# victordeleau/MUI-DeepAutoEncoder

Measured on AMD Instinct MI355X. Metric: training samples/sec at 3x512-dim input, batch 8192, higher is better.
Workload: dtype bf16; 1 GPU; embedding.yaml topology: 3 slots x 512 (io 1536), z=io, 4+4 layers -> 10 x Linear(1536,1536); batch 8192 rows per GPU, Adam lr 1e-5 wd 1e-4 clip 1.0, slot-blanking k=1; global_batch=8192, parallelism=dp1

## Files before the change

### mui-deepautoencoder_amd/csrc/codae_common.h

```cpp
#pragma once
#include <hip/hip_runtime.h>
#include <stdint.h>
#include <stdio.h>
#include <type_traits>

#include "codae_hip.h"

namespace codae {

void set_error(const char* fmt, ...);

#define CODAE_HIP_CHECK(expr)                                                              \
    do {                                                                                   \
        hipError_t e_ = (expr);                                                            \
        if (e_ != hipSuccess) {                                                            \
            codae::set_error("%s failed: %s (%s:%d)", #expr, hipGetErrorString(e_), __FILE__, __LINE__); \
            return CODAE_E_HIP;                                                            \
        }                                                                                  \
    } while (0)

#define CODAE_LAUNCH_CHECK()                                                               \
    do {                                                                                   \
        hipError_t e_ = hipGetLastError();                                                 \
        if (e_ != hipSuccess) {                                                            \
            codae::set_error("kernel launch failed: %s (%s:%d)", hipGetErrorString(e_), __FILE__, __LINE__); \
            return CODAE_E_HIP;                                                            \
        }                                                                                  \
    } while (0)

#define CODAE_REQUIRE(cond, ...)                                                           \
    do {                                                                                   \
        if (!(cond)) {                                                                     \
            codae::set_error(__VA_ARGS__);                                                 \
            return CODAE_E_INVALID;                                                        \
        }                                                                                  \
    } while (0)

typedef uint16_t bf16_t;

typedef __attribute__((ext_vector_type(16))) float f32x16;
typedef __attribute__((ext_vector_type(4))) float f32x4;
typedef __attribute__((ext_vector_type(8))) __bf16 bf16x8;
typedef __attribute__((ext_vector_type(4))) short s16x4;
typedef __attribute__((ext_vector_type(8))) short s16x8;
typedef __attribute__((ext_vector_type(2))) unsigned int u32x2;
typedef __attribute__((ext_vector_type(4))) unsigned int u32x4;

__device__ __forceinline__ float bf16_to_f32(bf16_t v) { return __uint_as_float(((uint32_t)v) << 16); }
__device__ __forceinline__ bf16_t f32_to_bf16(float f) {
    __bf16 b = (__bf16)f;
    return __builtin_bit_cast(bf16_t, b);
}

__device__ __forceinline__ uint32_t pack_bf16x2(float lo, float hi) {
    typedef float f32x2_t __attribute__((ext_vector_type(2)));
    typedef __bf16 bf16x2_t __attribute__((ext_vector_type(2)));
    const f32x2_t v = {lo, hi};
    return __builtin_bit_cast(uint32_t, __builtin_convertvector(v, bf16x2_t));
}
__device__ __forceinline__ float clamp_below(float x, float floor) {
    float r;
    asm("v_maximum3_f32 %0, %1, %2, %2" : "=v"(r) : "v"(x), "v"(floor));
    return r;
}

__device__ __forceinline__ float4 load_bias4(const float* __restrict__ bias, const void* valid, int j, int N) {
    const bool ok = bias != nullptr && j < N;
    const float4 v = *reinterpret_cast<const float4*>(ok ? bias + j : reinterpret_cast<const float*>(valid));
    return make_float4(ok ? v.x : 0.f, ok ? v.y : 0.f, ok ? v.z : 0.f, ok ? v.w : 0.f);
}

__device__ __forceinline__ float act_opaque(float x) { asm("" : "+v"(x)); return x; }
__device__ __forceinline__ float act_exp(float x) { return __builtin_amdgcn_exp2f(act_opaque(x * 1.44269504f)); }
__device__ __forceinline__ float act_log(float x) { return act_opaque(__builtin_amdgcn_logf(x)) * 0.693147181f; }
__device__ __forceinline__ float act_rcp(float x) { return __builtin_amdgcn_rcpf(x); }
__device__ __forceinline__ float act_expm1(float x) {
    const float u = act_opaque(act_exp(x));
    const float um1 = act_opaque(u - 1.f);
    if (u == 1.f) return x;
    if (um1 == -1.f) return -1.f;
    return act_opaque(um1 * x) * act_rcp(act_log(u));
}
__device__ __forceinline__ float act_log1p(float t) {
    const float u = act_opaque(1.f + t);
    if (u == 1.f) return t;
    return act_opaque(act_log(u) * t) * act_rcp(act_opaque(u - 1.f));
}
__device__ __forceinline__ float act_fwd_(int kind, const float* p, float v) {
    switch (kind) {
        case CODAE_ACT_RELU: return clamp_below(v, 0.f);
        case CODAE_ACT_LEAKY: return v > 0.f ? v : v * p[0];
        case CODAE_ACT_RELU6: return v <= 0.f ? 0.f : (v >= 6.f ? 6.f : v);
        case CODAE_ACT_ELU: return v > 0.f ? v * p[0] : act_expm1(v * p[2]) * act_opaque(p[1] * p[0]);
        case CODAE_ACT_SOFTPLUS: return v * p[0] > p[1] ? v : act_log1p(act_exp(v * p[0])) * act_rcp(p[0]);
        case CODAE_ACT_HARDSIGMOID: { const float t = clamp_below(v + 3.f, 0.f); return (t > 6.f ? 6.f : t) * (1.f / 6.f); }
        default: return v;
    }
}
__device__ __forceinline__ float act_fwd(int kind, const float* p, float v) {
    asm("" : "+v"(v));
    float r = act_fwd_(kind, p, v);
    asm("" : "+v"(r));
    return r;
}
__device__ __forceinline__ float act_dy_from_y_(int kind, const float* p, float y) {
    switch (kind) {
        case CODAE_ACT_RELU: return y > 0.f ? 1.f : 0.f;
        case CODAE_ACT_LEAKY: return y > 0.f ? 1.f : p[0];
        case CODAE_ACT_RELU6: return (y > 0.f && y < 6.f) ? 1.f : 0.f;
        case CODAE_ACT_ELU: return y > 0.f ? p[0] : p[2] * act_opaque(y + act_opaque(p[1] * p[0]));
        case CODAE_ACT_SOFTPLUS: return y * p[0] > p[1] ? 1.f : -act_expm1(-y * p[0]);
        case CODAE_ACT_HARDSIGMOID: return (y > 0.f && y < 1.f) ? 1.f / 6.f : 0.f;
        default: return 1.f;
    }
}
__device__ __forceinline__ float act_dy_from_y(int kind, const float* p, float y) {
    asm("" : "+v"(y));
    float r = act_dy_from_y_(kind, p, y);
    asm("" : "+v"(r));
    return r;
}

__device__ __forceinline__ float act_bwd(int kind, const float* p, float g, float y) {
    const float d = act_dy_from_y(kind, p, y);
    const bool selects = kind == CODAE_ACT_RELU || kind == CODAE_ACT_RELU6 || kind == CODAE_ACT_HARDSIGMOID;
    return (selects && d == 0.f) ? 0.f : g * d;
}

template <typename F>
__device__ __forceinline__ void act_dispatch(int kind, F&& f) {
    switch (kind) {
        case CODAE_ACT_RELU: f(std::integral_constant<int, CODAE_ACT_RELU>{}); break;
        case CODAE_ACT_LEAKY: f(std::integral_constant<int, CODAE_ACT_LEAKY>{}); break;
        case CODAE_ACT_RELU6: f(std::integral_constant<int, CODAE_ACT_RELU6>{}); break;
        case CODAE_ACT_ELU: f(std::integral_constant<int, CODAE_ACT_ELU>{}); break;
        case CODAE_ACT_SOFTPLUS: f(std::integral_constant<int, CODAE_ACT_SOFTPLUS>{}); break;
        case CODAE_ACT_HARDSIGMOID: f(std::integral_constant<int, CODAE_ACT_HARDSIGMOID>{}); break;
        default: f(std::integral_constant<int, CODAE_ACT_NONE>{}); break;
    }
}

__device__ __forceinline__ uint32_t act_dgrad_bf16x2(int kind, const float* p, uint32_t g2, uint32_t h2) {
    const float lo = act_bwd(kind, p, bf16_to_f32((bf16_t)(g2 & 0xffffu)), bf16_to_f32((bf16_t)(h2 & 0xffffu)));
    const float hi = act_bwd(kind, p, bf16_to_f32((bf16_t)(g2 >> 16)), bf16_to_f32((bf16_t)(h2 >> 16)));
    return pack_bf16x2(lo, hi);
}

static inline int64_t round_up(int64_t x, int64_t m) { return (x + m - 1) / m * m; }

struct EnvToggles {
    int gemm_tile = -1;
    int gemm_dbg = 0;
    int wgrad_splitk = 0;
    int small_tile_max = 200;
    int small_stages = 4;
    int f32_gemm = 0;
    int group_tile = -1;
    bool side_priority_set = false; int side_priority = 0;
    bool no_wt = false, single_stream = false, tail_on_side = false, no_fused_loss = false, flat_adam = false,
         no_fused_norm = false, no_chain = false, no_deep_small = false,
         no_relu_bits = false,
         no_prefetch = false,
         no_defer_wgrad = false;
};
const EnvToggles& env();
void env_reload();

struct GemmF32 {
    const float* A; int64_t a_rs, a_ks;
    const float* B; int64_t b_rs, b_ks;
    float* C; int64_t ldc;
    int M, N, K;
    const float* bias;
    int relu;
    const float* relu_src;
    int64_t ld_relu;
    float* colsum_part;
    const int* m_dev;
    int split_k;
    int act;
    float act_p[3];
};
int gemm_f32(const GemmF32& g, hipStream_t s);
int gemm_f32x3(const GemmF32& g, hipStream_t s);
bool gemm_f32x3_takes(const GemmF32& g);
inline int gemm_f32_colsum_rows(int M) { return (M + 63) / 64; }

constexpr int CODAE_GROUP_MAX = 16;
struct GemmF32Group {
    int n;
    GemmF32 g[CODAE_GROUP_MAX];
    int wg_begin[CODAE_GROUP_MAX + 1];
};
int gemm_f32x3_grouped(GemmF32Group& grp, hipStream_t s);

enum { OP_KC = 0,
       OP_KS = 1
};
struct LossFuse {
    int enabled;
    const float* data;
    const int32_t* row_idx;
    const int32_t* mask_id;
    const int32_t* mask_to_use;
    int nb_run, run;
    const uint8_t* table;
    int io;
    int B;
    float inv_n;
    double* parts;
};

struct GemmBf16 {
    const bf16_t* A; int64_t lda; int a_mode;
    const bf16_t* B; int64_t ldb; int b_mode;
    void* C; int64_t ldc; int c_f32;
    int M, N, K;
    const float* bias;
    int relu;
    const bf16_t* relu_src; int64_t ld_relu;
    float* colsum_part;
    int split_k;
    LossFuse loss;
    int dbg;
    uint8_t* relu_bits_out; const uint8_t* relu_bits; int64_t ld_bits;
    const void* prefetch; int64_t prefetch_bytes;
    int coscheduled;
    double* sumsq_slots;
    int act;
    float act_p[3];
};
bool gemm_bf16_supported(int M, int N, int K);
bool gemm_bf16_takes_relu_bits(int M, int N);
int gemm_bf16_colsum_rows(const GemmBf16& g);
int gemm_bf16_loss_parts(const GemmBf16& g);
int gemm_bf16(const GemmBf16& g, hipStream_t s);
int gemm_bf16_pipe(const GemmBf16& g, int cfg, hipStream_t s);
int choose_split_k(int N, int K, int rows);

struct GemmBf16Group {
    int n;
    GemmBf16 g[CODAE_GROUP_MAX];
    int wg_begin[CODAE_GROUP_MAX + 1];
};
int gemm_bf16_grouped(GemmBf16Group& grp, hipStream_t s);
int gemm_bf16_pipe_grouped(GemmBf16Group& grp, hipStream_t s);

constexpr int CODAE_CHAIN_MAX_WIDTH = 512;
constexpr int CODAE_CHAIN_MAX_LAYERS = 16;
constexpr int CODAE_CHAIN_MAX_BIAS = 6144;
struct ChainArgs {
    int L, rows, B;
    int width[CODAE_CHAIN_MAX_LAYERS + 1];
    uint32_t relu_flags;
    double* scalars;
    const bf16_t* W[CODAE_CHAIN_MAX_LAYERS];
    const bf16_t* Wt[CODAE_CHAIN_MAX_LAYERS];
    const float* bias[CODAE_CHAIN_MAX_LAYERS];
    bf16_t* act[CODAE_CHAIN_MAX_LAYERS];
    bf16_t* dact[CODAE_CHAIN_MAX_LAYERS];
    float* colsum_part[CODAE_CHAIN_MAX_LAYERS];
    const float* data; const int32_t* row_idx; const int32_t* mask_id; const uint8_t* mask_table;
    const int32_t* mask_to_use; int nb_run, run;
    float inv_n;
    double* loss_parts;
    int do_backward;
};
bool chain_supported(int L, const int* in, const int* out);
int chain_rows_per_workgroup();
int launch_chain_step(const ChainArgs& a, hipStream_t s);

int launch_gather_corrupt(const codae_batch* b, void* out, int out_bf16, hipStream_t s, int64_t out_ld = 0);
int check_noise(const codae_noise* noise);
int launch_gather_noise(const codae_batch* b, const codae_noise* noise, int32_t step, const double* step_dev, void* out,
                        int out_bf16, hipStream_t s, int64_t out_ld = 0, const int32_t* noise_rows = nullptr);
int launch_noise_box_muller(const uint32_t* ra, const uint32_t* rb, float* rho, float* c, float* sn, int64_t n, hipStream_t s);
int launch_cast_bf16(const float* src, bf16_t* dst, int64_t n, hipStream_t s);
int launch_corrupt(const float* x, const float* mask, float* out, int64_t n, hipStream_t s);
int launch_expand_masks(const int32_t* mask_id, const uint8_t* table, const int32_t* k_of_mask, int B, int io,
                        int k_max, float* masks_out, float* fmask_out, hipStream_t s);
int launch_mse_loss(const codae_batch* b, const float* y, void* dy, int dy_bf16, float inv_n, float* colsum_part,
                    double* loss_parts, int want_grad, hipStream_t s, int64_t dy_ld = 0);
int mse_loss_colsum_rows(int B);
int launch_mse_dense(const float* x, const float* y, const float* fmask, float* dy, int64_t n, float inv_n,
                     double* scalars, hipStream_t s);
int launch_sumsq(const float* g, int64_t n, double* out, hipStream_t s);
int launch_sumsq_to(const float* g, int64_t n, double* acc, hipStream_t s);
int launch_clip_coef(const double* total_sq, float max_norm, double* coef_out, hipStream_t s);
int launch_clip_adam(float* p, float* g, float* m, float* v, int64_t n, const codae_hyper* hp,
                     const double* grad_sq, bf16_t* shadow, const double* coef_in, hipStream_t s,
                     const double* step_dev = nullptr);
int launch_set_scalar(double* dst, double value, hipStream_t s);
int launch_clip_adam_tiled(float* p, float* g, float* m, float* v, const codae_hyper* hp, const double* grad_sq,
                           bf16_t* shadow, bf16_t* shadow_t, int n_layers, const int64_t* w_off, const int* rows,
                           const int* cols, int transposed_from, int64_t bias_off, int64_t bias_n, hipStream_t s,
                           const double* step_dev = nullptr);
int launch_transpose_bf16(const bf16_t* src, bf16_t* dst, int n, const int64_t* off, const int* rows, const int* cols,
                          hipStream_t s);
int gemm_bf16_timeline(unsigned long long* host_out, int n_wg);
int launch_reduce_slabs_epi(const float* slabs, int n_slabs, int64_t stride, int M, int N, float* C, int64_t ldc, const float* bias,
                            int relu, const float* relu_src, int64_t ld_relu, float* colsum_part, hipStream_t s,
                            int act = CODAE_ACT_NONE, const float* act_p = nullptr);
int launch_reduce_slabs(const float* slabs, int n_slabs, int64_t slab_stride, float* out, int64_t n, double* sumsq,
                        hipStream_t s);
int launch_finish_loss(double* scalars, double inv_n, hipStream_t s, const double* parts = nullptr, int n_parts = 0);
int launch_cast_f32(const bf16_t* src, float* dst, int64_t n, hipStream_t s);
int launch_colsum_f32(const float* src, int M, int N, float* out, hipStream_t s);
int launch_colsum_parts_f32(const float* src, int M, int N, float* parts, hipStream_t s);
struct BiasFinishJobs {
    int n;
    const float* parts[64];
    float* out[64];
    int rows[64], cols[64];
    int col_begin[65];
};
struct LossFinish { double* scalars; double inv_n; const double* parts; int n_parts; };
int launch_bias_finish(const BiasFinishJobs& jobs, double* sumsq, hipStream_t s, const LossFinish* loss = nullptr);

}
```

### mui-deepautoencoder_amd/csrc/elementwise.hip

```cpp
#include "codae_common.h"

namespace codae {
namespace {

constexpr int NT = 256;

inline int grid_for(int64_t work_items) {
    int64_t b = (work_items + NT - 1) / NT;
    if (b < 1) b = 1;
    if (b > 2048) b = 2048;
    return (int)b;
}

__device__ __forceinline__ float wave_sum(float v) {
#pragma unroll
    for (int o = 32; o > 0; o >>= 1) v += __shfl_xor(v, o);
    return v;
}

__device__ __forceinline__ float block_sum(float v, float* red ) {
    v = wave_sum(v);
    const int w = threadIdx.x >> 6;
    if ((threadIdx.x & 63) == 0) red[w] = v;
    __syncthreads();
    float r = 0.f;
    if (threadIdx.x == 0) r = red[0] + red[1] + red[2] + red[3];
    __syncthreads();
    return r;
}

__device__ __forceinline__ uint2 pack_bf16x4(float a, float b, float c, float d) {
    uint2 o;
    o.x = (uint32_t)f32_to_bf16(a) | ((uint32_t)f32_to_bf16(b) << 16);
    o.y = (uint32_t)f32_to_bf16(c) | ((uint32_t)f32_to_bf16(d) << 16);
    return o;
}

__global__ __launch_bounds__(NT) void gather_corrupt_bf16x8_kernel(const float* __restrict__ data,
                                                                   const int32_t* __restrict__ row_idx,
                                                                   const int32_t* __restrict__ mask_id,
                                                                   const uint8_t* __restrict__ table, int B, int io,
                                                                   bf16_t* __restrict__ out,
                                                                   const int32_t* __restrict__ mask_to_use, int nb_run,
                                                                   int run, int64_t out_ld) {
    const bool masked = (mask_id != nullptr) || (mask_to_use != nullptr);
    const int cols = io / 8;
    const int64_t total = (int64_t)B * cols;
    for (int64_t e = (int64_t)blockIdx.x * NT + threadIdx.x; e < total; e += (int64_t)gridDim.x * NT) {
        const int b = (int)(e / cols);
        const int c = (int)(e - (int64_t)b * cols) * 8;
        const int64_t src_row = row_idx ? row_idx[b] : b;
        const float* src = data + src_row * io + c;
        const float4 x0 = *reinterpret_cast<const float4*>(src);
        const float4 x1 = *reinterpret_cast<const float4*>(src + 4);
        float v[8] = {x0.x, x0.y, x0.z, x0.w, x1.x, x1.y, x1.z, x1.w};
        if (masked) {
            const int id = mask_id ? mask_id[b] : mask_to_use[src_row * nb_run + run];
            const uint2 m = *reinterpret_cast<const uint2*>(table + (int64_t)id * io + c);
#pragma unroll
            for (int k = 0; k < 8; ++k) v[k] = (((k < 4 ? m.x : m.y) >> (8 * (k & 3))) & 0xff) ? v[k] : 0.f;
        }
        uint4 o;
        o.x = pack_bf16x2(v[0], v[1]); o.y = pack_bf16x2(v[2], v[3]);
        o.z = pack_bf16x2(v[4], v[5]); o.w = pack_bf16x2(v[6], v[7]);
        *reinterpret_cast<uint4*>(out + (int64_t)b * out_ld + c) = o;
    }
}

template <bool VEC, bool OUT_BF16>
__global__ __launch_bounds__(NT) void gather_corrupt_kernel(const float* __restrict__ data,
                                                            const int32_t* __restrict__ row_idx,
                                                            const int32_t* __restrict__ mask_id,
                                                            const uint8_t* __restrict__ table, int B, int io,
                                                            void* __restrict__ out,
                                                            const int32_t* __restrict__ mask_to_use, int nb_run,
                                                            int run, int64_t out_ld) {
    constexpr int W = VEC ? 4 : 1;
    const bool masked = (mask_id != nullptr) || (mask_to_use != nullptr);
    const int cols = io / W;
    const int64_t total = (int64_t)B * cols;
    for (int64_t e = (int64_t)blockIdx.x * NT + threadIdx.x; e < total; e += (int64_t)gridDim.x * NT) {
        const int b = (int)(e / cols);
        const int c = (int)(e - (int64_t)b * cols) * W;
        const int64_t src_row = row_idx ? row_idx[b] : b;
        const float* src = data + src_row * io + c;
        float v[4];
        if constexpr (VEC) {
            const float4 x = *reinterpret_cast<const float4*>(src);
            v[0] = x.x; v[1] = x.y; v[2] = x.z; v[3] = x.w;
            if (masked) {
                const int id = mask_id ? mask_id[b] : mask_to_use[src_row * nb_run + run];
                const uint32_t m = *reinterpret_cast<const uint32_t*>(table + (int64_t)id * io + c);
#pragma unroll
                for (int k = 0; k < 4; ++k) v[k] = ((m >> (8 * k)) & 0xff) ? v[k] : 0.f;
            }
        } else {
            v[0] = src[0];
            if (masked) {
                const int id = mask_id ? mask_id[b] : mask_to_use[src_row * nb_run + run];
                v[0] = table[(int64_t)id * io + c] ? v[0] : 0.f;
            }
        }
        const int64_t o = (int64_t)b * out_ld + c;
        if constexpr (OUT_BF16) {
            bf16_t* op = reinterpret_cast<bf16_t*>(out) + o;
            if constexpr (VEC) *reinterpret_cast<uint2*>(op) = pack_bf16x4(v[0], v[1], v[2], v[3]);
            else op[0] = f32_to_bf16(v[0]);
        } else {
            float* op = reinterpret_cast<float*>(out) + o;
            if constexpr (VEC) *reinterpret_cast<float4*>(op) = make_float4(v[0], v[1], v[2], v[3]);
            else op[0] = v[0];
        }
    }
}

struct NoiseArgs {
    uint32_t key0, key1;
    uint32_t step;
    const double* step_dev;
    const int32_t* rows;
    uint64_t thresh;
    float p0, p1, p2;
};

__device__ __forceinline__ uint4 philox4x32_10(uint32_t c0, uint32_t c1, uint32_t c2, uint32_t c3, uint32_t k0, uint32_t k1) {
#pragma unroll
    for (int r = 0; r < 10; ++r) {
        const uint32_t hi0 = __umulhi(0xD2511F53u, c0), lo0 = 0xD2511F53u * c0;
        const uint32_t hi1 = __umulhi(0xCD9E8D57u, c2), lo1 = 0xCD9E8D57u * c2;
        c0 = hi1 ^ c1 ^ k0; c1 = lo1; c2 = hi0 ^ c3 ^ k1; c3 = lo0;
        k0 += 0x9E3779B9u; k1 += 0xBB67AE85u;
    }
    return make_uint4(c0, c1, c2, c3);
}

__device__ __forceinline__ void box_muller_parts(uint32_t ra, uint32_t rb, float& rho, float& c, float& sn) {
    const float u1 = (float)((ra >> 8) + 1u) * 5.9604644775390625e-8f;
    const float two_u2 = (float)(rb >> 8) * 1.1920928955078125e-7f;
    rho = sqrtf(-2.f * logf(u1));
    sincospif(two_u2, &sn, &c);
}

__device__ __forceinline__ float noise_elem(int kind_masking, uint32_t rk, float x, const NoiseArgs& a) {
    const bool hit = (uint64_t)rk < a.thresh;
    if (kind_masking) return hit ? 0.f : x;
    return hit ? ((uint64_t)rk < (a.thresh >> 1) ? a.p1 : a.p2) : x;
}

template <int KIND>
__device__ __forceinline__ void noise_apply4(float* v, const uint4 r, const NoiseArgs& a) {
    if constexpr (KIND == CODAE_NOISE_GAUSSIAN) {
        float rho, c, sn;
        box_muller_parts(r.x, r.y, rho, c, sn);
        v[0] = fmaf(a.p0, rho * c, v[0]); v[1] = fmaf(a.p0, rho * sn, v[1]);
        box_muller_parts(r.z, r.w, rho, c, sn);
        v[2] = fmaf(a.p0, rho * c, v[2]); v[3] = fmaf(a.p0, rho * sn, v[3]);
    } else {
        constexpr int M = KIND == CODAE_NOISE_MASKING;
        v[0] = noise_elem(M, r.x, v[0], a); v[1] = noise_elem(M, r.y, v[1], a);
        v[2] = noise_elem(M, r.z, v[2], a); v[3] = noise_elem(M, r.w, v[3], a);
    }
}

template <int KIND>
__device__ __forceinline__ float noise_apply1(float x, const uint4 r, int k, const NoiseArgs& a) {
    if constexpr (KIND == CODAE_NOISE_GAUSSIAN) {
        float rho, c, sn;
        box_muller_parts((k & 2) ? r.z : r.x, (k & 2) ? r.w : r.y, rho, c, sn);
        return fmaf(a.p0, rho * ((k & 1) ? sn : c), x);
    } else {
        const uint32_t rk = (k & 2) ? ((k & 1) ? r.w : r.z) : ((k & 1) ? r.y : r.x);
        return noise_elem(KIND == CODAE_NOISE_MASKING, rk, x, a);
    }
}

template <int KIND>
__global__ __launch_bounds__(NT) void gather_noise_bf16x8_kernel(const float* __restrict__ data, const int32_t* __restrict__ row_idx,
                                                                 const int32_t* __restrict__ mask_id, const uint8_t* __restrict__ table,
                                                                 int B, int io, bf16_t* __restrict__ out,
                                                                 const int32_t* __restrict__ mask_to_use, int nb_run, int run,
                                                                 int64_t out_ld, NoiseArgs na) {
    const bool masked = (mask_id != nullptr) || (mask_to_use != nullptr);
    const uint32_t step = na.step_dev ? (uint32_t)*na.step_dev : na.step;
    const int cols = io / 8;
    const int64_t total = (int64_t)B * cols;
    for (int64_t e = (int64_t)blockIdx.x * NT + threadIdx.x; e < total; e += (int64_t)gridDim.x * NT) {
        const int b = (int)(e / cols);
        const int c = (int)(e - (int64_t)b * cols) * 8;
        const int64_t src_row = row_idx ? row_idx[b] : b;
        const float* src = data + src_row * io + c;
        const float4 x0 = *reinterpret_cast<const float4*>(src);
        const float4 x1 = *reinterpret_cast<const float4*>(src + 4);
        float v[8] = {x0.x, x0.y, x0.z, x0.w, x1.x, x1.y, x1.z, x1.w};
        const uint32_t nrow = na.rows ? (uint32_t)na.rows[b] : (uint32_t)src_row;
        noise_apply4<KIND>(v, philox4x32_10((uint32_t)(c >> 2), nrow, step, 0u, na.key0, na.key1), na);
        noise_apply4<KIND>(v + 4, philox4x32_10((uint32_t)(c >> 2) + 1u, nrow, step, 0u, na.key0, na.key1), na);
        if (masked) {
            const int id = mask_id ? mask_id[b] : mask_to_use[src_row * nb_run + run];
            const uint2 m = *reinterpret_cast<const uint2*>(table + (int64_t)id * io + c);
#pragma unroll
            for (int k = 0; k < 8; ++k) v[k] = (((k < 4 ? m.x : m.y) >> (8 * (k & 3))) & 0xff) ? v[k] : 0.f;
        }
        uint4 o;
        o.x = pack_bf16x2(v[0], v[1]); o.y = pack_bf16x2(v[2], v[3]);
        o.z = pack_bf16x2(v[4], v[5]); o.w = pack_bf16x2(v[6], v[7]);
        *reinterpret_cast<uint4*>(out + (int64_t)b * out_ld + c) = o;
    }
}

template <bool VEC, bool OUT_BF16, int KIND>
__global__ __launch_bounds__(NT) void gather_noise_kernel(const float* __restrict__ data, const int32_t* __restrict__ row_idx,
                                                          const int32_t* __restrict__ mask_id, const uint8_t* __restrict__ table, int B,
                                                          int io, void* __restrict__ out, const int32_t* __restrict__ mask_to_use,
                                                          int nb_run, int run, int64_t out_ld, NoiseArgs na) {
    constexpr int W = VEC ? 4 : 1;
    const bool masked = (mask_id != nullptr) || (mask_to_use != nullptr);
    const uint32_t step = na.step_dev ? (uint32_t)*na.step_dev : na.step;
    const int cols = io / W;
    const int64_t total = (int64_t)B * cols;
    for (int64_t e = (int64_t)blockIdx.x * NT + threadIdx.x; e < total; e += (int64_t)gridDim.x * NT) {
        const int b = (int)(e / cols);
        const int c = (int)(e - (int64_t)b * cols) * W;
        const int64_t src_row = row_idx ? row_idx[b] : b;
        const float* src = data + src_row * io + c;
        const uint32_t nrow = na.rows ? (uint32_t)na.rows[b] : (uint32_t)src_row;
        const uint4 r = philox4x32_10((uint32_t)(c >> 2), nrow, step, 0u, na.key0, na.key1);
        float v[4];
        if constexpr (VEC) {
            const float4 x = *reinterpret_cast<const float4*>(src);
            v[0] = x.x; v[1] = x.y; v[2] = x.z; v[3] = x.w;
            noise_apply4<KIND>(v, r, na);
            if (masked) {
                const int id = mask_id ? mask_id[b] : mask_to_use[src_row * nb_run + run];
                const uint32_t m = *reinterpret_cast<const uint32_t*>(table + (int64_t)id * io + c);
#pragma unroll
                for (int k = 0; k < 4; ++k) v[k] = ((m >> (8 * k)) & 0xff) ? v[k] : 0.f;
            }
        } else {
            v[0] = src[0];
            v[0] = noise_apply1<KIND>(v[0], r, c & 3, na);
            if (masked) {
                const int id = mask_id ? mask_id[b] : mask_to_use[src_row * nb_run + run];
                v[0] = table[(int64_t)id * io + c] ? v[0] : 0.f;
            }
        }
        const int64_t o = (int64_t)b * out_ld + c;
        if constexpr (OUT_BF16) {
            bf16_t* op = reinterpret_cast<bf16_t*>(out) + o;
            if constexpr (VEC) *reinterpret_cast<uint2*>(op) = pack_bf16x4(v[0], v[1], v[2], v[3]);
            else op[0] = f32_to_bf16(v[0]);
        } else {
            float* op = reinterpret_cast<float*>(out) + o;
            if constexpr (VEC) *reinterpret_cast<float4*>(op) = make_float4(v[0], v[1], v[2], v[3]);
            else op[0] = v[0];
        }
    }
}

__global__ __launch_bounds__(NT) void noise_box_muller_kernel(const uint32_t* __restrict__ ra, const uint32_t* __restrict__ rb,
                                                              float* __restrict__ rho, float* __restrict__ c, float* __restrict__ sn,
                                                              int64_t n) {
    for (int64_t e = (int64_t)blockIdx.x * NT + threadIdx.x; e < n; e += (int64_t)gridDim.x * NT)
        box_muller_parts(ra[e], rb[e], rho[e], c[e], sn[e]);
}

__global__ __launch_bounds__(NT) void cast_bf16_kernel(const float* __restrict__ src, bf16_t* __restrict__ dst,
                                                       int64_t n) {
    const int64_t n4 = n / 4;
    for (int64_t e = (int64_t)blockIdx.x * NT + threadIdx.x; e < n4; e += (int64_t)gridDim.x * NT) {
        const float4 x = reinterpret_cast<const float4*>(src)[e];
        reinterpret_cast<uint2*>(dst)[e] = pack_bf16x4(x.x, x.y, x.z, x.w);
    }
    for (int64_t e = n4 * 4 + (int64_t)blockIdx.x * NT + threadIdx.x; e < n; e += (int64_t)gridDim.x * NT)
        dst[e] = f32_to_bf16(src[e]);
}

__global__ __launch_bounds__(NT) void cast_f32_kernel(const bf16_t* __restrict__ src, float* __restrict__ dst,
                                                      int64_t n) {
    for (int64_t e = (int64_t)blockIdx.x * NT + threadIdx.x; e < n; e += (int64_t)gridDim.x * NT)
        dst[e] = bf16_to_f32(src[e]);
}

__global__ __launch_bounds__(NT) void corrupt_kernel(const float* __restrict__ x, const float* __restrict__ m,
                                                     float* __restrict__ out, int64_t n) {
    for (int64_t e = (int64_t)blockIdx.x * NT + threadIdx.x; e < n; e += (int64_t)gridDim.x * NT)
        out[e] = x[e] * m[e];
}

__global__ __launch_bounds__(NT) void expand_masks_kernel(const int32_t* __restrict__ mask_id,
                                                          const uint8_t* __restrict__ table,
                                                          const int32_t* __restrict__ k_of_mask, int B, int io,
                                                          int k_max, float* __restrict__ masks,
                                                          float* __restrict__ fmask) {
    const int64_t total = (int64_t)B * io;
    for (int64_t e = (int64_t)blockIdx.x * NT + threadIdx.x; e < total; e += (int64_t)gridDim.x * NT) {
        const int b = (int)(e / io);
        const int c = (int)(e - (int64_t)b * io);
        const int id = mask_id[b];
        const float v = table[(int64_t)id * io + c] ? 1.f : 0.f;
        const int k = k_of_mask[id] - 1;
        for (int kk = 0; kk < k_max; ++kk) masks[(int64_t)kk * total + e] = (kk == k) ? v : 0.f;
        fmask[e] = v;
    }
}

constexpr int LOSS_ROWS = 32;
constexpr int LOSS_UNROLL = 8;
template <bool VEC, bool DY_BF16>
__global__ __launch_bounds__(NT) void mse_loss_kernel(const float* __restrict__ data,
                                                      const int32_t* __restrict__ row_idx,
                                                      const int32_t* __restrict__ mask_id,
                                                      const uint8_t* __restrict__ table, int B, int io,
                                                      const float* __restrict__ y, void* __restrict__ dy,
                                                      float inv_n, float* __restrict__ colsum_part,
                                                      double* __restrict__ loss_parts, int want_grad,
                                                      const int32_t* __restrict__ mask_to_use, int nb_run, int run, int64_t dy_ld) {
    __shared__ float red[4];
    const bool masked = (mask_id != nullptr) || (mask_to_use != nullptr);
    constexpr int W = VEC ? 4 : 1;
    const int cols = io / W;
    const int r_begin = blockIdx.x * LOSS_ROWS;
    float sq = 0.f, sqp = 0.f;
    for (int cv = threadIdx.x; cv < cols; cv += NT) {
        const int c = cv * W;
        float cs[4] = {0.f, 0.f, 0.f, 0.f};
        for (int r0 = 0; r0 < LOSS_ROWS; r0 += LOSS_UNROLL)
#pragma unroll
        for (int ru = 0; ru < LOSS_UNROLL; ++ru) {
            const int rr = r0 + ru;
            const bool live = r_begin + rr < B;
            const int b = live ? r_begin + rr : B - 1;
            const int64_t src_row = row_idx ? row_idx[b] : b;
            float xv[4], yv[4];
            uint32_t m = 0x01010101u;
            const int id = !masked ? 0 : (mask_id ? mask_id[b] : mask_to_use[src_row * nb_run + run]);
            if constexpr (VEC) {
                const float4 x4 = *reinterpret_cast<const float4*>(data + src_row * io + c);
                const float4 y4 = *reinterpret_cast<const float4*>(y + (int64_t)b * io + c);
                xv[0] = x4.x; xv[1] = x4.y; xv[2] = x4.z; xv[3] = x4.w;
                yv[0] = y4.x; yv[1] = y4.y; yv[2] = y4.z; yv[3] = y4.w;
                if (masked) m = *reinterpret_cast<const uint32_t*>(table + (int64_t)id * io + c);
            } else {
                xv[0] = data[src_row * io + c];
                yv[0] = y[(int64_t)b * io + c];
                if (masked) m = table[(int64_t)id * io + c];
            }
            float g[4];
#pragma unroll
            for (int k = 0; k < W; ++k) {
                const float d = live ? xv[k] - yv[k] : 0.f;
                const float se = d * d;
                sq += se;
                if (((m >> (8 * k)) & 0xff) == 0) sqp += se;
                g[k] = -2.f * d * inv_n;
                cs[k] += g[k];
            }
            if (want_grad && live) {
                const int64_t o = (int64_t)b * dy_ld + c;
                if constexpr (DY_BF16) {
                    bf16_t* op = reinterpret_cast<bf16_t*>(dy) + o;
                    if constexpr (VEC) *reinterpret_cast<uint2*>(op) = pack_bf16x4(g[0], g[1], g[2], g[3]);
                    else op[0] = f32_to_bf16(g[0]);
                } else {
                    float* op = reinterpret_cast<float*>(dy) + o;
                    if constexpr (VEC) *reinterpret_cast<float4*>(op) = make_float4(g[0], g[1], g[2], g[3]);
                    else op[0] = g[0];
                }
// ... 218 lines not shown
                    a.z = act_bwd(act, p, a.z, h.z); a.w = act_bwd(act, p, a.w, h.w);
                } else {
                    a.x = act_fwd(act, p, a.x); a.y = act_fwd(act, p, a.y); a.z = act_fwd(act, p, a.z); a.w = act_fwd(act, p, a.w);
                }
            } else {
                if (relu) { a.x = clamp_below(a.x, 0.f); a.y = clamp_below(a.y, 0.f); a.z = clamp_below(a.z, 0.f); a.w = clamp_below(a.w, 0.f); }
                if (relu_src != nullptr) {
                    const float4 h = *reinterpret_cast<const float4*>(relu_src + (int64_t)i * ld_relu + j);
                    a.x = h.x > 0.f ? a.x : 0.f; a.y = h.y > 0.f ? a.y : 0.f; a.z = h.z > 0.f ? a.z : 0.f; a.w = h.w > 0.f ? a.w : 0.f;
                }
            }
            *reinterpret_cast<float4*>(C + (int64_t)i * ldc + j) = a;
            cs[0] += a.x; cs[1] += a.y; cs[2] += a.z; cs[3] += a.w;
        }
    }
    if (colsum_part != nullptr) {
        red[rg][cg * 4 + 0] = cs[0]; red[rg][cg * 4 + 1] = cs[1]; red[rg][cg * 4 + 2] = cs[2]; red[rg][cg * 4 + 3] = cs[3];
        __syncthreads();
        if (threadIdx.x < 64 && blockIdx.x * 64 + (int)threadIdx.x < N) {
            float t = 0.f;
            for (int r = 0; r < 16; ++r) t += red[r][threadIdx.x];
            colsum_part[(int64_t)blockIdx.y * N + blockIdx.x * 64 + threadIdx.x] = t;
        }
    }
}

__global__ __launch_bounds__(NT) void colsum_parts_f32_kernel(const float* __restrict__ src, int M, int N,
                                                              float* __restrict__ parts) {
    const int r_begin = blockIdx.x * 64;
    const int r_end = min(M, r_begin + 64);
    const int c = blockIdx.y * NT + threadIdx.x;
    if (c >= N) return;
    float s = 0.f;
    for (int r0 = r_begin; r0 < r_end; r0 += 8) {
        float v[8];
#pragma unroll
        for (int k = 0; k < 8; ++k) v[k] = src[(int64_t)min(r0 + k, r_end - 1) * N + c];
#pragma unroll
        for (int k = 0; k < 8; ++k) s += (r0 + k < r_end) ? v[k] : 0.f;
    }
    parts[(int64_t)blockIdx.x * N + c] = s;
}

__global__ __launch_bounds__(NT) void colsum_f32_kernel(const float* __restrict__ src, int M, int N,
                                                        float* __restrict__ out) {
    const int c = blockIdx.x * NT + threadIdx.x;
    if (c >= N) return;
    float s = 0.f;
    for (int r = 0; r < M; ++r) s += src[(int64_t)r * N + c];
    out[c] = s;
}

__global__ __launch_bounds__(NT) void bias_finish_kernel(BiasFinishJobs jobs, double* __restrict__ sumsq, LossFinish lf) {
    __shared__ float red[4];
    if (lf.scalars != nullptr && blockIdx.x == gridDim.x - 1) {
        __shared__ double lred[2][NT];
        double a = 0.0, b = 0.0;
        for (int i = threadIdx.x; i < lf.n_parts; i += NT) { a += lf.parts[2 * i]; b += lf.parts[2 * i + 1]; }
        lred[0][threadIdx.x] = a; lred[1][threadIdx.x] = b;
        __syncthreads();
        for (int o = NT / 2; o > 0; o >>= 1) {
            if ((int)threadIdx.x < o) { lred[0][threadIdx.x] += lred[0][threadIdx.x + o]; lred[1][threadIdx.x] += lred[1][threadIdx.x + o]; }
            __syncthreads();
        }
        if (threadIdx.x == 0) {
            lf.scalars[CODAE_S_SQ_FULL] += lred[0][0];
            lf.scalars[CODAE_S_SQ_PARTIAL] += lred[1][0];
            lf.scalars[CODAE_S_LAST_LOSS] = lred[0][0] * lf.inv_n;
            lf.scalars[CODAE_S_STEP_SQ] = 0.0;
        }
        return;
    }
    const int gc = blockIdx.x * NT + threadIdx.x;
    float sq = 0.f;
    if (gc < jobs.col_begin[jobs.n]) {
        int j = 0;
        while (j + 1 < jobs.n && gc >= jobs.col_begin[j + 1]) ++j;
        const int c = gc - jobs.col_begin[j];
        const int N = jobs.cols[j], R = jobs.rows[j];
        const float* p = jobs.parts[j] + c;
        float s = 0.f;
        int r = 0;
        for (; r + 32 <= R; r += 32) {
            float v[32];
#pragma unroll
            for (int u = 0; u < 32; ++u) v[u] = p[(int64_t)(r + u) * N];
#pragma unroll
            for (int u = 0; u < 32; ++u) s += v[u];
        }
        for (; r + 8 <= R; r += 8) {
            float v[8];
#pragma unroll
            for (int u = 0; u < 8; ++u) v[u] = p[(int64_t)(r + u) * N];
#pragma unroll
            for (int u = 0; u < 8; ++u) s += v[u];
        }
        for (; r < R; ++r) s += p[(int64_t)r * N];
        jobs.out[j][c] = s;
        sq = s * s;
    }
    if (sumsq != nullptr) {
        const float bsq = block_sum(sq, red);
        if (threadIdx.x == 0)
            atomicAdd(sumsq + (CODAE_S_GRAD_SQ_SLOTS - CODAE_S_GRAD_SQ) + (blockIdx.x & (CODAE_S_N_SLOTS - 1)), (double)bsq);
    }
}

struct TransposeJobs {
    int n;
    int64_t off[64];
    int rows[64], cols[64];
    int tile_begin[65];
};
__global__ __launch_bounds__(NT) void transpose_bf16_kernel(const bf16_t* __restrict__ src, bf16_t* __restrict__ dst,
                                                            TransposeJobs jobs) {
    __shared__ bf16_t tile[64][72];
    int m = 0;
    while (m + 1 < jobs.n && (int)blockIdx.x >= jobs.tile_begin[m + 1]) ++m;
    const int t = blockIdx.x - jobs.tile_begin[m];
    const int R = jobs.rows[m], C = jobs.cols[m];
    const int tiles_c = (C + 63) / 64;
    const int r0 = (t / tiles_c) * 64, c0 = (t % tiles_c) * 64;
    const bf16_t* S = src + jobs.off[m];
    bf16_t* D = dst + jobs.off[m];
#pragma unroll
    for (int p = 0; p < 2; ++p) {
        const int q = threadIdx.x + p * NT;
        const int r = q >> 3, c8 = (q & 7) * 8;
        uint4 v = make_uint4(0u, 0u, 0u, 0u);
        if (r0 + r < R && c0 + c8 < C) v = *reinterpret_cast<const uint4*>(S + (int64_t)(r0 + r) * C + c0 + c8);
        *reinterpret_cast<uint4*>(&tile[r][c8]) = v;
    }
    __syncthreads();
#pragma unroll
    for (int p = 0; p < 2; ++p) {
        const int q = threadIdx.x + p * NT;
        const int c = q >> 3, r8 = (q & 7) * 8;
        if (c0 + c < C && r0 + r8 < R) {
            bf16_t e[8];
#pragma unroll
            for (int k = 0; k < 8; ++k) e[k] = tile[r8 + k][c];
            uint4 v;
            v.x = (uint32_t)e[0] | ((uint32_t)e[1] << 16); v.y = (uint32_t)e[2] | ((uint32_t)e[3] << 16);
            v.z = (uint32_t)e[4] | ((uint32_t)e[5] << 16); v.w = (uint32_t)e[6] | ((uint32_t)e[7] << 16);
            *reinterpret_cast<uint4*>(D + (int64_t)(c0 + c) * R + r0 + r8) = v;
        }
    }
}

inline bool a16(const void* p) { return (reinterpret_cast<uintptr_t>(p) & 15) == 0; }

}

int launch_gather_corrupt(const codae_batch* b, void* out, int out_bf16, hipStream_t s, int64_t out_ld) {
    if (out_ld <= 0) out_ld = b ? b->io : 0;
    CODAE_REQUIRE(b && b->data && out && b->B > 0 && b->io > 0, "gather_corrupt: bad batch");
    const bool masked = b->mask_id || b->mask_to_use;
    CODAE_REQUIRE(!masked || b->mask_table, "gather_corrupt: mask ids without mask_table");
    CODAE_REQUIRE(!b->mask_to_use || b->mask_id || (b->nb_run > 0 && b->run >= 0 && b->run < b->nb_run),
                  "gather_corrupt: run %d outside [0, %d)", b->run, b->nb_run);
    const bool vec = (b->io % 4 == 0) && (out_ld % 4 == 0) && a16(b->data) && a16(out) && (!masked || (reinterpret_cast<uintptr_t>(b->mask_table) & 3) == 0);
    const int64_t items = (int64_t)b->B * (vec ? b->io / 4 : b->io);
    const int grid = grid_for(items);
    if (vec && out_bf16 && b->io % 8 == 0 && (!masked || (reinterpret_cast<uintptr_t>(b->mask_table) & 7) == 0)) {
        hipLaunchKernelGGL(gather_corrupt_bf16x8_kernel, dim3(grid_for(items / 2)), dim3(NT), 0, s, b->data, b->row_idx, b->mask_id,
                           b->mask_table, b->B, b->io, reinterpret_cast<bf16_t*>(out), b->mask_to_use, b->nb_run, b->run, out_ld);
        CODAE_LAUNCH_CHECK();
        return CODAE_OK;
    }
#define GC(V, O) hipLaunchKernelGGL((gather_corrupt_kernel<V, O>), dim3(grid), dim3(NT), 0, s, b->data, b->row_idx, \
                                    b->mask_id, b->mask_table, b->B, b->io, out, b->mask_to_use, b->nb_run, b->run, out_ld)
    if (vec && out_bf16) GC(true, true);
    else if (vec) GC(true, false);
    else if (out_bf16) GC(false, true);
    else GC(false, false);
#undef GC
    CODAE_LAUNCH_CHECK();
    return CODAE_OK;
}

static bool finite_f(float x) { return x == x && fabsf(x) <= 3.402823466e38f; }

int check_noise(const codae_noise* n) {
    if (n == nullptr || n->kind == CODAE_NOISE_NONE) return CODAE_OK;
    CODAE_REQUIRE(n->kind == CODAE_NOISE_GAUSSIAN || n->kind == CODAE_NOISE_MASKING || n->kind == CODAE_NOISE_SALT_PEPPER,
                  "input noise: unknown kind %d", n->kind);
    if (n->kind == CODAE_NOISE_GAUSSIAN) {
        CODAE_REQUIRE(finite_f(n->p0) && n->p0 >= 0.f, "input noise: sigma %g must be finite and >= 0", (double)n->p0);
        return CODAE_OK;
    }
    CODAE_REQUIRE(finite_f(n->p0) && n->p0 >= 0.f && n->p0 <= 1.f, "input noise: p %g outside [0, 1]", (double)n->p0);
    if (n->kind == CODAE_NOISE_SALT_PEPPER) {
        CODAE_REQUIRE(finite_f(n->p1), "input noise: lo %g is not finite", (double)n->p1);
        CODAE_REQUIRE(finite_f(n->p2), "input noise: hi %g is not finite", (double)n->p2);
    }
    return CODAE_OK;
}

int launch_gather_noise(const codae_batch* b, const codae_noise* noise, int32_t step, const double* step_dev, void* out, int out_bf16,
                        hipStream_t s, int64_t out_ld, const int32_t* noise_rows) {
    if (noise == nullptr || noise->kind == CODAE_NOISE_NONE) return launch_gather_corrupt(b, out, out_bf16, s, out_ld);
    int rc = check_noise(noise);
    if (rc) return rc;
    if (out_ld <= 0) out_ld = b ? b->io : 0;
    CODAE_REQUIRE(b && b->data && out && b->B > 0 && b->io > 0, "gather_corrupt: bad batch");
    const bool masked = b->mask_id || b->mask_to_use;
    CODAE_REQUIRE(!masked || b->mask_table, "gather_corrupt: mask ids without mask_table");
    CODAE_REQUIRE(!b->mask_to_use || b->mask_id || (b->nb_run > 0 && b->run >= 0 && b->run < b->nb_run),
                  "gather_corrupt: run %d outside [0, %d)", b->run, b->nb_run);
    NoiseArgs na{};
    na.key0 = (uint32_t)(noise->seed & 0xffffffffu); na.key1 = (uint32_t)(noise->seed >> 32);
    na.step = (uint32_t)step; na.step_dev = step_dev; na.rows = noise_rows;
    na.thresh = (uint64_t)floor((double)noise->p0 * 4294967296.0);
    na.p0 = noise->p0; na.p1 = noise->p1; na.p2 = noise->p2;
    const bool vec = (b->io % 4 == 0) && (out_ld % 4 == 0) && a16(b->data) && a16(out) && (!masked || (reinterpret_cast<uintptr_t>(b->mask_table) & 3) == 0);
    const int64_t items = (int64_t)b->B * (vec ? b->io / 4 : b->io);
    const int grid = grid_for(items);
    const bool x8 = vec && out_bf16 && b->io % 8 == 0 && (!masked || (reinterpret_cast<uintptr_t>(b->mask_table) & 7) == 0);
#define GN8(K) hipLaunchKernelGGL((gather_noise_bf16x8_kernel<K>), dim3(grid_for(items / 2)), dim3(NT), 0, s, b->data, b->row_idx, b->mask_id, \
                                  b->mask_table, b->B, b->io, reinterpret_cast<bf16_t*>(out), b->mask_to_use, b->nb_run, b->run, out_ld, na)
#define GN(V, O, K) hipLaunchKernelGGL((gather_noise_kernel<V, O, K>), dim3(grid), dim3(NT), 0, s, b->data, b->row_idx, b->mask_id, \
                                       b->mask_table, b->B, b->io, out, b->mask_to_use, b->nb_run, b->run, out_ld, na)
#define GN_KIND(K)                           \
    do {                                     \
        if (x8) GN8(K);                      \
        else if (vec && out_bf16) GN(true, true, K);  \
        else if (vec) GN(true, false, K);    \
        else if (out_bf16) GN(false, true, K);        \
        else GN(false, false, K);            \
    } while (0)
    if (noise->kind == CODAE_NOISE_GAUSSIAN) GN_KIND(CODAE_NOISE_GAUSSIAN);
    else if (noise->kind == CODAE_NOISE_MASKING) GN_KIND(CODAE_NOISE_MASKING);
    else GN_KIND(CODAE_NOISE_SALT_PEPPER);
#undef GN_KIND
#undef GN
#undef GN8
    CODAE_LAUNCH_CHECK();
    return CODAE_OK;
}

int launch_noise_box_muller(const uint32_t* ra, const uint32_t* rb, float* rho, float* c, float* sn, int64_t n, hipStream_t s) {
    CODAE_REQUIRE(ra && rb && rho && c && sn && n > 0, "noise_box_muller: bad args");
    hipLaunchKernelGGL(noise_box_muller_kernel, dim3(grid_for(n)), dim3(NT), 0, s, ra, rb, rho, c, sn, n);
    CODAE_LAUNCH_CHECK();
    return CODAE_OK;
}

int launch_cast_bf16(const float* src, bf16_t* dst, int64_t n, hipStream_t s) {
    CODAE_REQUIRE(src && dst && n > 0 && a16(src) && (reinterpret_cast<uintptr_t>(dst) & 7) == 0, "cast: bad args");
    hipLaunchKernelGGL(cast_bf16_kernel, dim3(grid_for(n / 4 + 1)), dim3(NT), 0, s, src, dst, n);
    CODAE_LAUNCH_CHECK();
    return CODAE_OK;
}

int launch_cast_f32(const bf16_t* src, float* dst, int64_t n, hipStream_t s) {
    CODAE_REQUIRE(src && dst && n > 0, "cast: bad args");
    hipLaunchKernelGGL(cast_f32_kernel, dim3(grid_for(n)), dim3(NT), 0, s, src, dst, n);
    CODAE_LAUNCH_CHECK();
    return CODAE_OK;
}

int launch_corrupt(const float* x, const float* mask, float* out, int64_t n, hipStream_t s) {
    CODAE_REQUIRE(x && mask && out && n > 0, "corrupt: bad args");
    hipLaunchKernelGGL(corrupt_kernel, dim3(grid_for(n)), dim3(NT), 0, s, x, mask, out, n);
    CODAE_LAUNCH_CHECK();
    return CODAE_OK;
}

int launch_expand_masks(const int32_t* mask_id, const uint8_t* table, const int32_t* k_of_mask, int B, int io,
                        int k_max, float* masks_out, float* fmask_out, hipStream_t s) {
    CODAE_REQUIRE(mask_id && table && k_of_mask && masks_out && fmask_out && B > 0 && io > 0 && k_max > 0,
                  "expand_masks: bad args");
    hipLaunchKernelGGL(expand_masks_kernel, dim3(grid_for((int64_t)B * io)), dim3(NT), 0, s, mask_id, table,
                       k_of_mask, B, io, k_max, masks_out, fmask_out);
    CODAE_LAUNCH_CHECK();
    return CODAE_OK;
}

int mse_loss_colsum_rows(int B) { return (B + LOSS_ROWS - 1) / LOSS_ROWS; }

int launch_mse_loss(const codae_batch* b, const float* y, void* dy, int dy_bf16, float inv_n, float* colsum_part,
                    double* loss_parts, int want_grad, hipStream_t s, int64_t dy_ld) {
    if (dy_ld <= 0) dy_ld = b ? b->io : 0;
    CODAE_REQUIRE(b && b->data && y && loss_parts && b->B > 0 && b->io > 0, "mse_loss: bad args");
    CODAE_REQUIRE(!want_grad || dy, "mse_loss: gradient requested without dy");
    const bool masked = b->mask_id || b->mask_to_use;
    CODAE_REQUIRE(!masked || b->mask_table, "mse_loss: mask ids without mask_table");
    const bool vec = (b->io % 4 == 0) && (dy_ld % 4 == 0) && a16(b->data) && a16(y) && (!dy || a16(dy)) &&
                     (!masked || (reinterpret_cast<uintptr_t>(b->mask_table) & 3) == 0);
    const int grid = (b->B + LOSS_ROWS - 1) / LOSS_ROWS;
#define ML(V, O) hipLaunchKernelGGL((mse_loss_kernel<V, O>), dim3(grid), dim3(NT), 0, s, b->data, b->row_idx, \
                                    b->mask_id, b->mask_table, b->B, b->io, y, dy, inv_n, colsum_part, loss_parts, want_grad, \
                                    b->mask_to_use, b->nb_run, b->run, dy_ld)
    if (vec && dy_bf16) ML(true, true);
    else if (vec) ML(true, false);
    else if (dy_bf16) ML(false, true);
    else ML(false, false);
#undef ML
    CODAE_LAUNCH_CHECK();
    return CODAE_OK;
}

int launch_mse_dense(const float* x, const float* y, const float* fmask, float* dy, int64_t n, float inv_n,
                     double* scalars, hipStream_t s) {
    CODAE_REQUIRE(x && y && scalars && n > 0, "mse_dense: bad args");
    hipLaunchKernelGGL(mse_dense_kernel, dim3(grid_for(n)), dim3(NT), 0, s, x, y, fmask, dy, n, inv_n, scalars);
    CODAE_LAUNCH_CHECK();
    return CODAE_OK;
}

int launch_finish_loss(double* scalars, double inv_n, hipStream_t s, const double* parts, int n_parts) {
    hipLaunchKernelGGL(finish_loss_kernel, dim3(1), dim3(NT), 0, s, scalars, inv_n, parts, parts ? n_parts : 0);
    CODAE_LAUNCH_CHECK();
    return CODAE_OK;
}

int launch_sumsq(const float* g, int64_t n, double* out, hipStream_t s) {
    CODAE_REQUIRE(g && out && n > 0 && a16(g), "sumsq: bad args");
    hipLaunchKernelGGL(sumsq_kernel, dim3(grid_for(n / 4 + 1)), dim3(NT), 0, s, g, n, out);
    CODAE_LAUNCH_CHECK();
    return CODAE_OK;
}

struct AdamTiles {
    int n_layers;
    int64_t off[64];
    int rows[64], cols[64];
    int tile_begin[65];
    int transposed_from;
    int64_t bias_off, bias_n;
};
constexpr int AT_R = 64, AT_C = 128;

__global__ __launch_bounds__(NT) void clip_adam_tiled_kernel(float* __restrict__ p, const float* __restrict__ g,
                                                             float* __restrict__ m, float* __restrict__ v, AdamConst c,
                                                             const double* __restrict__ grad_sq, bf16_t* __restrict__ shadow,
                                                             bf16_t* __restrict__ shadow_t, AdamTiles jobs,
                                                             const double* __restrict__ step_dev) {
    __shared__ bf16_t tt[AT_C][AT_R + 8];
    __shared__ double total_sq;
    if (step_dev != nullptr) {
        const double t = *step_dev;
        c.lr_over_bc1 = (float)((double)c.lr / (1.0 - pow((double)c.beta1, t)));
        c.inv_sqrt_bc2 = (float)(1.0 / sqrt(1.0 - pow((double)c.beta2, t)));
    }
    float coef = 1.f;
    if (c.max_norm > 0.f) {
        if (threadIdx.x < 64) {
            double sv = grad_sq[(CODAE_S_GRAD_SQ_SLOTS - CODAE_S_GRAD_SQ) + threadIdx.x];
#pragma unroll
            for (int o = 32; o > 0; o >>= 1) sv += __shfl_xor(sv, o);
            if (threadIdx.x == 0) total_sq = sv + grad_sq[0];
        }
        __syncthreads();
        coef = clip_coef(c.max_norm, sqrtf((float)total_sq));
    }
    const int n_tiles = jobs.tile_begin[jobs.n_layers];
    if ((int)blockIdx.x >= n_tiles) {
        const int64_t nb = (int64_t)gridDim.x - n_tiles;
        for (int64_t e = ((int64_t)blockIdx.x - n_tiles) * NT + threadIdx.x; e < jobs.bias_n; e += nb * NT) {
            const int64_t i = jobs.bias_off + e;
            float pp = p[i], mm = m[i], vv = v[i];
            adam_one(pp, g[i], mm, vv, coef, c);
            p[i] = pp; m[i] = mm; v[i] = vv;
            shadow[i] = f32_to_bf16(pp);
// ... 194 lines not shown
```

### mui-deepautoencoder_amd/csrc/engine.hip

```cpp
#include <stdarg.h>
#include <stdlib.h>
#include <string.h>

#include <cmath>
#include <vector>

#include "layer_gemm.h"
#include <dlfcn.h>
#include <rccl/rccl.h>

namespace codae {

static thread_local char g_err[512] = "";

void set_error(const char* fmt, ...) {
    va_list ap;
    va_start(ap, fmt);
    vsnprintf(g_err, sizeof(g_err), fmt, ap);
    va_end(ap);
}

static EnvToggles g_env;
static bool g_env_loaded = false;

void env_reload() {
    EnvToggles e;
    if (const char* t = getenv("CODAE_GEMM_TILE")) {
        switch (t[0]) { case 's': e.gemm_tile = 0; break; case 'q': e.gemm_tile = 3; break; case 'x': e.gemm_tile = 6; break; case 'm': e.gemm_tile = 7; break; default: break; }
    }
    if (const char* d = getenv("CODAE_GEMM_DBG")) e.gemm_dbg = atoi(d);
    if (const char* k = getenv("CODAE_WGRAD_SPLITK")) e.wgrad_splitk = atoi(k) > 0 ? atoi(k) : 0;
    if (const char* k = getenv("CODAE_GROUP_TILE")) e.group_tile = (k[0] >= '0' && k[0] <= '2') ? k[0] - '0' : -1;
    if (const char* pr = getenv("CODAE_SIDE_PRIORITY")) { e.side_priority_set = true; e.side_priority = atoi(pr); }
    e.no_wt = getenv("CODAE_NO_WT") != nullptr;
    e.single_stream = getenv("CODAE_SINGLE_STREAM") != nullptr;
    e.tail_on_side = getenv("CODAE_TAIL_ON_SIDE") != nullptr;
    e.no_fused_loss = getenv("CODAE_NO_FUSED_LOSS") != nullptr;
    e.flat_adam = getenv("CODAE_FLAT_ADAM") != nullptr;
    e.no_fused_norm = getenv("CODAE_NO_FUSED_NORM") != nullptr;
    e.no_chain = getenv("CODAE_NO_CHAIN") != nullptr;
    e.no_deep_small = getenv("CODAE_NO_DEEP_SMALL") != nullptr;
    e.no_defer_wgrad = getenv("CODAE_NO_DEFER_WGRAD") != nullptr;
    e.no_prefetch = getenv("CODAE_NO_PREFETCH") != nullptr;
    e.no_relu_bits = getenv("CODAE_NO_RELU_BITS") != nullptr;
    if (const char* k = getenv("CODAE_F32_GEMM")) e.f32_gemm = k[0] == 'n' ? 1 : (k[0] == 'x' ? 2 : 0);
    if (const char* k = getenv("CODAE_SMALL_TILE_MAX")) e.small_tile_max = atoi(k);
    if (const char* k = getenv("CODAE_SMALL_STAGES")) e.small_stages = atoi(k) == 2 ? 2 : 4;
    g_env = e;
    g_env_loaded = true;
}

const EnvToggles& env() {
    if (!g_env_loaded) env_reload();
    return g_env;
}

}

using namespace codae;

constexpr int CODAE_MAX_DACT = 16;

struct codae_engine {
    int L = 0;
    std::vector<int> in, out;
    std::vector<int> in_ld, out_ld;
    std::vector<uint8_t> relu;
    std::vector<uint8_t> act;
    std::vector<float> act_p;
    int max_batch = 0, max_rows = 0;
    int prec = CODAE_PREC_F32;
    std::vector<int64_t> w_off, b_off;
    int64_t n_param = 0, bias_begin = 0;
    int maxw = 0;
    std::vector<int64_t> act_off;
    int64_t act_bytes = 0, dact_one = 0, slab_bytes = 0;
    std::vector<int64_t> bits_off;
    int n_dact = 3;
    std::vector<int> split_k;
    std::vector<int64_t> part_off;
    int64_t part_floats = 0;
    int64_t loss_part_off = 0;
    int loss_part_cap = 0;
    bool chain_ok = false;
    codae_noise noise{};
    std::vector<int> parts_pending;
    hipStream_t side = nullptr;
    hipEvent_t ev_ready[CODAE_MAX_DACT] = {}, ev_join = nullptr, ev_w[CODAE_MAX_DACT] = {};
    unsigned ready_turn = 0;
    bool w_pending[CODAE_MAX_DACT] = {};
    bool side_dirty = false;
    bool norm_scalars_zero = false;
    bool prof_on = false;
    uint32_t prof_mask = 0;
    int prof_n = 0;
    int prof_every = 1, prof_step = 0;
    hipGraphExec_t graph_exec = nullptr;
    bool capturing = false;
    struct GraphKey { codae_batch batch; codae_hyper hyper; codae_buffers bufs; codae_noise noise; } graph_key{};
    std::vector<hipEvent_t> prof_start, prof_stop;
    std::vector<int> prof_kind;
    std::vector<int> prof_count;
    bool prof_group = false;
    EnvToggles cfg;
    struct DpState* dp = nullptr;
    int esize() const { return prec == CODAE_PREC_BF16 ? 2 : 4; }
    int rows_for(int B) const { return prec == CODAE_PREC_BF16 ? (int)round_up(B, 64) : B; }
};

struct RcclApi {
    void* lib = nullptr;
    ncclResult_t (*GetUniqueId)(ncclUniqueId*) = nullptr;
    ncclResult_t (*CommInitRank)(ncclComm_t*, int, ncclUniqueId, int) = nullptr;
    ncclResult_t (*CommDestroy)(ncclComm_t) = nullptr;
    ncclResult_t (*AllReduce)(const void*, void*, size_t, ncclDataType_t, ncclRedOp_t, ncclComm_t, hipStream_t) = nullptr;
    const char* (*GetErrorString)(ncclResult_t) = nullptr;
};
static RcclApi g_rccl;

static int rccl_load() {
    if (g_rccl.lib != nullptr) return CODAE_OK;
    void* lib = nullptr;
    for (const char* name : {"librccl.so.1", "librccl.so"}) {
        lib = dlopen(name, RTLD_NOW | RTLD_NOLOAD | RTLD_LOCAL);
        if (lib != nullptr) break;
    }
    if (lib == nullptr)
        for (const char* name : {"librccl.so.1", "librccl.so", "/opt/rocm/lib/librccl.so.1"}) {
            lib = dlopen(name, RTLD_NOW | RTLD_LOCAL);
            if (lib != nullptr) break;
        }
    if (lib == nullptr) { codae::set_error("codae_dp: librccl.so not found (%s)", dlerror()); return CODAE_E_UNSUPPORTED; }
    RcclApi a;
    a.lib = lib;
    a.GetUniqueId = reinterpret_cast<decltype(a.GetUniqueId)>(dlsym(lib, "ncclGetUniqueId"));
    a.CommInitRank = reinterpret_cast<decltype(a.CommInitRank)>(dlsym(lib, "ncclCommInitRank"));
    a.CommDestroy = reinterpret_cast<decltype(a.CommDestroy)>(dlsym(lib, "ncclCommDestroy"));
    a.AllReduce = reinterpret_cast<decltype(a.AllReduce)>(dlsym(lib, "ncclAllReduce"));
    a.GetErrorString = reinterpret_cast<decltype(a.GetErrorString)>(dlsym(lib, "ncclGetErrorString"));
    if (!a.GetUniqueId || !a.CommInitRank || !a.CommDestroy || !a.AllReduce || !a.GetErrorString) {
        codae::set_error("codae_dp: librccl.so lacks an entry point");
        return CODAE_E_UNSUPPORTED;
    }
    g_rccl = a;
    return CODAE_OK;
}

#define CODAE_RCCL_CHECK(expr)                                                                         \
    do {                                                                                               \
        ncclResult_t r_ = (expr);                                                                      \
        if (r_ != ncclSuccess) {                                                                       \
            codae::set_error("%s failed: %s (%s:%d)", #expr, g_rccl.GetErrorString(r_), __FILE__, __LINE__); \
            return CODAE_E_HIP;                                                                        \
        }                                                                                              \
    } while (0)

constexpr int CODAE_DP_MAX_BUCKETS = 64;
struct DpState {
    ncclComm_t comm = nullptr;
    int rank = 0, world = 1;
    hipStream_t stream = nullptr;
    hipEvent_t ev_bucket[CODAE_DP_MAX_BUCKETS + 1] = {};
    hipEvent_t ev_done = nullptr;
};

namespace codae {

int choose_split_k(int N, int K, int rows) {
    const int kt = rows / 64;
    int s;
    if (kt <= 4 && env().wgrad_splitk <= 0) return 1;
    if (env().wgrad_splitk > 0) {
        s = env().wgrad_splitk;
    } else {
        const int tiles_big = ((N + 255) / 256) * ((K + 191) / 192);
        s = (256 + tiles_big / 2) / tiles_big;
        if (s > 8) s = 8;
        if (s > kt) s = kt;
        if (s < 1) s = 1;
        if (tiles_big * s >= 160) return s;
        const int tiles = ((N + 127) / 128) * ((K + 127) / 128);
        s = (512 + tiles / 2) / tiles;
        if (s > 8) s = 8;
    }
    if (s > kt) s = kt;
    if (s < 1) s = 1;
    return s;
}

}

namespace {

struct ProfScope {
    codae_engine* e;
    hipStream_t s;
    int slot = -1;
// ... 132 lines not shown
    const int B = batch->B, L = e->L, rows = e->rows_for(B);
    ChainArgs a{};
    a.L = L; a.rows = rows; a.B = B;
    for (int l = 0; l < L; ++l) {
        a.width[l] = e->in[l];
        if (e->relu[l]) a.relu_flags |= 1u << l;
        a.W[l] = reinterpret_cast<const bf16_t*>(b->shadow_w) + e->w_off[l];
        a.Wt[l] = reinterpret_cast<const bf16_t*>(b->shadow_wt) + e->w_off[l];
        a.bias[l] = b->params + e->b_off[l];
        a.act[l] = reinterpret_cast<bf16_t*>(act_ptr(e, b, l));
        a.dact[l] = reinterpret_cast<bf16_t*>(dact_ptr(e, b, l));
        a.colsum_part[l] = part_ptr(e, b, l);
    }
    a.width[L] = e->out[L - 1];
    a.data = batch->data; a.row_idx = batch->row_idx; a.mask_id = batch->mask_id; a.mask_table = batch->mask_table;
    a.mask_to_use = batch->mask_to_use; a.nb_run = batch->nb_run; a.run = batch->run;
    a.inv_n = (float)loss_inv_n(hyper, batch);
    a.loss_parts = loss_parts_ptr(e, b);
    a.do_backward = backward ? 1 : 0;
    a.scalars = loss_out != nullptr ? b->scalars : nullptr;
    const int n_wg = rows / chain_rows_per_workgroup();
    CODAE_REQUIRE(n_wg <= e->loss_part_cap, "chain: %d workgroups exceed the partial-sum rows (%d)", n_wg, e->loss_part_cap);
    int rc;
    {
        ProfScope prof(e, CODAE_K_CHAIN, s);
        rc = launch_chain_step(a, s);
    }
    if (rc) return rc;
    if (backward)
        for (int l = 0; l < L; ++l) e->parts_pending[l] = n_wg;
    e->norm_scalars_zero = true;
    if (loss_out != nullptr) {
        loss_out->scalars = b->scalars; loss_out->inv_n = 1.0 / ((double)B * batch->io);
        loss_out->parts = loss_parts_ptr(e, b); loss_out->n_parts = n_wg;
        return CODAE_OK;
    }
    return finish_loss(e, b, batch, n_wg, s);
}

int run_wgrad_grouped(codae_engine* e, const codae_buffers* b, int rows, bool with_norm, hipStream_t s) {
    for (int base = 0; base < e->L; base += CODAE_GROUP_MAX) {
        GemmBf16Group grp{};
        grp.n = 0;
        for (int l = base; l < e->L && grp.n < CODAE_GROUP_MAX; ++l) {
            GemmBf16& g = grp.g[grp.n++];
            g = layer_wgrad_bf16(e, b, l, rows);
            g.sumsq_slots = with_norm ? b->scalars + CODAE_S_GRAD_SQ_SLOTS : nullptr;
        }
        ProfScope prof(e, CODAE_K_GEMM_WGRAD, s);
        int rc = gemm_bf16_grouped(grp, s);
        if (rc) return rc;
    }
    return CODAE_OK;
}

int defer_wgrad_mode(codae_engine* e, int rows) {
    if (e->prec == CODAE_PREC_F32) {
        if (env().f32_gemm == 1 || e->cfg.no_defer_wgrad || e->cfg.single_stream || e->L > CODAE_GROUP_MAX || e->n_dact <= e->L || rows < 256 ||
            rows % 32 != 0)
            return 0;
        int total = 0;
        for (int l = 0; l < e->L; ++l) {
            if (e->in[l] % 4 != 0 || e->out[l] % 4 != 0) return 0;
            total += ((e->out[l] + 127) / 128) * ((e->in[l] + 127) / 128);
        }
        return total >= 256 ? 3 : 0;
    }
    if (e->prec != CODAE_PREC_BF16 || e->cfg.no_defer_wgrad || e->cfg.single_stream || e->L > CODAE_GROUP_MAX || e->n_dact <= e->L || rows < 64)
        return 0;
    int total = 0, total_small = 0;
    for (int l = 0; l < e->L; ++l) {
        total += ((e->out[l] + 255) / 256) * ((e->in[l] + 191) / 192);
        total_small += ((e->out[l] + 63) / 64) * ((e->in[l] + 63) / 64);
        if ((int64_t)rows * e->out_ld[l] * 2 >= (int64_t)1 << 32 || (int64_t)rows * e->in_ld[l] * 2 >= (int64_t)1 << 32) return 0;
    }
    if (total >= 200) return 1;
    return total_small >= 128 ? 2 : 0;
}

int run_wgrad_deferred_f32(codae_engine* e, const codae_buffers* b, int rows, hipStream_t s) {
    GemmF32Group grp{};
    grp.n = 0;
    for (int l = e->L - 1; l >= 0; --l)
        grp.g[grp.n++] = layer_wgrad_f32(e, b, l, rows);
    ProfScope prof(e, CODAE_K_GEMM_WGRAD, s);
    prof.counts_as(grp.n);
    return gemm_f32x3_grouped(grp, s);
}

int run_wgrad_deferred(codae_engine* e, const codae_buffers* b, int rows, bool with_norm, hipStream_t s) {
    GemmBf16Group grp{};
    grp.n = 0;
    for (int l = e->L - 1; l >= 0; --l) {
        GemmBf16& g = grp.g[grp.n++];
        g = layer_wgrad_bf16(e, b, l, rows);
        g.sumsq_slots = with_norm ? b->scalars + CODAE_S_GRAD_SQ_SLOTS : nullptr;
    }
    ProfScope prof(e, CODAE_K_GEMM_WGRAD, s);
    prof.counts_as(grp.n);
    return gemm_bf16_pipe_grouped(grp, s);
}

int gemm_f32_small(codae_engine* e, const codae_buffers* b, const GemmF32& g, hipStream_t s) {
    const int tiles = ((g.M + 127) / 128) * ((g.N + 127) / 128);
    const int kt = (g.K + 31) / 32;
    int S = tiles >= 128 ? 1 : (256 + tiles / 2) / tiles;
    if (S > kt / 4) S = kt / 4;
    if (S > 16) S = 16;
    while (S > 1 && (int64_t)S * g.M * g.N * 4 > e->slab_bytes) --S;
    if (S <= 1 || b->slabs == nullptr || e->cfg.no_deep_small || (g.N % 4) != 0 || (g.ldc % 4) != 0 || g.m_dev != nullptr ||
        (g.relu_src != nullptr && (g.ld_relu % 4) != 0))
        return gemm_f32(g, s);
    float* slab = reinterpret_cast<float*>(reinterpret_cast<char*>(b->slabs) + 2 * e->slab_bytes);
    GemmF32 p = g;
    p.C = slab; p.ldc = g.N; p.bias = nullptr; p.relu = 0; p.relu_src = nullptr; p.ld_relu = 0; p.colsum_part = nullptr; p.split_k = S;
    p.act = CODAE_ACT_NONE;
    int rc = gemm_f32(p, s);
    if (rc) return rc;
    return launch_reduce_slabs_epi(slab, S, (int64_t)g.M * g.N, g.M, g.N, g.C, g.ldc, g.bias, g.relu, g.relu_src, g.ld_relu, g.colsum_part, s,
                                   g.act, g.act_p);
}

int run_linear(codae_engine* e, const codae_buffers* b, int l, const void* x, void* y, bool y_f32, int rows,
               hipStream_t s) {
    const int N = e->out[l], K = e->in[l];
    ProfScope prof(e, CODAE_K_GEMM_FWD, s);
    if (e->prec == CODAE_PREC_BF16) {
        GemmBf16 g = layer_fwd_bf16(e, b, l, x, y, y_f32 ? N : e->out_ld[l], y_f32, rows);
        set_activation(g, e->relu[l], e->act[l], &e->act_p[3 * l]);
        if (!y_f32 && l + 1 < e->L && e->bits_off[l + 1] >= 0 && e->relu[l] && y == act_ptr(e, b, l + 1) && gemm_bf16_takes_relu_bits(rows, N)) {
            g.relu_bits_out = reinterpret_cast<uint8_t*>(b->acts) + e->bits_off[l + 1];
            g.ld_bits = e->in_ld[l + 1] / 8;
        }
        if (l + 1 < e->L && !e->cfg.no_prefetch) {
            g.prefetch = reinterpret_cast<const bf16_t*>(b->shadow_w) + e->w_off[l + 1];
            g.prefetch_bytes = (int64_t)e->in[l + 1] * e->out[l + 1] * 2;
        }
        return gemm_bf16(g, s);
    }
    GemmF32 g = fwd_gemm_f32(reinterpret_cast<const float*>(x), b->params + e->w_off[l], reinterpret_cast<float*>(y), rows, N, K,
                             b->params + e->b_off[l]);
    set_activation(g, e->relu[l], e->act[l], &e->act_p[3 * l]);
    return gemm_f32_small(e, b, g, s);
}

int run_wgrad(codae_engine* e, const codae_buffers* b, int l, int rows, bool with_norm, hipStream_t s, int slot = 0) {
    const int N = e->out[l], K = e->in[l];
    float* dW = b->grads + e->w_off[l];
    if (e->prec == CODAE_PREC_BF16) {
        const int S = e->split_k[l] <= rows / 64 ? e->split_k[l] : rows / 64;
        GemmBf16 g = layer_wgrad_bf16(e, b, l, rows);
        g.split_k = S;
        if (S > 1) {
            CODAE_REQUIRE(b->slabs != nullptr, "bf16 wgrad needs the slab workspace");
            char* slab = reinterpret_cast<char*>(b->slabs) + (int64_t)slot * e->slab_bytes;
            g.C = slab;
            int rc;
            {
                ProfScope prof(e, CODAE_K_GEMM_WGRAD, s);
                rc = gemm_bf16(g, s);
            }
            if (rc) return rc;
            ProfScope prof(e, CODAE_K_SLAB_REDUCE, s);
            return launch_reduce_slabs(reinterpret_cast<const float*>(slab), S, (int64_t)N * K, dW, (int64_t)N * K,
                                       with_norm ? b->scalars + CODAE_S_GRAD_SQ : nullptr, s);
        }
        if (with_norm) g.sumsq_slots = b->scalars + CODAE_S_GRAD_SQ_SLOTS;
        ProfScope prof(e, CODAE_K_GEMM_WGRAD, s);
        return gemm_bf16(g, s);
    }
    GemmF32 g = layer_wgrad_f32(e, b, l, rows);
    int S = e->split_k[l];
    if (S > rows / 32) S = rows / 32;
    if (S > 1 && b->slabs != nullptr) {
        float* slab = reinterpret_cast<float*>(reinterpret_cast<char*>(b->slabs) + (int64_t)slot * e->slab_bytes);
        g.C = slab; g.split_k = S;
        int rc;
        {
            ProfScope prof(e, CODAE_K_GEMM_WGRAD, s);
            rc = gemm_f32(g, s);
        }
        if (rc) return rc;
        ProfScope prof(e, CODAE_K_SLAB_REDUCE, s);
        return launch_reduce_slabs(slab, S, (int64_t)N * K, dW, (int64_t)N * K, nullptr, s);
    }
    ProfScope prof(e, CODAE_K_GEMM_WGRAD, s);
    return gemm_f32(g, s);
}

int run_dgrad(codae_engine* e, const codae_buffers* b, int l, int rows, bool coscheduled, float* dx_f32, hipStream_t s) {
    const int N = e->out[l], K = e->in[l];
    const bool to_dx = (dx_f32 != nullptr);
    ProfScope prof(e, CODAE_K_GEMM_DGRAD, s);
    if (e->prec == CODAE_PREC_BF16) {
        const bool wt = b->shadow_wt != nullptr && l >= 1 && !e->cfg.no_wt;
        const bf16_t* W = reinterpret_cast<const bf16_t*>(wt ? b->shadow_wt : b->shadow_w) + e->w_off[l];
        GemmBf16 g = dgrad_gemm_bf16(dact_ptr(e, b, l), e->out_ld[l], W, wt ? N : K, wt, to_dx ? (void*)dx_f32 : dact_ptr(e, b, l - 1),
                                     to_dx ? K : e->out_ld[l - 1], to_dx ? 1 : 0, rows, K, e->out_ld[l]);
        g.coscheduled = coscheduled ? 1 : 0;
        if (!to_dx) {
            if (e->act[l - 1] != CODAE_ACT_NONE) {
                g.relu_src = reinterpret_cast<const bf16_t*>(act_ptr(e, b, l)); g.ld_relu = e->in_ld[l];
                set_activation(g, 0, e->act[l - 1], &e->act_p[3 * (l - 1)]);
            } else if (e->relu[l - 1]) {
                g.relu_src = reinterpret_cast<const bf16_t*>(act_ptr(e, b, l)); g.ld_relu = e->in_ld[l];
                if (e->bits_off[l] >= 0 && gemm_bf16_takes_relu_bits(rows, K)) {
                    g.relu_bits = reinterpret_cast<const uint8_t*>(b->acts) + e->bits_off[l];
                    g.ld_bits = e->in_ld[l] / 8;
                }
            }
            g.colsum_part = part_ptr(e, b, l - 1);
            e->parts_pending[l - 1] = gemm_bf16_colsum_rows(g);
            if (b->shadow_wt != nullptr && l >= 2 && !e->cfg.no_wt && !e->cfg.no_prefetch) {
                g.prefetch = reinterpret_cast<const bf16_t*>(b->shadow_wt) + e->w_off[l - 1];
                g.prefetch_bytes = (int64_t)e->in[l - 1] * e->out[l - 1] * 2;
            }
        }
        return gemm_bf16(g, s);
    }
    GemmF32 g = dgrad_gemm_f32(reinterpret_cast<const float*>(dact_ptr(e, b, l)), b->params + e->w_off[l],
                               to_dx ? dx_f32 : reinterpret_cast<float*>(dact_ptr(e, b, l - 1)), rows, N, K);
    if (!to_dx) {
        if (e->relu[l - 1] || e->act[l - 1] != CODAE_ACT_NONE) {
            g.relu_src = reinterpret_cast<const float*>(act_ptr(e, b, l)); g.ld_relu = K;
            set_activation(g, 0, e->act[l - 1], &e->act_p[3 * (l - 1)]);
        }
        g.colsum_part = part_ptr(e, b, l - 1);
        e->parts_pending[l - 1] = gemm_f32_colsum_rows(rows);
    }
    return gemm_f32_small(e, b, g, s);
}

int refresh_transposed(codae_engine* e, const codae_buffers* b, hipStream_t s, int l_lo = 1, int l_hi = -1) {
    if (e->prec != CODAE_PREC_BF16 || b->shadow_wt == nullptr || e->L < 2) return CODAE_OK;
    if (l_hi < 0) l_hi = e->L;
    for (int base = l_lo; base < l_hi; base += 64) {
        int64_t off[64]; int rows[64], cols[64]; int n = 0;
        for (int l = base; l < l_hi && n < 64; ++l) { off[n] = e->w_off[l]; rows[n] = e->out[l]; cols[n] = e->in[l]; ++n; }
        int rc = launch_transpose_bf16(reinterpret_cast<const bf16_t*>(b->shadow_w), reinterpret_cast<bf16_t*>(b->shadow_wt),
                                       n, off, rows, cols, s);
        if (rc) return rc;
    }
    return CODAE_OK;
}

int zero_pad_rows(codae_engine* e, void* base, int B, int rows, int width, hipStream_t s) {
    if (rows > B) {
        char* p = reinterpret_cast<char*>(base) + (int64_t)B * width * e->esize();
        CODAE_HIP_CHECK(hipMemsetAsync(p, 0, (int64_t)(rows - B) * width * e->esize(), s));
    }
    return CODAE_OK;
}

int ensure_side_stream(codae_engine* h) {
    if (h->side != nullptr) return CODAE_OK;
    int prio_least = 0, prio_greatest = 0;
    CODAE_HIP_CHECK(hipDeviceGetStreamPriorityRange(&prio_least, &prio_greatest));
    const int prio = h->cfg.side_priority_set ? h->cfg.side_priority : prio_least;
    CODAE_HIP_CHECK(hipStreamCreateWithPriority(&h->side, hipStreamNonBlocking, prio));
    for (int i = 0; i < CODAE_MAX_DACT; ++i) CODAE_HIP_CHECK(hipEventCreateWithFlags(&h->ev_ready[i], hipEventDisableTiming));
    CODAE_HIP_CHECK(hipEventCreateWithFlags(&h->ev_join, hipEventDisableTiming));
    for (int i = 0; i < CODAE_MAX_DACT; ++i) CODAE_HIP_CHECK(hipEventCreateWithFlags(&h->ev_w[i], hipEventDisableTiming));
    return CODAE_OK;
}

int join_side(codae_engine* h, hipStream_t s) {
    if (!h->side_dirty || h->side == nullptr) return CODAE_OK;
    CODAE_HIP_CHECK(hipEventRecord(h->ev_join, h->side));
    CODAE_HIP_CHECK(hipStreamWaitEvent(s, h->ev_join, 0));
    for (int i = 0; i < CODAE_MAX_DACT; ++i) h->w_pending[i] = false;
    h->side_dirty = false;
    return CODAE_OK;
}

int backward_range(codae_handle h, const codae_buffers* b, int B, int lo, int hi, float* dx, bool step_mode, bool with_norm,
                   hipStream_t s, bool join = true) {
    const int rows = h->rows_for(B);
    const bool dual = !h->cfg.single_stream;
    if (dual) {
        int rc = ensure_side_stream(h);
        if (rc) return rc;
    }
    const int defer = ((step_mode || dx == nullptr) && join && lo == 0 && hi == h->L && h->L >= 2) ? defer_wgrad_mode(h, rows) : 0;
    if (defer != 0) {
        int rc = join_side(h, s);
        if (rc) return rc;
        for (int l = hi - 1; l >= 1; --l) {
            rc = run_dgrad(h, b, l, rows, false, nullptr, s);
            if (rc) return rc;
        }
        rc = defer == 3 ? run_wgrad_deferred_f32(h, b, rows, s)
                        : (defer == 1 ? run_wgrad_deferred(h, b, rows, with_norm, s) : run_wgrad_grouped(h, b, rows, with_norm, s));
        if (rc) return rc;
        return finish_bias(h, b, s, with_norm);
    }
    bool* w_pending = h->w_pending;
    const bool coscheduled = dual;
    for (int l = hi - 1; l >= lo; --l) {
        int rc;
        if (!dual) {
            rc = run_wgrad(h, b, l, rows, with_norm, s);
        } else if (join && step_mode && l == 0 && hi - lo >= 3 && !h->cfg.tail_on_side) {
            rc = run_wgrad(h, b, l, rows, with_norm, s, 2);
        } else {
            hipEvent_t ready = h->ev_ready[h->ready_turn++ % CODAE_MAX_DACT];
            CODAE_HIP_CHECK(hipEventRecord(ready, s));
            CODAE_HIP_CHECK(hipStreamWaitEvent(h->side, ready, 0));
            rc = run_wgrad(h, b, l, rows, with_norm, h->side, l & 1);
            if (rc == CODAE_OK && h->n_dact <= h->L) {
                CODAE_HIP_CHECK(hipEventRecord(h->ev_w[l % h->n_dact], h->side));
                w_pending[l % h->n_dact] = true;
            }
        }
        if (rc) return rc;
        const bool chain = step_mode ? (l > 0) : (l > lo);
        const bool to_dx = !chain && !step_mode && dx != nullptr;
        if (chain || to_dx) {
            const int wb = (l - 1 + h->n_dact) % h->n_dact;
            if (dual && chain && w_pending[wb]) {
                CODAE_HIP_CHECK(hipStreamWaitEvent(s, h->ev_w[wb], 0));
                w_pending[wb] = false;
            }
            rc = chain ? run_dgrad(h, b, l, rows, coscheduled, nullptr, s) : run_dgrad(h, b, l, B, coscheduled, dx, s);
            if (rc) return rc;
        }
    }
    if (join || lo == 0) {
        int rc = finish_bias(h, b, s, with_norm);
        if (rc) return rc;
    }
    if (dual) {
        h->side_dirty = true;
        if (join) return join_side(h, s);
    }
    return CODAE_OK;
}

}

extern "C" {

const char* codae_last_error(void) { return g_err; }
int codae_abi_version(void) { return CODAE_ABI_VERSION; }

int codae_reload_env(void) {
    env_reload();
    return CODAE_OK;
}

int codae_struct_sizes(int32_t* out, int32_t capacity) {
    CODAE_REQUIRE(out != nullptr && capacity >= CODAE_N_STRUCTS, "codae_struct_sizes: need room for %d entries", CODAE_N_STRUCTS);
    out[0] = (int32_t)sizeof(codae_spec);
    out[1] = (int32_t)sizeof(codae_sizes);
    out[2] = (int32_t)sizeof(codae_buffers);
    out[3] = (int32_t)sizeof(codae_batch);
    out[4] = (int32_t)sizeof(codae_hyper);
    out[5] = CODAE_S_COUNT;
    out[6] = CODAE_K_COUNT;
    return CODAE_OK;
}

int codae_create(const codae_spec* spec, codae_handle* out) {
    CODAE_REQUIRE(spec && out, "codae_create: null argument");
    CODAE_REQUIRE(spec->n_layers > 0 && spec->n_layers <= 64, "codae_create: n_layers %d", spec->n_layers);
    CODAE_REQUIRE(spec->max_batch > 0, "codae_create: max_batch %d", spec->max_batch);
    CODAE_REQUIRE(spec->precision == CODAE_PREC_F32 || spec->precision == CODAE_PREC_BF16, "codae_create: precision");
    for (int l = 0; l < spec->n_layers; ++l) {
        CODAE_REQUIRE(spec->in_features[l] > 0 && spec->out_features[l] > 0, "codae_create: layer %d has an empty side", l);
        CODAE_REQUIRE(l == 0 || spec->in_features[l] == spec->out_features[l - 1],
                      "codae_create: layer %d input %d != previous output %d", l, spec->in_features[l], spec->out_features[l - 1]);
        if (spec->precision == CODAE_PREC_BF16) {
            if (spec->in_features[l] % 8 != 0 || spec->out_features[l] % 8 != 0) {
                set_error("codae_create: bf16 mode needs every layer width to be a multiple of 8 (layer %d is %d -> %d); use CODAE_PREC_F32",
                          l, spec->in_features[l], spec->out_features[l]);
                return CODAE_E_UNSUPPORTED;
            }
        }
    }
    if (spec->act_kind != nullptr) {
        for (int l = 0; l < spec->n_layers; ++l) {
            const int kind = spec->act_kind[l];
            const float* p = spec->act_param ? spec->act_param + 3 * l : nullptr;
            CODAE_REQUIRE(kind >= CODAE_ACT_NONE && kind <= CODAE_ACT_HARDSIGMOID, "codae_create: layer %d: unknown activation kind %d", l, kind);
            CODAE_REQUIRE(l + 1 < spec->n_layers || kind == CODAE_ACT_NONE || kind == CODAE_ACT_RELU,
                          "codae_create: the last layer takes no activation other than ReLU (kind %d)", kind);
            const bool needs_p = kind == CODAE_ACT_LEAKY || kind == CODAE_ACT_ELU || kind == CODAE_ACT_SOFTPLUS;
            CODAE_REQUIRE(!needs_p || p != nullptr, "codae_create: layer %d: activation kind %d needs act_param", l, kind);
            if (kind == CODAE_ACT_LEAKY)
                CODAE_REQUIRE(p[0] >= 0.f && std::isfinite(p[0]), "codae_create: layer %d: LeakyReLU slope %g (need >= 0)", l, p[0]);
            if (kind == CODAE_ACT_ELU)
                CODAE_REQUIRE(p[0] > 0.f && p[1] > 0.f && p[2] > 0.f && std::isfinite(p[0]) && std::isfinite(p[1]) && std::isfinite(p[2]),
                              "codae_create: layer %d: ELU parameters scale %g alpha %g 1/beta %g (need all > 0)", l, p[0], p[1], p[2]);
            if (kind == CODAE_ACT_SOFTPLUS)
                CODAE_REQUIRE(p[0] > 0.f && std::isfinite(p[0]) && !std::isnan(p[1]),
                              "codae_create: layer %d: Softplus beta %g threshold %g (need beta > 0)", l, p[0], p[1]);
        }
    }
    env_reload();
    codae_engine* e = new codae_engine();
    e->cfg = env();
    e->L = spec->n_layers;
    e->prec = spec->precision;
    e->max_batch = spec->max_batch;
    e->max_rows = (int)round_up(spec->max_batch, 64);
    int64_t off = 0;
    for (int l = 0; l < e->L; ++l) {
        e->in.push_back(spec->in_features[l]);
        e->out.push_back(spec->out_features[l]);
        const int kind = spec->act_kind ? spec->act_kind[l] : (spec->relu[l] ? CODAE_ACT_RELU : CODAE_ACT_NONE);
        e->relu.push_back(kind == CODAE_ACT_RELU ? 1 : 0);
        e->act.push_back(kind == CODAE_ACT_RELU ? CODAE_ACT_NONE : (uint8_t)kind);
        for (int k = 0; k < 3; ++k) e->act_p.push_back(spec->act_kind && spec->act_param ? spec->act_param[3 * l + k] : 0.f);
        e->in_ld.push_back(e->prec == CODAE_PREC_BF16 ? (int)round_up(e->in[l], 64) : e->in[l]);
        e->out_ld.push_back(e->prec == CODAE_PREC_BF16 ? (int)round_up(e->out[l], 64) : e->out[l]);
        e->w_off.push_back(off);
        off += round_up((int64_t)e->in[l] * e->out[l], 64);
        if (e->in_ld[l] > e->maxw) e->maxw = e->in_ld[l];
        if (e->out_ld[l] > e->maxw) e->maxw = e->out_ld[l];
    }
    e->bias_begin = off;
    for (int l = 0; l < e->L; ++l) {
        e->b_off.push_back(off);
        off += round_up(e->out[l], 64);
    }
    e->n_param = off;
    int64_t a = 0;
    for (int l = 0; l < e->L; ++l) {
        e->act_off.push_back(a);
        a += round_up((int64_t)e->max_rows * e->in_ld[l] * e->esize(), 256);
    }
    e->act_off.push_back(a);
    a += round_up((int64_t)e->max_rows * e->out[e->L - 1] * 4, 256);
    e->bits_off.assign(e->L, -1);
    if (e->prec == CODAE_PREC_BF16 && !e->cfg.no_relu_bits) {
        for (int l = 1; l < e->L; ++l) {
            if (!e->relu[l - 1]) continue;
            e->bits_off[l] = a;
            a += round_up((int64_t)e->max_rows * (e->in_ld[l] / 8), 256);
        }
    }
    e->act_bytes = a;
    e->dact_one = round_up((int64_t)e->max_rows * e->maxw * e->esize(), 256);
    e->n_dact = e->L + 1 <= CODAE_MAX_DACT ? e->L + 1 : CODAE_MAX_DACT;
    if (e->n_dact < 3) e->n_dact = 3;
    if (e->prec == CODAE_PREC_BF16 && e->n_dact <= e->L) {
        for (int l = 0; l < e->L; ++l)
            if (e->in[l] % 64 != 0 || e->out[l] % 64 != 0) {
                set_error("codae_create: bf16 stacks deeper than %d layers need widths that are multiples of 64 (layer %d is %d -> %d)",
                          CODAE_MAX_DACT - 1, l, e->in[l], e->out[l]);
                delete e;
                return CODAE_E_UNSUPPORTED;
            }
    }
    bool generic_act = false;
    for (int l = 0; l < e->L; ++l) generic_act = generic_act || e->act[l] != CODAE_ACT_NONE;
    e->chain_ok = e->prec == CODAE_PREC_BF16 && !e->cfg.no_chain && !generic_act && e->L + 1 <= CODAE_MAX_DACT &&
                  chain_supported(e->L, e->in.data(), e->out.data()) && e->in[0] == e->out[e->L - 1];
    e->parts_pending.assign(e->L, 0);
    e->part_floats = 0;
    const int chain_rows = e->max_rows < CHAIN_MAX_ROWS ? e->max_rows : CHAIN_MAX_ROWS;
    for (int l = 0; l < e->L; ++l) {
        e->part_off.push_back(e->part_floats);
        int64_t rows_cap = (l == e->L - 1) ? (e->max_rows + 31) / 32 : (e->max_rows + 63) / 64;
        if (e->chain_ok && chain_rows / 16 > rows_cap) rows_cap = chain_rows / 16;
        e->part_floats += round_up(rows_cap * (int64_t)e->out[l], 64);
    }
    {
        const int io = e->out[e->L - 1];
        const int by_rows = (e->max_rows + 31) / 32;
        const int by_tiles = ((e->max_rows + 63) / 64) * ((io + 63) / 64);
        e->loss_part_cap = by_rows > by_tiles ? by_rows : by_tiles;
        if (e->chain_ok && chain_rows / 16 > e->loss_part_cap) e->loss_part_cap = chain_rows / 16;
        e->loss_part_off = e->part_floats;
        e->part_floats += round_up((int64_t)e->loss_part_cap * 4, 64);
    }
    e->slab_bytes = 0;
    for (int l = 0; l < e->L; ++l) {
        int s = 1;
        if (e->prec == CODAE_PREC_BF16) s = choose_split_k(e->out[l], e->in[l], e->max_rows);
        else s = choose_split_k_f32(e->out[l], e->in[l], e->max_rows);
        e->split_k.push_back(s);
        if (s > 1) {
            const int64_t bytes = (int64_t)s * e->in[l] * e->out[l] * 4;
            if (bytes > e->slab_bytes) e->slab_bytes = bytes;
        }
    }
    if (e->prec == CODAE_PREC_F32 && e->max_rows <= 512) {
        const int64_t bytes = (int64_t)16 * e->max_rows * e->maxw * 4;
        if (bytes > e->slab_bytes) e->slab_bytes = bytes;
    }
    *out = e;
    return CODAE_OK;
}

static void profile_release(codae_handle h) {
    for (hipEvent_t ev : h->prof_start) (void)hipEventDestroy(ev);
    for (hipEvent_t ev : h->prof_stop) (void)hipEventDestroy(ev);
    h->prof_start.clear(); h->prof_stop.clear(); h->prof_kind.clear(); h->prof_count.clear(); h->prof_group = false;
    h->prof_on = false; h->prof_n = 0;
}

int codae_destroy(codae_handle h) {
    if (h) profile_release(h);
    if (h && h->graph_exec) { (void)hipGraphExecDestroy(h->graph_exec); h->graph_exec = nullptr; }
    if (h && h->side) {
        (void)hipStreamSynchronize(h->side);
        for (int i = 0; i < CODAE_MAX_DACT; ++i) if (h->ev_ready[i]) (void)hipEventDestroy(h->ev_ready[i]);
        (void)hipEventDestroy(h->ev_join);
        for (int i = 0; i < CODAE_MAX_DACT; ++i) (void)hipEventDestroy(h->ev_w[i]);
        (void)hipStreamDestroy(h->side);
    }
    if (h && h->dp) (void)codae_dp_destroy(h);
    delete h;
    return CODAE_OK;
}

int codae_profile_begin(codae_handle h, uint32_t class_mask, int32_t max_records) {
    CODAE_REQUIRE(h && max_records > 0 && max_records <= (1 << 20), "codae_profile_begin: bad arguments");
    profile_release(h);
    h->prof_start.resize(max_records); h->prof_stop.resize(max_records); h->prof_kind.assign(max_records, -1); h->prof_count.assign(max_records, 1);
    for (int i = 0; i < max_records; ++i) {
        CODAE_HIP_CHECK(hipEventCreate(&h->prof_start[i]));
        CODAE_HIP_CHECK(hipEventCreate(&h->prof_stop[i]));
    }
    h->prof_mask = class_mask; h->prof_n = 0; h->prof_on = true; h->prof_step = 0;
    return CODAE_OK;
}

int codae_profile_stride(codae_handle h, int32_t every_n_steps) {
    CODAE_REQUIRE(h && every_n_steps >= 1, "codae_profile_stride: bad arguments");
    h->prof_every = every_n_steps;
    return CODAE_OK;
}

int codae_profile_end(codae_handle h, int32_t* kinds, float* ms, int32_t capacity, int32_t* n_out) {
    CODAE_REQUIRE(h && kinds && ms && n_out, "codae_profile_end: null argument");
    h->prof_on = false;
    int n = 0;
    for (int i = 0; i < h->prof_n && n < capacity; ++i) {
        CODAE_HIP_CHECK(hipEventSynchronize(h->prof_stop[i]));
        float t = 0.f;
        CODAE_HIP_CHECK(hipEventElapsedTime(&t, h->prof_start[i], h->prof_stop[i]));
        const int c = h->prof_count[i];
        for (int k = 0; k < c && n < capacity; ++k) { kinds[n] = h->prof_kind[i]; ms[n] = t / (float)c; ++n; }
    }
    *n_out = n;
    profile_release(h);
    return CODAE_OK;
}

int codae_get_sizes(codae_handle h, codae_sizes* out) {
    CODAE_REQUIRE(h && out, "codae_get_sizes: null argument");
    out->n_param = h->n_param;
    out->n_weight = h->prec == CODAE_PREC_BF16 ? h->n_param + (int64_t)64 * h->maxw : 0;
    out->act_bytes = h->act_bytes;
    out->dact_bytes = h->n_dact * h->dact_one;
    out->slab_bytes = 3 * h->slab_bytes;
    out->bias_part_bytes = h->part_floats * 4;
    out->n_scalars = CODAE_S_COUNT;
    return CODAE_OK;
}

int codae_param_offsets(codae_handle h, int32_t layer, int64_t* w_off, int64_t* b_off, int64_t* shadow_off) {
    CODAE_REQUIRE(h && layer >= 0 && layer < h->L, "codae_param_offsets: layer %d", layer);
    if (w_off) *w_off = h->w_off[layer];
    if (b_off) *b_off = h->b_off[layer];
    if (shadow_off) *shadow_off = h->w_off[layer];
    return CODAE_OK;
}

int codae_sync_shadows(codae_handle h, const codae_buffers* b, void* stream) {
    CODAE_REQUIRE(h && b && b->params, "codae_sync_shadows: null argument");
    if (h->prec != CODAE_PREC_BF16) return CODAE_OK;
    CODAE_REQUIRE(b->shadow_w, "codae_sync_shadows: shadow_w missing");
    int rc = launch_cast_bf16(b->params, reinterpret_cast<bf16_t*>(b->shadow_w), h->n_param, (hipStream_t)stream);
    if (rc) return rc;
    return refresh_transposed(h, b, (hipStream_t)stream);
}

int codae_forward(codae_handle h, const codae_buffers* b, const float* x, float* y, int32_t B, int32_t layer_lo,
                  int32_t layer_hi, int32_t save_for_backward, void* stream) {
    int rc = check_common(h, b, B);
    if (rc) return rc;
    CODAE_REQUIRE(x && y, "codae_forward: null x or y");
    CODAE_REQUIRE(layer_lo >= 0 && layer_lo < layer_hi && layer_hi <= h->L, "codae_forward: layer range [%d, %d)", layer_lo, layer_hi);
    (void)save_for_backward;
    hipStream_t s = (hipStream_t)stream;
    const int rows = h->rows_for(B);
    codae_batch in{};
    in.data = x; in.B = B; in.io = h->in[layer_lo];
    rc = launch_gather_corrupt(&in, act_ptr(h, b, layer_lo), h->prec == CODAE_PREC_BF16, s, h->in_ld[layer_lo]);
    if (rc) return rc;
    rc = zero_pad_rows(h, act_ptr(h, b, layer_lo), B, rows, h->in_ld[layer_lo], s);
    if (rc) return rc;
    for (int l = layer_lo; l < layer_hi; ++l) {
        const bool last = (l == layer_hi - 1);
        if (last) {
            rc = run_linear(h, b, l, act_ptr(h, b, l), y, true, B, s);
        } else {
            rc = run_linear(h, b, l, act_ptr(h, b, l), act_ptr(h, b, l + 1), false, rows, s);
        }
        if (rc) return rc;
    }
    return CODAE_OK;
}

int codae_backward(codae_handle h, const codae_buffers* b, const float* dy, float* dx, int32_t B, int32_t layer_lo,
                   int32_t layer_hi, void* stream) {
    int rc = check_common(h, b, B);
    if (rc) return rc;
    CODAE_REQUIRE(dy && b->grads && b->dacts, "codae_backward: null dy / grads / dacts");
    CODAE_REQUIRE(layer_lo >= 0 && layer_lo < layer_hi && layer_hi <= h->L, "codae_backward: layer range [%d, %d)", layer_lo, layer_hi);
    hipStream_t s = (hipStream_t)stream;
    const int rows = h->rows_for(B);
    const int top = layer_hi - 1;
    CODAE_REQUIRE(b->bias_parts, "codae_backward: bias_parts missing");
    codae_batch in{};
    in.data = dy; in.B = B; in.io = h->out[top];
    rc = launch_gather_corrupt(&in, dact_ptr(h, b, top), h->prec == CODAE_PREC_BF16, s, h->out_ld[top]);
    if (rc) return rc;
    rc = zero_pad_rows(h, dact_ptr(h, b, top), B, rows, h->out_ld[top], s);
    if (rc) return rc;
    rc = launch_colsum_parts_f32(dy, B, h->out[top], part_ptr(h, b, top), s);
    if (rc) return rc;
    h->parts_pending[top] = (B + 63) / 64;
    return backward_range(h, b, B, layer_lo, layer_hi, dx, false, false, s);
}

int codae_step_forward_loss(codae_handle h, const codae_buffers* b, const codae_batch* batch, const codae_hyper* hyper,
                            float* out_y, void* stream) {
    CODAE_REQUIRE(batch != nullptr, "codae_step_forward_loss: null batch");
    int rc = check_common(h, b, batch->B);
    if (rc) return rc;
    CODAE_REQUIRE(batch->io == h->in[0] && batch->io == h->out[h->L - 1], "batch.io %d does not match the model (%d -> %d)",
                  batch->io, h->in[0], h->out[h->L - 1]);
    CODAE_REQUIRE(b->grads && b->dacts && b->scalars, "codae_step_forward_loss: grads / dacts / scalars missing");
    CODAE_REQUIRE(b->bias_parts, "codae_step_forward_loss: bias_parts missing");
    if (h->prof_on) ++h->prof_step;
    hipStream_t s = (hipStream_t)stream;
    const int B = batch->B, L = h->L;
    const int rows = h->rows_for(B);
    const bool bf = h->prec == CODAE_PREC_BF16;
    {
        ProfScope prof(h, CODAE_K_GATHER, s);
        if (hyper != nullptr && h->noise.kind != CODAE_NOISE_NONE)
            rc = launch_gather_noise(batch, &h->noise, hyper->step, h->capturing ? b->scalars + CODAE_S_ADAM_STEP : nullptr,
                                     act_ptr(h, b, 0), bf, s, h->in_ld[0]);
        else
            rc = launch_gather_corrupt(batch, act_ptr(h, b, 0), bf, s, h->in_ld[0]);
    }
    if (rc) return rc;
    rc = zero_pad_rows(h, act_ptr(h, b, 0), B, rows, h->in_ld[0], s);
    if (rc) return rc;
    float* y = out_y ? out_y : reinterpret_cast<float*>(act_ptr(h, b, L));
    const bool fuse_loss = bf && hyper != nullptr && out_y == nullptr && !h->cfg.no_fused_loss;
    GroupScope fwd_group(h, CODAE_K_GEMM_FWD, s);
    for (int l = 0; l < L; ++l) {
        const bool last = (l == L - 1);
        if (last && fuse_loss) {
            fwd_group.close();
            GemmBf16 g = layer_fwd_bf16(h, b, l, act_ptr(h, b, l), dact_ptr(h, b, l), h->out_ld[l], false, rows);
            g.colsum_part = part_ptr(h, b, l);
            g.loss.enabled = 1; g.loss.data = batch->data; g.loss.row_idx = batch->row_idx; g.loss.mask_id = batch->mask_id;
            g.loss.mask_to_use = batch->mask_to_use; g.loss.nb_run = batch->nb_run; g.loss.run = batch->run;
            g.loss.table = batch->mask_table; g.loss.io = batch->io; g.loss.B = B; g.loss.inv_n = (float)loss_inv_n(hyper, batch);
            g.loss.parts = loss_parts_ptr(h, b);
            if (b->shadow_wt != nullptr && l >= 1 && !h->cfg.no_wt && !h->cfg.no_prefetch) {
                g.prefetch = reinterpret_cast<const bf16_t*>(b->shadow_wt) + h->w_off[l];
                g.prefetch_bytes = (int64_t)h->in[l] * h->out[l] * 2;
            }
            const int n_loss_parts = gemm_bf16_loss_parts(g);
            CODAE_REQUIRE(n_loss_parts <= h->loss_part_cap, "fused loss: %d workgroups exceed the partial-sum rows (%d)", n_loss_parts, h->loss_part_cap);
            {
                ProfScope prof(h, CODAE_K_LOSS, s);
                rc = gemm_bf16(g, s);
            }
            if (rc) return rc;
            h->parts_pending[l] = gemm_bf16_colsum_rows(g);
            h->norm_scalars_zero = true;
            return finish_loss(h, b, batch, n_loss_parts, s);
        }
        rc = last ? run_linear(h, b, l, act_ptr(h, b, l), y, true, B, s)
                  : run_linear(h, b, l, act_ptr(h, b, l), act_ptr(h, b, l + 1), false, rows, s);
        if (rc) return rc;
        fwd_group.launched();
    }
    fwd_group.close();
    if (hyper != nullptr) {
        rc = zero_pad_rows(h, dact_ptr(h, b, L - 1), B, rows, h->out_ld[L - 1], s);
        if (rc) return rc;
        {
            ProfScope prof(h, CODAE_K_LOSS, s);
            rc = launch_mse_loss(batch, y, dact_ptr(h, b, L - 1), bf, (float)loss_inv_n(hyper, batch), part_ptr(h, b, L - 1),
                                 loss_parts_ptr(h, b), 1, s, h->out_ld[L - 1]);
        }
        if (rc) return rc;
        h->parts_pending[L - 1] = mse_loss_colsum_rows(B);
        h->norm_scalars_zero = true;
        return finish_loss(h, b, batch, mse_loss_colsum_rows(B), s);
    }
    rc = launch_mse_loss(batch, y, nullptr, 0, 0.f, nullptr, loss_parts_ptr(h, b), 0, s);
    if (rc) return rc;
    return finish_loss(h, b, batch, mse_loss_colsum_rows(B), s);
}

int codae_set_input_noise(codae_handle h, const codae_noise* noise) {
    CODAE_REQUIRE(h != nullptr, "codae_set_input_noise: null handle");
    int rc = check_noise(noise);
    if (rc) return rc;
    codae_noise n{};
    if (noise != nullptr && noise->kind != CODAE_NOISE_NONE) {
        n.kind = noise->kind; n.p0 = noise->p0; n.seed = noise->seed;
        if (noise->kind == CODAE_NOISE_SALT_PEPPER) { n.p1 = noise->p1; n.p2 = noise->p2; }
    }
    h->noise = n;
    return CODAE_OK;
}

int codae_eval_step(codae_handle h, const codae_buffers* b, const codae_batch* batch, float* out_y, void* stream) {
    return codae_step_forward_loss(h, b, batch, nullptr, out_y, stream);
}

int codae_step_backward(codae_handle h, const codae_buffers* b, int32_t B, int32_t layer_lo, int32_t layer_hi, void* stream) {
    int rc = check_common(h, b, B);
    if (rc) return rc;
    CODAE_REQUIRE(b->grads && b->dacts, "codae_step_backward: grads / dacts missing");
    CODAE_REQUIRE(layer_lo >= 0 && layer_lo < layer_hi && layer_hi <= h->L, "codae_step_backward: layer range [%d, %d)", layer_lo, layer_hi);
    return backward_range(h, b, B, layer_lo, layer_hi, nullptr, true, false, (hipStream_t)stream);
}

int codae_step_backward_async(codae_handle h, const codae_buffers* b, int32_t B, int32_t layer_lo, int32_t layer_hi, void* stream) {
    int rc = check_common(h, b, B);
    if (rc) return rc;
    CODAE_REQUIRE(b->grads && b->dacts, "codae_step_backward_async: grads / dacts missing");
    CODAE_REQUIRE(layer_lo >= 0 && layer_lo < layer_hi && layer_hi <= h->L, "codae_step_backward_async: layer range [%d, %d)", layer_lo, layer_hi);
    return backward_range(h, b, B, layer_lo, layer_hi, nullptr, true, false, (hipStream_t)stream, false);
}

int codae_side_stream(codae_handle h, void** out) {
    CODAE_REQUIRE(h && out, "codae_side_stream: null argument");
    *out = nullptr;
    if (h->cfg.single_stream) return CODAE_OK;
    int rc = ensure_side_stream(h);
    if (rc) return rc;
    *out = h->side;
    return CODAE_OK;
}

static int update_impl(codae_handle h, const codae_buffers* b, const codae_hyper* hyper, hipStream_t s, bool weights_norm_done) {
    CODAE_REQUIRE(h && b && hyper, "codae_step_update: null argument");
    CODAE_REQUIRE(b->params && b->grads && b->adam_m && b->adam_v && b->scalars, "codae_step_update: buffer missing");
    int rc = join_side(h, s);
    if (rc) return rc;
    bool pending = false;
    for (int l = 0; l < h->L; ++l) pending = pending || h->parts_pending[l] > 0;
    if (pending && b->bias_parts != nullptr) {
        rc = finish_bias(h, b, s, false);
        if (rc) return rc;
    }
    const bool scalars_zero = h->norm_scalars_zero;
    h->norm_scalars_zero = false;
    if (hyper->max_grad_norm > 0.f && !weights_norm_done) {
        ProfScope prof(h, CODAE_K_SUMSQ, s);
        if (!scalars_zero) {
            CODAE_HIP_CHECK(hipMemsetAsync(b->scalars + CODAE_S_GRAD_SQ, 0, sizeof(double), s));
            CODAE_HIP_CHECK(hipMemsetAsync(b->scalars + CODAE_S_GRAD_SQ_SLOTS, 0, CODAE_S_N_SLOTS * sizeof(double), s));
        }
        rc = launch_sumsq(b->grads, h->n_param, b->scalars + CODAE_S_GRAD_SQ, s);
        if (rc) return rc;
    }
    bf16_t* shadow = h->prec == CODAE_PREC_BF16 ? reinterpret_cast<bf16_t*>(b->shadow_w) : nullptr;
    CODAE_REQUIRE(h->prec != CODAE_PREC_BF16 || shadow, "codae_step_update: shadow_w missing");
    const double* step_dev = h->capturing ? b->scalars + CODAE_S_ADAM_STEP : nullptr;
    ProfScope prof(h, CODAE_K_ADAM, s);
    if (h->prec == CODAE_PREC_BF16 && b->shadow_wt != nullptr && h->L <= 64 && !h->cfg.flat_adam) {
        return launch_clip_adam_tiled(b->params, b->grads, b->adam_m, b->adam_v, hyper, b->scalars + CODAE_S_GRAD_SQ, shadow,
                                      reinterpret_cast<bf16_t*>(b->shadow_wt), h->L, h->w_off.data(), h->out.data(), h->in.data(),
                                      1, h->bias_begin, h->n_param - h->bias_begin, s, step_dev);
    }
    rc = launch_clip_adam(b->params, b->grads, b->adam_m, b->adam_v, h->n_param, hyper, b->scalars + CODAE_S_GRAD_SQ,
                          shadow, nullptr, s, step_dev);
    if (rc) return rc;
    return refresh_transposed(h, b, s);
}

int codae_step_update(codae_handle h, const codae_buffers* b, const codae_hyper* hyper, void* stream) {
    return update_impl(h, b, hyper, (hipStream_t)stream, false);
}

int codae_span_sumsq(const float* g, int64_t n, double* acc, void* stream) {
    return launch_sumsq_to(g, n, acc, (hipStream_t)stream);
}

int codae_step_update_span(codae_handle h, const codae_buffers* b, const codae_hyper* hyper, int64_t lo, int64_t hi,
                           const double* total_sq, void* stream) {
    CODAE_REQUIRE(h && b && hyper, "codae_step_update_span: null argument");
    CODAE_REQUIRE(b->params && b->grads && b->adam_m && b->adam_v && b->scalars, "codae_step_update_span: buffer missing");
    CODAE_REQUIRE(lo >= 0 && lo < hi && hi <= h->n_param && lo % 4 == 0 && hi % 4 == 0, "codae_step_update_span: range [%lld, %lld)",
                  (long long)lo, (long long)hi);
    CODAE_REQUIRE(hyper->max_grad_norm <= 0.f || total_sq != nullptr, "codae_step_update_span: clipping needs the global sum g^2");
    hipStream_t s = (hipStream_t)stream;
    int rc = join_side(h, s);
    if (rc) return rc;
    h->norm_scalars_zero = false;
    const double* coef = nullptr;
    if (hyper->max_grad_norm > 0.f) {
        rc = launch_clip_coef(total_sq, hyper->max_grad_norm, b->scalars + CODAE_S_CLIP_COEF, s);
        if (rc) return rc;
        coef = b->scalars + CODAE_S_CLIP_COEF;
    }
    bf16_t* shadow = h->prec == CODAE_PREC_BF16 ? reinterpret_cast<bf16_t*>(b->shadow_w) : nullptr;
    CODAE_REQUIRE(h->prec != CODAE_PREC_BF16 || shadow, "codae_step_update_span: shadow_w missing");
    ProfScope prof(h, CODAE_K_ADAM, s);
    return launch_clip_adam(b->params + lo, b->grads + lo, b->adam_m + lo, b->adam_v + lo, hi - lo, hyper, nullptr,
                            shadow ? shadow + lo : nullptr, coef, s);
}

int codae_sync_transposed(codae_handle h, const codae_buffers* b, void* stream) {
    CODAE_REQUIRE(h && b, "codae_sync_transposed: null argument");
    return refresh_transposed(h, b, (hipStream_t)stream);
}

int codae_join(codae_handle h, void* stream) {
    CODAE_REQUIRE(h != nullptr, "codae_join: null handle");
    return join_side(h, (hipStream_t)stream);
}

int codae_step_path(codae_handle h, const codae_buffers* b, int32_t B) {
    return (h != nullptr && b != nullptr && B > 0 && B <= h->max_batch && chain_eligible(h, b, B)) ? 1 : 0;
}

int codae_train_step(codae_handle h, const codae_buffers* b, const codae_batch* batch, const codae_hyper* hyper, void* stream) {
    CODAE_REQUIRE(hyper != nullptr, "codae_train_step: null hyper");
    CODAE_REQUIRE(batch != nullptr, "codae_train_step: null batch");
    if (h != nullptr && b != nullptr && chain_eligible(h, b, batch->B)) {
        int rcc = check_common(h, b, batch->B);
        if (rcc) return rcc;
        CODAE_REQUIRE(batch->io == h->in[0], "batch.io %d does not match the model (%d)", batch->io, h->in[0]);
        CODAE_REQUIRE(b->grads && b->dacts && b->scalars && b->bias_parts, "codae_train_step: grads / dacts / scalars / bias_parts missing");
        CODAE_REQUIRE(batch->data && batch->B > 0 && (!(batch->mask_id || batch->mask_to_use) || batch->mask_table), "codae_train_step: bad batch");
        CODAE_REQUIRE(!batch->mask_to_use || batch->mask_id || (batch->nb_run > 0 && batch->run >= 0 && batch->run < batch->nb_run),
                      "codae_train_step: run %d outside [0, %d)", batch->run, batch->nb_run);
        if (h->prof_on) ++h->prof_step;
        hipStream_t s = (hipStream_t)stream;
        rcc = join_side(h, s);
        if (rcc) return rcc;
        LossFinish lf{};
        rcc = run_chain(h, b, batch, hyper, true, s, &lf);
        if (rcc) return rcc;
        const bool with_norm = hyper->max_grad_norm > 0.f && !h->cfg.no_fused_norm;
        rcc = run_wgrad_grouped(h, b, h->rows_for(batch->B), with_norm, s);
        if (rcc) return rcc;
        rcc = finish_bias(h, b, s, with_norm, &lf);
        if (rcc) return rcc;
        return update_impl(h, b, hyper, s, with_norm);
    }
    int rc = codae_step_forward_loss(h, b, batch, hyper, nullptr, stream);
    if (rc) return rc;
    const bool all_slabbed = h->prec == CODAE_PREC_BF16 && hyper->max_grad_norm > 0.f && !h->cfg.no_fused_norm;
    rc = backward_range(h, b, batch->B, 0, h->L, nullptr, true, all_slabbed, (hipStream_t)stream);
    if (rc) return rc;
    return update_impl(h, b, hyper, (hipStream_t)stream, all_slabbed);
}

static bool same_bytes(const void* a, const void* b, size_t n) { return memcmp(a, b, n) == 0; }

int codae_train_step_graph(codae_handle h, const codae_buffers* b, const codae_batch* batch, const codae_hyper* hyper, void* stream) {
    CODAE_REQUIRE(h && b && batch && hyper, "codae_train_step_graph: null argument");
    CODAE_REQUIRE(!h->prof_on, "codae_train_step_graph: launch profiling (codae_profile_begin) cannot run inside a graph");
    CODAE_REQUIRE(b->scalars != nullptr, "codae_train_step_graph: scalars missing");
    CODAE_REQUIRE(stream != nullptr, "codae_train_step_graph: the default (null) stream cannot be captured - pass a created stream");
    hipStream_t s = (hipStream_t)stream;
    codae_hyper hk = *hyper;
    hk.step = 0;
    const bool fresh = h->graph_exec == nullptr || !same_bytes(&h->graph_key.batch, batch, sizeof(*batch)) ||
                       !same_bytes(&h->graph_key.hyper, &hk, sizeof(hk)) || !same_bytes(&h->graph_key.bufs, b, sizeof(*b)) ||
                       !same_bytes(&h->graph_key.noise, &h->noise, sizeof(h->noise));
    if (fresh) {
        if (h->graph_exec) { (void)hipGraphExecDestroy(h->graph_exec); h->graph_exec = nullptr; }
        int rc = check_common(h, b, batch->B);
        if (rc) return rc;
        if (!h->cfg.single_stream) {
            rc = ensure_side_stream(h);
            if (rc) return rc;
        }
        rc = codae_join(h, stream);
        if (rc) return rc;
        CODAE_HIP_CHECK(hipStreamBeginCapture(s, hipStreamCaptureModeRelaxed));
        h->capturing = true;
        rc = codae_train_step(h, b, batch, hyper, stream);
        h->capturing = false;
        hipGraph_t graph = nullptr;
        const hipError_t ee = hipStreamEndCapture(s, &graph);
        if (rc != CODAE_OK) { if (graph) (void)hipGraphDestroy(graph); return rc; }
        if (ee != hipSuccess || graph == nullptr) {
            set_error("codae_train_step_graph: stream capture failed: %s", hipGetErrorString(ee));
            return CODAE_E_HIP;
        }
        const hipError_t ei = hipGraphInstantiate(&h->graph_exec, graph, nullptr, nullptr, 0);
        (void)hipGraphDestroy(graph);
        if (ei != hipSuccess) {
            h->graph_exec = nullptr;
            set_error("codae_train_step_graph: hipGraphInstantiate failed: %s", hipGetErrorString(ei));
            return CODAE_E_HIP;
        }
        h->graph_key.batch = *batch; h->graph_key.hyper = hk; h->graph_key.bufs = *b; h->graph_key.noise = h->noise;
    }
    int rc = launch_set_scalar(b->scalars + CODAE_S_ADAM_STEP, (double)hyper->step, s);
    if (rc) return rc;
    CODAE_HIP_CHECK(hipGraphLaunch(h->graph_exec, s));
    return CODAE_OK;
}


int codae_dp_unique_id(void* out, int32_t capacity) {
    CODAE_REQUIRE(out != nullptr && capacity >= (int32_t)sizeof(ncclUniqueId), "codae_dp_unique_id: need %d bytes", (int)sizeof(ncclUniqueId));
    int rc = rccl_load();
    if (rc) return rc;
    ncclUniqueId id;
    CODAE_RCCL_CHECK(g_rccl.GetUniqueId(&id));
    memcpy(out, &id, sizeof(id));
    return CODAE_OK;
}

int codae_dp_init(codae_handle h, const void* unique_id, int32_t rank, int32_t world) {
    CODAE_REQUIRE(h != nullptr && unique_id != nullptr && world >= 1 && rank >= 0 && rank < world, "codae_dp_init: bad arguments");
    CODAE_REQUIRE(h->dp == nullptr, "codae_dp_init: this engine already has a communicator");
    int rc = rccl_load();
    if (rc) return rc;
    DpState* d = new DpState();
    d->rank = rank; d->world = world;
    ncclUniqueId id;
    memcpy(&id, unique_id, sizeof(id));
    ncclResult_t r = g_rccl.CommInitRank(&d->comm, world, id, rank);
    if (r != ncclSuccess) { set_error("ncclCommInitRank failed: %s", g_rccl.GetErrorString(r)); delete d; return CODAE_E_HIP; }
    int prio_least = 0, prio_greatest = 0;
    hipError_t e1 = hipDeviceGetStreamPriorityRange(&prio_least, &prio_greatest);
    if (e1 == hipSuccess) e1 = hipStreamCreateWithPriority(&d->stream, hipStreamNonBlocking, prio_greatest);
    for (int i = 0; i <= CODAE_DP_MAX_BUCKETS && e1 == hipSuccess; ++i) e1 = hipEventCreateWithFlags(&d->ev_bucket[i], hipEventDisableTiming);
    if (e1 == hipSuccess) e1 = hipEventCreateWithFlags(&d->ev_done, hipEventDisableTiming);
    if (e1 != hipSuccess) {
        set_error("codae_dp_init: stream / event creation failed: %s", hipGetErrorString(e1));
        (void)g_rccl.CommDestroy(d->comm);
        delete d;
        return CODAE_E_HIP;
    }
    h->dp = d;
    return CODAE_OK;
}

int codae_dp_destroy(codae_handle h) {
    if (h == nullptr || h->dp == nullptr) return CODAE_OK;
    DpState* d = h->dp;
    if (d->stream) (void)hipStreamSynchronize(d->stream);
    if (d->comm) (void)g_rccl.CommDestroy(d->comm);
    for (int i = 0; i <= CODAE_DP_MAX_BUCKETS; ++i) if (d->ev_bucket[i]) (void)hipEventDestroy(d->ev_bucket[i]);
    if (d->ev_done) (void)hipEventDestroy(d->ev_done);
    if (d->stream) (void)hipStreamDestroy(d->stream);
    delete d;
    h->dp = nullptr;
    return CODAE_OK;
}

int codae_train_step_dp(codae_handle h, const codae_buffers* b, const codae_batch* batch, const codae_hyper* hyper, int32_t n_buckets,
                        const int32_t* bucket_lo, const int32_t* bucket_hi, void* stream) {
    CODAE_REQUIRE(h != nullptr && h->dp != nullptr, "codae_train_step_dp: codae_dp_init has not been called on this engine");
    CODAE_REQUIRE(b && batch && hyper && bucket_lo && bucket_hi, "codae_train_step_dp: null argument");
    CODAE_REQUIRE(n_buckets >= 1 && n_buckets <= CODAE_DP_MAX_BUCKETS, "codae_train_step_dp: %d buckets", n_buckets);
    CODAE_REQUIRE(bucket_hi[0] == h->L && bucket_lo[n_buckets - 1] == 0, "codae_train_step_dp: buckets must run from the top layer down to layer 0");
    for (int i = 0; i < n_buckets; ++i) {
        CODAE_REQUIRE(bucket_lo[i] >= 0 && bucket_lo[i] < bucket_hi[i] && (i == 0 || bucket_hi[i] == bucket_lo[i - 1]),
                      "codae_train_step_dp: bucket %d = [%d, %d) does not continue the one above it", i, bucket_lo[i], bucket_hi[i]);
    }
    DpState* d = h->dp;
    hipStream_t s = (hipStream_t)stream;
    int rc = codae_step_forward_loss(h, b, batch, hyper, nullptr, stream);
    if (rc) return rc;
    for (int i = 0; i < n_buckets; ++i) {
        rc = backward_range(h, b, batch->B, bucket_lo[i], bucket_hi[i], nullptr, true, false, s, false);
        if (rc) return rc;
        hipStream_t producer = h->side != nullptr && !h->cfg.single_stream ? h->side : s;
        CODAE_HIP_CHECK(hipEventRecord(d->ev_bucket[i], producer));
        CODAE_HIP_CHECK(hipStreamWaitEvent(d->stream, d->ev_bucket[i], 0));
        const int64_t lo_off = h->w_off[bucket_lo[i]];
        const int64_t hi_off = bucket_hi[i] < h->L ? h->w_off[bucket_hi[i]] : h->bias_begin;
        float* span = b->grads + lo_off;
        CODAE_RCCL_CHECK(g_rccl.AllReduce(span, span, (size_t)(hi_off - lo_off), ncclFloat, ncclSum, d->comm, d->stream));
    }
    rc = join_side(h, s);
    if (rc) return rc;
    CODAE_HIP_CHECK(hipEventRecord(d->ev_bucket[n_buckets], s));
    CODAE_HIP_CHECK(hipStreamWaitEvent(d->stream, d->ev_bucket[n_buckets], 0));
    float* bias = b->grads + h->bias_begin;
    CODAE_RCCL_CHECK(g_rccl.AllReduce(bias, bias, (size_t)(h->n_param - h->bias_begin), ncclFloat, ncclSum, d->comm, d->stream));
    CODAE_HIP_CHECK(hipEventRecord(d->ev_done, d->stream));
    CODAE_HIP_CHECK(hipStreamWaitEvent(s, d->ev_done, 0));
    return update_impl(h, b, hyper, s, false);
}

}
```

### mui-deepautoencoder_amd/csrc/gemm_bf16.hip

```cpp
#include "codae_common.h"

namespace codae {
namespace {

constexpr int BK = 64;

#if defined(CODAE_DBG_5D)
constexpr int DBG5D_WGS = 1024;
__device__ float g_dbg5d[DBG5D_WGS * 256 * 2];
#endif

typedef __attribute__((address_space(3))) char lds_char;
typedef __attribute__((address_space(1))) const void gvoid;

__device__ __forceinline__ void glds16(const void* gsrc, lds_char* dst_wave_base) {
    __builtin_amdgcn_global_load_lds((gvoid*)gsrc, (__attribute__((address_space(3))) void*)dst_wave_base, 16, 0, 0);
}

template <int R>
__device__ __forceinline__ int ks_to_lds_block(int block, int kr) {
    if constexpr (R == 192) {
        const int b = block + ((kr >> 1) & 1) + 2 * ((kr >> 3) & 1);
        return b >= 12 ? b - 12 : b;
    } else if constexpr (R == 64) {
// ... 428 lines not shown
    }
    {
        constexpr int NT = 64 * NW;
        constexpr int HR = BM / 2;
        constexpr int PITCH = BN * 4 + 16;
        static_assert(HR * PITCH <= 2 * BUF_BYTES, "fp32 half tile must fit in the staging buffers");
        static_assert((BM / WM) <= HR, "a wave's rows must lie in one half");
        constexpr int CH = BN / 4, RL = NT / CH;
        float* Cf = reinterpret_cast<float*>(g.C);
        if (g.split_k > 1) Cf += (int64_t)z * g.M * g.ldc;
        const int c = threadIdx.x % CH, rl = threadIdx.x / CH;
        const int j = j0 + c * 4;
        float sq = 0.f;
#pragma unroll
        for (int hh = 0; hh < 2; ++hh) {
            if (((BM / WM) * wr) / HR == hh) {
#pragma unroll
                for (int nt = 0; nt < TN; ++nt) {
                    const int jl = (BN / WN) * wc + 16 * nt + g4;
                    const float4 bj = load_bias4(g.bias, g.A, j0 + jl, g.N);
#pragma unroll
                    for (int mt = 0; mt < TM; ++mt) {
                        const int il = (BM / WM) * wr + 16 * mt + li - hh * HR;
                        f32x4 v = acc[mt][nt];
                        v[0] += bj.x; v[1] += bj.y; v[2] += bj.z; v[3] += bj.w;
                        if (!ACT && g.relu) {
                            v[0] = clamp_below(v[0], 0.f); v[1] = clamp_below(v[1], 0.f); v[2] = clamp_below(v[2], 0.f); v[3] = clamp_below(v[3], 0.f);
                        }
                        *reinterpret_cast<__attribute__((address_space(3))) f32x4*>(smem + il * PITCH + jl * 4) = v;
                    }
                }
            }
            __syncthreads();
            if (rl < RL && j < g.N) {
                for (int r = rl; r < HR; r += RL) {
                    const int i = i0 + hh * HR + r;
                    if (i >= g.M) break;
                    f32x4 v = *reinterpret_cast<const __attribute__((address_space(3))) f32x4*>(smem + r * PITCH + c * 16);
                    if constexpr (ACT) {
                        v[0] = act_fwd(g.act, g.act_p, v[0]); v[1] = act_fwd(g.act, g.act_p, v[1]);
                        v[2] = act_fwd(g.act, g.act_p, v[2]); v[3] = act_fwd(g.act, g.act_p, v[3]);
                    }
                    *reinterpret_cast<float4*>(Cf + (int64_t)i * g.ldc + j) = make_float4(v[0], v[1], v[2], v[3]);
                    sq += v[0] * v[0] + v[1] * v[1] + v[2] * v[2] + v[3] * v[3];
                }
            }
            __syncthreads();
        }
        if (g.sumsq_slots != nullptr) {
#pragma unroll
            for (int o = 32; o > 0; o >>= 1) sq += __shfl_xor(sq, o);
            float* red = reinterpret_cast<float*>(smem_raw);
            if (lane == 0) red[w] = sq;
            __syncthreads();
            if (threadIdx.x == 0) {
                float t = 0.f;
                for (int ww = 0; ww < NW; ++ww) t += red[ww];
                atomicAdd(g.sumsq_slots + (blockIdx.x & (CODAE_S_N_SLOTS - 1)), (double)t);
            }
        }
    }
}

template <int BM, int BN, int WM, int WN, int A_MODE, int B_MODE, bool C_F32, bool LOSS = false, int NS = 2, bool ACT = false>
__global__ __launch_bounds__(64 * WM * WN, (64 * WM * WN) / 256 * ((NS * (BM + BN) * 128 <= 80 * 1024) ? 2 : 1))
void gemm_bf16_kernel(GemmBf16 g, int tiles_n, int tiles_mn, int kt_total) {
    __shared__ __attribute__((aligned(16))) char smem_raw[NS * (BM + BN) * 128 + (LOSS ? BM * 8 : 0)];
    gemm_bf16_tile<BM, BN, WM, WN, A_MODE, B_MODE, C_F32, LOSS, NS, ACT>(g, tiles_n, tiles_mn, kt_total, blockIdx.x, gridDim.x, smem_raw);
}

template <int BM, int BN>
__global__ __launch_bounds__(256, 2) void gemm_bf16_grouped_kernel(GemmBf16Group grp) {
    __shared__ __attribute__((aligned(16))) char smem_raw[2 * (BM + BN) * 128];
    int j = 0;
    while (j + 1 < grp.n && (int)blockIdx.x >= grp.wg_begin[j + 1]) ++j;
    const GemmBf16& g = grp.g[j];
    const int tiles_m = (g.M + BM - 1) / BM, tiles_n = (g.N + BN - 1) / BN;
    gemm_bf16_tile<BM, BN, 2, 2, OP_KS, OP_KS, true, false>(g, tiles_n, tiles_m * tiles_n, g.K / BK, blockIdx.x - grp.wg_begin[j],
                                                            grp.wg_begin[j + 1] - grp.wg_begin[j], smem_raw);
}

template <int BM, int BN, int WM, int WN>
int launch_cfg(const GemmBf16& g, hipStream_t s) {
    const int tiles_m = (g.M + BM - 1) / BM, tiles_n = (g.N + BN - 1) / BN;
    const int kt_total = g.K / BK;
    const int64_t nwg = (int64_t)tiles_m * tiles_n * g.split_k;
    CODAE_REQUIRE(nwg < (1 << 30), "gemm_bf16: grid too large");
    dim3 grid((unsigned)nwg), block(64 * WM * WN);
    if (g.act != CODAE_ACT_NONE) {
#define LAUNCH_ACT(BMODE, CF, NS) \
    hipLaunchKernelGGL((gemm_bf16_kernel<BM, BN, WM, WN, OP_KC, BMODE, CF, false, NS, true>), grid, block, 0, s, g, tiles_n, tiles_m * tiles_n, kt_total)
        const bool deep = !g.c_f32 && nwg <= 256 && kt_total >= 6 && !env().no_deep_small && env().small_stages >= 4;
        if (g.b_mode == OP_KC) {
            if (g.c_f32) LAUNCH_ACT(OP_KC, true, 2);
            else if (deep) LAUNCH_ACT(OP_KC, false, 4);
            else LAUNCH_ACT(OP_KC, false, 2);
        } else {
            LAUNCH_ACT(OP_KS, false, 2);
        }
#undef LAUNCH_ACT
        CODAE_LAUNCH_CHECK();
        return CODAE_OK;
    }
#define LAUNCH(AM, BMODE, CF) \
    hipLaunchKernelGGL((gemm_bf16_kernel<BM, BN, WM, WN, AM, BMODE, CF>), grid, block, 0, s, g, tiles_n, tiles_m * tiles_n, kt_total)
    if (g.loss.enabled) {
        hipLaunchKernelGGL((gemm_bf16_kernel<BM, BN, WM, WN, OP_KC, OP_KC, false, true>), grid, block, 0, s, g, tiles_n,
                           tiles_m * tiles_n, kt_total);
    } else if (g.a_mode == OP_KC && g.b_mode == OP_KC) {
        const bool deep = !g.c_f32 && nwg <= 256 && kt_total >= 6 && !env().no_deep_small && env().small_stages >= 4;
        if (g.c_f32) LAUNCH(OP_KC, OP_KC, true);
        else if (deep)
            hipLaunchKernelGGL((gemm_bf16_kernel<BM, BN, WM, WN, OP_KC, OP_KC, false, false, 4>), grid, block, 0, s, g, tiles_n,
                               tiles_m * tiles_n, kt_total);
        else LAUNCH(OP_KC, OP_KC, false);
    }
    else if (g.a_mode == OP_KC && g.b_mode == OP_KS) { if (g.c_f32) LAUNCH(OP_KC, OP_KS, true); else LAUNCH(OP_KC, OP_KS, false); }
    else if (g.a_mode == OP_KS && g.b_mode == OP_KS) { if (g.c_f32) LAUNCH(OP_KS, OP_KS, true); else LAUNCH(OP_KS, OP_KS, false); }
    else { set_error("gemm_bf16: operand mode combination not built"); return CODAE_E_UNSUPPORTED; }
#undef LAUNCH
    CODAE_LAUNCH_CHECK();
    return CODAE_OK;
}

}

int gemm_bf16_grouped(GemmBf16Group& grp, hipStream_t s) {
    CODAE_REQUIRE(grp.n >= 1 && grp.n <= CODAE_GROUP_MAX, "gemm_bf16_grouped: %d GEMMs", grp.n);
    auto count = [&](int bm, int bn) {
        int total = 0;
        for (int j = 0; j < grp.n; ++j) {
            const GemmBf16& g = grp.g[j];
            grp.wg_begin[j] = total;
            total += ((g.M + bm - 1) / bm) * ((g.N + bn - 1) / bn) * g.split_k;
        }
        grp.wg_begin[grp.n] = total;
        return total;
    };
    for (int j = 0; j < grp.n; ++j) {
        const GemmBf16& g = grp.g[j];
        CODAE_REQUIRE(g.a_mode == OP_KS && g.b_mode == OP_KS && g.c_f32 && g.split_k >= 1 && g.K % BK == 0 && g.K >= BK && g.M % 8 == 0 &&
                          g.N % 8 == 0 && !g.loss.enabled && g.relu_src == nullptr && g.colsum_part == nullptr && g.bias == nullptr,
                      "gemm_bf16_grouped: GEMM %d is not a plain weight-gradient form", j);
    }
    int tile = env().group_tile;
    if (tile < 0) tile = count(128, 128) >= 256 ? 0 : (count(64, 128) >= 256 ? 1 : 2);
    if (tile == 0) { const int total = count(128, 128); hipLaunchKernelGGL((gemm_bf16_grouped_kernel<128, 128>), dim3(total), dim3(256), 0, s, grp); }
    else if (tile == 1) { const int total = count(64, 128); hipLaunchKernelGGL((gemm_bf16_grouped_kernel<64, 128>), dim3(total), dim3(256), 0, s, grp); }
    else { const int total = count(64, 64); hipLaunchKernelGGL((gemm_bf16_grouped_kernel<64, 64>), dim3(total), dim3(256), 0, s, grp); }
    CODAE_LAUNCH_CHECK();
    return CODAE_OK;
}

bool gemm_bf16_supported(int M, int N, int K) {
    return M > 0 && N >= 8 && K >= BK && (K % BK) == 0 && (N % 8) == 0;
}

int gemm_bf16_tile_big(int M, int N, int split_k, bool k_strided = false) {
    if (env().gemm_tile >= 0) return env().gemm_tile;
    const int64_t big = (int64_t)((M + 255) / 256) * ((N + 191) / 192) * split_k;
    (void)k_strided;
    if (big < 160) return 0;
    return 6;
}

static bool small_tile_64(const GemmBf16& g) {
    if (env().no_deep_small || g.c_f32 || g.a_mode != OP_KC || g.b_mode != OP_KC || g.split_k != 1) return false;
    return (int64_t)((g.M + 127) / 128) * ((g.N + 127) / 128) <= env().small_tile_max;
}

static int bf16_path(const GemmBf16& g) {
    const int t = gemm_bf16_tile_big(g.M, g.N, g.split_k, g.b_mode == OP_KS || g.c_f32);
    switch (t) {
        case 3: return 1;
        case 6: return 6;
        case 7: return 7;
        default:
            if (small_tile_64(g)) return -64;
            if (g.a_mode == OP_KC && g.b_mode == OP_KC && !g.c_f32 && g.split_k == 1 && !env().no_deep_small) return 7;
            return -128;
    }
}

bool gemm_bf16_takes_relu_bits(int M, int N) {
    if (env().gemm_dbg) return false;
    GemmBf16 probe{};
    probe.M = M; probe.N = N; probe.a_mode = OP_KC; probe.b_mode = OP_KC; probe.c_f32 = 0; probe.split_k = 1;
    return bf16_path(probe) > 0;
}

int gemm_bf16_colsum_rows(const GemmBf16& g) {
    const int t = gemm_bf16_tile_big(g.M, g.N, g.loss.enabled ? 1 : g.split_k, g.b_mode == OP_KS || g.c_f32);
    const int bm = (t && g.act == CODAE_ACT_NONE) ? 256 : (small_tile_64(g) ? 64 : 128);
    return (g.M + bm - 1) / bm;
}

int gemm_bf16_loss_parts(const GemmBf16& g) {
    const int t = gemm_bf16_tile_big(g.M, g.N, 1);
    const int sm = small_tile_64(g) ? 64 : 128;
    const int bm = t ? 256 : sm, bn = t ? 192 : sm;
    return ((g.M + bm - 1) / bm) * ((g.N + bn - 1) / bn);
}

int gemm_bf16(const GemmBf16& g, hipStream_t s) {
    CODAE_REQUIRE(gemm_bf16_supported(g.M, g.N, g.K), "gemm_bf16: unsupported shape M=%d N=%d K=%d (need K %% 64 == 0, N %% 8 == 0)",
                  g.M, g.N, g.K);
    CODAE_REQUIRE(g.a_mode == OP_KC || g.M % 8 == 0, "gemm_bf16: k-strided A needs M %% 8 == 0");
    CODAE_REQUIRE(g.a_mode == OP_KC || g.M >= 8, "gemm_bf16: k-strided A needs M >= 8");
    CODAE_REQUIRE((g.lda % 8) == 0 && (g.ldb % 8) == 0 && (g.ldc % 4) == 0, "gemm_bf16: leading dimensions must keep 16-byte rows");
    CODAE_REQUIRE(g.split_k >= 1 && (g.split_k == 1 || g.c_f32), "gemm_bf16: split-K needs fp32 output slabs");
    CODAE_REQUIRE((reinterpret_cast<uintptr_t>(g.A) & 15) == 0 && (reinterpret_cast<uintptr_t>(g.B) & 15) == 0 &&
                      (reinterpret_cast<uintptr_t>(g.C) & 15) == 0,
                  "gemm_bf16: operands must be 16-byte aligned");
    CODAE_REQUIRE(g.split_k <= g.K / BK, "gemm_bf16: split_k %d > k tiles %d", g.split_k, g.K / BK);
    CODAE_REQUIRE(!g.c_f32 || (g.relu_src == nullptr && g.colsum_part == nullptr), "gemm_bf16: ReLU mask / column sums need bf16 output");
    if (g.act != CODAE_ACT_NONE) {
        CODAE_REQUIRE(!g.loss.enabled && g.a_mode == OP_KC && g.split_k == 1 && g.relu_bits == nullptr && g.relu_bits_out == nullptr &&
                          !(g.c_f32 && g.b_mode == OP_KS) && g.dbg == 0,
                      "gemm_bf16: an activation needs the forward / data-gradient form (k-contiguous A, unsplit, no 1-bit masks, "
                      "no fused loss, k-strided B only with bf16 output)");
    }
    if (g.loss.enabled) {
        CODAE_REQUIRE(g.a_mode == OP_KC && g.b_mode == OP_KC && !g.c_f32 && g.split_k == 1 && !g.relu && !g.relu_src,
                      "gemm_bf16: fused loss only on the plain forward form");
        CODAE_REQUIRE(g.loss.data && g.loss.parts && g.loss.io == g.N && g.loss.B <= g.M && (g.N % 8) == 0,
                      "gemm_bf16: fused loss arguments");
        CODAE_REQUIRE(!(g.loss.mask_id || g.loss.mask_to_use) || ((reinterpret_cast<uintptr_t>(g.loss.table) & 7) == 0),
                      "gemm_bf16: mask table must be 8-byte aligned");
        CODAE_REQUIRE((reinterpret_cast<uintptr_t>(g.loss.data) & 15) == 0, "gemm_bf16: dataset must be 16-byte aligned");
    }
    if (env().gemm_dbg && g.act == CODAE_ACT_NONE) { GemmBf16 g2 = g; g2.dbg = env().gemm_dbg; return gemm_bf16_pipe(g2, 0, s); }
    if (g.loss.enabled) {
        const int t = gemm_bf16_tile_big(g.M, g.N, 1);
        if (t) return gemm_bf16_pipe(g, t >= 6 ? 6 : 1, s);
        if (small_tile_64(g)) return launch_cfg<64, 64, 2, 2>(g, s);
        return launch_cfg<128, 128, 2, 2>(g, s);
    }
    if (g.act != CODAE_ACT_NONE) return small_tile_64(g) ? launch_cfg<64, 64, 2, 2>(g, s) : launch_cfg<128, 128, 2, 2>(g, s);
    const int path = bf16_path(g);
    if (path > 0) return gemm_bf16_pipe(g, path, s);
    if (path == -64) return launch_cfg<64, 64, 2, 2>(g, s);
    return launch_cfg<128, 128, 2, 2>(g, s);
}

#if defined(CODAE_DBG_5D) && (CODAE_DBG_5D & 2)
}
extern "C" int codae_debug_5d(float* host_out, int n_floats) {
    if (hipMemcpyFromSymbol(host_out, HIP_SYMBOL(codae::g_dbg5d), (size_t)n_floats * sizeof(float)) != hipSuccess) return -1;
    return 0;
}
namespace codae {
#endif
}
```

### mui-deepautoencoder_amd/csrc/gemm_bf16_pipe.hip

```cpp
#include "codae_common.h"
#include <type_traits>

namespace codae {
namespace {

#include "gemm_bf16_halftile.h"

constexpr int TIMELINE_WGS = 4096, TIMELINE_SLOTS = 6;
__device__ unsigned long long g_timeline[TIMELINE_WGS * TIMELINE_SLOTS];

template <int BM, int BN, int WM, int WN, int NLB, int A_MODE, int B_MODE, bool C_F32, int DBG = 0, int EPI = 0>
__device__ __forceinline__ void gemm_bf16_pipe_tile(const GemmBf16& g, int tiles_n, int tiles_mn, int kt_total, int wg, int nwg,
                                                    char* smem_raw) {
    constexpr int NW = WM * WN;
    constexpr int SM = BM / WM, SN = BN / WN;
    constexpr int AHR = BM / 2, BHR = BN / 2;
    constexpr int TMH = SM / 32, TNH = SN / 32;
    constexpr int AH = AHR * 128, BH = BHR * 128;
    constexpr int BUF = 2 * AH + 2 * BH;
    constexpr int NLA = (NLB == 4 && NW == 8) ? 4 : (((AHR / 8) % NW == 0) ? NW : 8);
    constexpr int NA = AHR / 8 / NLA, NB = BHR / 8 / NLB;
    static_assert(NLB <= NW && NLA <= NW && (AHR / 8) % NLA == 0 && (BHR / 8) % NLB == 0, "loader waves");
    static_assert(SM % 32 == 0 && SN % 32 == 0, "wave sub-tile must split into 16-wide half tiles");
    lds_char* smem = (lds_char*)smem_raw;

    const int lane = threadIdx.x & 63;
    const int w = __builtin_amdgcn_readfirstlane(threadIdx.x >> 6);
    const int wr = w / WN, wc = w % WN;

    int bid = wg;
    if (nwg > 0) {
        const int q = nwg >> 3, r = nwg & 7, xcd = bid & 7;
        bid = (xcd < r ? xcd * (q + 1) : r * (q + 1) + (xcd - r) * q) + (bid >> 3);
    }
    const int z = bid / tiles_mn;
    const int tmn = bid - z * tiles_mn;
    constexpr int TILE_GROUP_M = 4;
    const int tiles_m = tiles_mn / tiles_n;
    const int grp = tmn / (TILE_GROUP_M * tiles_n);
    const int tm0 = grp * TILE_GROUP_M;
    const int gsz = tiles_m - tm0 < TILE_GROUP_M ? tiles_m - tm0 : TILE_GROUP_M;
    const int within = tmn - grp * (TILE_GROUP_M * tiles_n);
    const int tn = within / gsz, tm = tm0 + (within - tn * gsz);
    const int i0 = tm * BM, j0 = tn * BN;
    const int kt_begin = (int)((int64_t)kt_total * z / g.split_k);
    const int kt_end = (int)((int64_t)kt_total * (z + 1) / g.split_k);
    const int nkt = kt_end - kt_begin;

    auto a_img = [&](int tile, int h) { return smem + (tile & 1) * BUF + h * AH; };
    auto b_img = [&](int tile, int h) { return smem + (tile & 1) * BUF + 2 * AH + h * BH; };
    constexpr bool dbg_noload = DBG & 1, dbg_nomma = DBG & 2, dbg_nostore = DBG & 4, dbg_time = DBG & 8;
    constexpr bool dbg_no_a = DBG & 16, dbg_no_b = DBG & 32;
    auto stamp = [&](int slot) {
        if constexpr (dbg_time) {
            if (threadIdx.x == 0 && blockIdx.x < TIMELINE_WGS) g_timeline[blockIdx.x * TIMELINE_SLOTS + slot] = wall_clock64();
        }
    };
    stamp(0);
    if constexpr (dbg_time) {
        if (threadIdx.x == 0 && blockIdx.x < TIMELINE_WGS) {
            unsigned xcc;
            asm volatile("s_getreg_b32 %0, hwreg(HW_REG_XCC_ID)" : "=s"(xcc));
            g_timeline[blockIdx.x * TIMELINE_SLOTS + 5] = xcc & 0xf;
        }
    }
    if constexpr (EPI == 3) {
        const LossFuse& L = g.loss;
        int* rowinfo = reinterpret_cast<int*>(smem_raw + 2 * BUF);
        for (int r = threadIdx.x; r < BM; r += 64 * NW) {
            const int i = i0 + r;
            int src = -1, id = 0;
            if (i < L.B && i < g.M) {
                src = L.row_idx ? L.row_idx[i] : i;
                if (L.mask_id != nullptr) id = L.mask_id[i];
                else if (L.mask_to_use != nullptr) id = L.mask_to_use[(int64_t)src * L.nb_run + L.run];
            }
            rowinfo[2 * r] = src; rowinfo[2 * r + 1] = id;
        }
    }

    f32x4 acc[2][TMH][2][TNH];
#pragma unroll
    for (int a = 0; a < 2; ++a)
#pragma unroll
        for (int b = 0; b < TMH; ++b)
#pragma unroll
            for (int c = 0; c < 2; ++c)
#pragma unroll
                for (int d = 0; d < TNH; ++d) acc[a][b][c][d] = (f32x4){0.f, 0.f, 0.f, 0.f};

    auto k_loop = [&](auto al_tag, auto bl_tag) {
    constexpr bool a_loader = decltype(al_tag)::value, b_loader = decltype(bl_tag)::value;
    uint32_t a_src[2][NA], b_src[2][NB];
#pragma unroll
    for (int h = 0; h < 2; ++h) {
#pragma unroll
        for (int it = 0; it < NA; ++it) a_src[h][it] = half_src<A_MODE, AHR, SM, NLA>(g.lda, i0, g.M, h, it, a_loader ? w : 0, lane);
#pragma unroll
        for (int it = 0; it < NB; ++it) b_src[h][it] = half_src<B_MODE, BHR, SN, NLB>(g.ldb, j0, g.N, h, it, b_loader ? w : 0, lane);
    }
    const int64_t a_step = (A_MODE == OP_KC ? BK : (int64_t)BK * g.lda) * 2;
    const int64_t b_step = (B_MODE == OP_KC ? BK : (int64_t)BK * g.ldb) * 2;
    const char* a_base = reinterpret_cast<const char*>(g.A) + kt_begin * a_step;
    const char* b_base = reinterpret_cast<const char*>(g.B) + kt_begin * b_step;
    auto issue_a = [&](int tile, int h) {
        if constexpr (!dbg_noload && !dbg_no_a && a_loader) {
            const char* base = a_base + (int64_t)(tile < nkt ? tile : nkt - 1) * a_step;
            lds_char* img = a_img(tile, h);
#pragma unroll
            for (int it = 0; it < NA; ++it) glds16(base + a_src[h][it], img + (it * NLA + w) * 1024);
        }
    };
    auto issue_b = [&](int tile, int h) {
        if constexpr (!dbg_noload && !dbg_no_b && b_loader) {
            const char* base = b_base + (int64_t)(tile < nkt ? tile : nkt - 1) * b_step;
            lds_char* img = b_img(tile, h);
#pragma unroll
            for (int it = 0; it < NB; ++it) glds16(base + b_src[h][it], img + (it * NLB + w) * 1024);
        }
    };

    bf16x8 a0x[TMH][2], a0y[TMH][2], a1[TMH][2], b0[TNH][2], b1[TNH][2];

    auto read_a = [&](bf16x8 (&dst)[TMH][2], int tile, int h) {
#pragma unroll
        for (int mt = 0; mt < TMH; ++mt) dst[mt][0] = read_frag<A_MODE, AHR, 0>(a_img(tile, h), wr * TMH + mt, lane);
#pragma unroll
        for (int mt = 0; mt < TMH; ++mt) dst[mt][1] = read_frag<A_MODE, AHR, 1>(a_img(tile, h), wr * TMH + mt, lane);
    };
    auto read_b = [&](bf16x8 (&dst)[TNH][2], int tile, int h) {
#pragma unroll
        for (int nt = 0; nt < TNH; ++nt) dst[nt][0] = read_frag<B_MODE, BHR, 0>(b_img(tile, h), wc * TNH + nt, lane);
#pragma unroll
        for (int nt = 0; nt < TNH; ++nt) dst[nt][1] = read_frag<B_MODE, BHR, 1>(b_img(tile, h), wc * TNH + nt, lane);
    };
    auto mma = [&](const bf16x8 (&a)[TMH][2], const bf16x8 (&b)[TNH][2], int mh, int nh) {
        if constexpr (dbg_nomma) {
#pragma unroll
            for (int s = 0; s < 2; ++s) {
#pragma unroll
                for (int mt = 0; mt < TMH; ++mt) asm volatile("" ::"v"(a[mt][s]));
#pragma unroll
                for (int nt = 0; nt < TNH; ++nt) asm volatile("" ::"v"(b[nt][s]));
            }
            return;
        }
#pragma unroll
        for (int s = 0; s < 2; ++s)
#pragma unroll
            for (int mt = 0; mt < TMH; ++mt)
#pragma unroll
                for (int nt = 0; nt < TNH; ++nt)
                    acc[mh][mt][nh][nt] = __builtin_amdgcn_mfma_f32_16x16x32_bf16(b[nt][s], a[mt][s], acc[mh][mt][nh][nt], 0, 0, 0);
    };
    auto wait_dma = [&](auto ca, auto cb) {
        constexpr int CA = decltype(ca)::value, CB = decltype(cb)::value;
        constexpr int N = (a_loader ? CA * NA : 0) + (b_loader ? CB * NB : 0);
        if constexpr (a_loader || b_loader) wait_vmcnt<N>();
    };
    auto wait_for_a = [&]() { wait_dma(std::integral_constant<int, 2>{}, std::integral_constant<int, 3>{}); };
    auto wait_for_b = [&]() { wait_dma(std::integral_constant<int, 3>{}, std::integral_constant<int, 2>{}); };

    issue_a(0, 0); issue_b(0, 0); issue_a(0, 1); issue_b(0, 1);
    issue_a(1, 0); issue_b(1, 0); issue_a(1, 1); issue_b(1, 1);
// ... 41 lines not shown
        if constexpr (A_MODE == OP_KS) settle(a1);
        issue_b(t + 2, 0);
        read_b(b1, t, 1);
        mma(a1, b0, 1, 0);
        phase_order(RB{}, DB{});
        wait_for_a();
        phase_barrier<KEEP_B, PINP>();
        if constexpr (B_MODE == OP_KS) settle(b1);
        issue_a(t + 2, 1);
        read_a(a0n, t + 1, 0);
        mma(a1, b1, 1, 1);
        phase_order(RA{}, DA{});
        wait_for_b();
        phase_barrier<KEEP_A, PINP>();
        issue_b(t + 2, 1);
        read_b(b0, t + 1, 0);
        mma(a0, b1, 0, 1);
        phase_order(RB{}, DB{});
    };
    int t = 0;
    for (; t + 1 < nkt; t += 2) {
        ktile(t, a0x, a0y);
        ktile(t + 1, a0y, a0x);
    }
    if (t < nkt) ktile(t, a0x, a0y);
    if constexpr (A_MODE == OP_KS || B_MODE == OP_KS) {
        asm volatile("s_waitcnt lgkmcnt(0)" ::: "memory");
        if constexpr (A_MODE == OP_KS) { settle(a0x); settle(a0y); }
        if constexpr (B_MODE == OP_KS) settle(b0);
    }
    };
    {
        const bool al = (NLA == NW) || (w < NLA), bl = (NLB == NW) || (w < NLB);
        if constexpr (NLA == NW && NLB == NW) k_loop(std::true_type{}, std::true_type{});
        else if constexpr (NLA == NW) { if (bl) k_loop(std::true_type{}, std::true_type{}); else k_loop(std::true_type{}, std::false_type{}); }
        else {
            if (al && bl) k_loop(std::true_type{}, std::true_type{});
            else if (al) k_loop(std::true_type{}, std::false_type{});
            else if (bl) k_loop(std::false_type{}, std::true_type{});
            else k_loop(std::false_type{}, std::false_type{});
        }
    }
    wait_vmcnt<0>();
    stamp(2);

    const int li = lane & 15, g4 = (lane >> 4) * 4;
    uint32_t pf_val = 0;
    if (g.prefetch != nullptr) {
        const int64_t lines = (g.prefetch_bytes + 127) >> 7;
        const int64_t per_wg = (lines + nwg - 1) / nwg;
        for (int64_t i = threadIdx.x; i < per_wg; i += 64 * NW) {
            const int64_t mine = (int64_t)wg * per_wg + i;
            if (mine < lines) pf_val ^= *reinterpret_cast<const uint32_t*>(reinterpret_cast<const char*>(g.prefetch) + (mine << 7));
        }
    }
    auto consume_prefetch = [&]() { asm volatile("" ::"v"(pf_val)); };
    phase_barrier();
    if constexpr (EPI == 3) {
        const LossFuse& L = g.loss;
        const int* rowinfo = reinterpret_cast<const int*>(smem_raw + 2 * BUF);
        const bool masked = (L.mask_id != nullptr) || (L.mask_to_use != nullptr);
        const uint8_t* tb = masked ? L.table : reinterpret_cast<const uint8_t*>(L.data);
        constexpr int NT = 64 * NW;
        constexpr int PITCH = BN * 2 + 16;
        static_assert(BM * PITCH <= 2 * BUF, "output tile must fit in the staging buffers");
        float sq = 0.f, sqp = 0.f;
        float cs[2][TNH][4];
        int jcl[2][TNH];
        bool jok[2][TNH];
#pragma unroll
        for (int nh = 0; nh < 2; ++nh)
#pragma unroll
            for (int nt = 0; nt < TNH; ++nt) {
                const int j = j0 + nh * BHR + wc * (SN / 2) + 16 * nt + g4;
                jok[nh][nt] = j < g.N;
                jcl[nh][nt] = jok[nh][nt] ? j : 0;
                const float4 bj = load_bias4(g.bias, g.A, j, g.N);
#pragma unroll
                for (int mh = 0; mh < 2; ++mh)
#pragma unroll
                    for (int mt = 0; mt < TMH; ++mt) {
                        acc[mh][mt][nh][nt][0] += bj.x; acc[mh][mt][nh][nt][1] += bj.y;
                        acc[mh][mt][nh][nt][2] += bj.z; acc[mh][mt][nh][nt][3] += bj.w;
                    }
#pragma unroll
                for (int k = 0; k < 4; ++k) cs[nh][nt][k] = 0.f;
            }
        const int jbase = j0 + wc * (SN / 2) + g4;
        auto loss_rows = [&](auto full_tag) {
            constexpr bool FULL = decltype(full_tag)::value;
#pragma unroll
            for (int mh = 0; mh < 2; ++mh) {
                float4 xv[TMH][2][TNH];
                uint32_t mk[TMH][2][TNH];
                bool live[TMH];
#pragma unroll
                for (int mt = 0; mt < TMH; ++mt) {
                    const int il = mh * AHR + wr * (SM / 2) + 16 * mt + li;
                    const int src = rowinfo[2 * il], id = rowinfo[2 * il + 1];
                    live[mt] = src >= 0;
                    const float* xrow = L.data + (int64_t)(src >= 0 ? src : 0) * L.io;
                    const uint8_t* mrow = tb + (int64_t)id * L.io;
#pragma unroll
                    for (int nh = 0; nh < 2; ++nh)
#pragma unroll
                        for (int nt = 0; nt < TNH; ++nt) {
                            const int off = FULL ? jbase + (nh * BHR + 16 * nt) : jcl[nh][nt];
                            xv[mt][nh][nt] = *reinterpret_cast<const float4*>(xrow + off);
                            const uint32_t mv = *reinterpret_cast<const uint32_t*>(mrow + off);
                            mk[mt][nh][nt] = masked ? mv : 0x01010101u;
                        }
                }
#pragma unroll
                for (int mt = 0; mt < TMH; ++mt) {
                    const int il = mh * AHR + wr * (SM / 2) + 16 * mt + li;
#pragma unroll
                    for (int nh = 0; nh < 2; ++nh)
#pragma unroll
                        for (int nt = 0; nt < TNH; ++nt) {
                            const int jl = nh * BHR + wc * (SN / 2) + 16 * nt + g4;
                            const f32x4 a = acc[mh][mt][nh][nt];
                            const float4 x = xv[mt][nh][nt];
                            const float yv[4] = {a[0], a[1], a[2], a[3]};
                            const float xs[4] = {x.x, x.y, x.z, x.w};
                            const bool on = live[mt] && (FULL || jok[nh][nt]);
                            float gq[4];
#pragma unroll
                            for (int k = 0; k < 4; ++k) {
                                const float d = on ? xs[k] - yv[k] : 0.f;
                                const float se = d * d;
                                sq += se;
                                asm volatile("" : "+v"(sq));
                                sqp += ((mk[mt][nh][nt] >> (8 * k)) & 0xffu) == 0 ? se : 0.f;
                                gq[k] = on ? -2.f * d * L.inv_n : 0.f;
                                cs[nh][nt][k] += gq[k];
                            }
                            u32x2 o;
                            o[0] = pack_bf16x2(gq[0], gq[1]);
                            o[1] = pack_bf16x2(gq[2], gq[3]);
                            *reinterpret_cast<__attribute__((address_space(3))) u32x2*>(smem + il * PITCH + jl * 2) = o;
                        }
                }
                __builtin_amdgcn_sched_barrier(0);
            }
        };
        if (j0 + BN <= g.N) loss_rows(std::true_type{}); else loss_rows(std::false_type{});
        stamp(3);
        phase_barrier();
        {
            constexpr int CH = BN / 8, RL = NT / CH;
            const int c = threadIdx.x % CH, rl = threadIdx.x / CH;
            const int j = j0 + c * 8;
            bf16_t* Cb = reinterpret_cast<bf16_t*>(g.C);
            constexpr int ITER = (BM + RL - 1) / RL;
#pragma unroll
            for (int it = 0; it < ITER; ++it) {
                const int r = rl + it * RL;
                const bool ok = rl < RL && j < g.N && r < BM && i0 + r < g.M;
                const u32x4 lv = *reinterpret_cast<const __attribute__((address_space(3))) u32x4*>(smem + (ok ? r : 0) * PITCH + c * 16);
                if (ok) *reinterpret_cast<uint4*>(Cb + (int64_t)(i0 + r) * g.ldc + j) = make_uint4(lv[0], lv[1], lv[2], lv[3]);
            }
        }
        if constexpr (dbg_time) { wait_vmcnt<0>(); stamp(4); }
#pragma unroll
        for (int o2 = 32; o2 > 0; o2 >>= 1) { sq += __shfl_xor(sq, o2); sqp += __shfl_xor(sqp, o2); }
#pragma unroll
        for (int nh = 0; nh < 2; ++nh)
#pragma unroll
            for (int nt = 0; nt < TNH; ++nt)
#pragma unroll
                for (int k = 0; k < 4; ++k) {
                    float v = cs[nh][nt][k];
                    v += __shfl_xor(v, 1); v += __shfl_xor(v, 2); v += __shfl_xor(v, 4); v += __shfl_xor(v, 8);
                    cs[nh][nt][k] = v;
                }
        phase_barrier();
        float* red = reinterpret_cast<float*>(smem_raw);
        static_assert((WM * BN + 2 * NW) * 4 <= 2 * BUF, "reduction scratch must fit");
        if (li == 0) {
#pragma unroll
            for (int nh = 0; nh < 2; ++nh)
#pragma unroll
                for (int nt = 0; nt < TNH; ++nt) {
                    const int jl = nh * BHR + wc * (SN / 2) + 16 * nt + g4;
#pragma unroll
                    for (int k = 0; k < 4; ++k) red[wr * BN + jl + k] = cs[nh][nt][k];
                }
        }
        float* wsum = red + WM * BN;
        if (lane == 0) { wsum[2 * w] = sq; wsum[2 * w + 1] = sqp; }
        phase_barrier();
        if (threadIdx.x == 0) {
            float a = 0.f, b2 = 0.f;
            for (int ww = 0; ww < NW; ++ww) { a += wsum[2 * ww]; b2 += wsum[2 * ww + 1]; }
            L.parts[2 * bid] = (double)a;
            L.parts[2 * bid + 1] = masked ? (double)b2 : 0.0;
        }
        if (g.colsum_part != nullptr) {
            for (int col = threadIdx.x; col < BN; col += NT) {
                float sum = 0.f;
#pragma unroll
                for (int r = 0; r < WM; ++r) sum += red[r * BN + col];
                if (j0 + col < g.N) g.colsum_part[(int64_t)tm * g.N + j0 + col] = sum;
            }
        }
        consume_prefetch();
        return;
    }
    if constexpr (!C_F32 && !dbg_nostore) {
        constexpr int NT = 64 * NW;
        constexpr int PITCH = BN * 2 + 16;
        static_assert(BM * PITCH <= 2 * BUF, "output tile must fit in the staging buffers");
        const float floor_v = g.relu ? 0.f : -__builtin_inff();
        constexpr int CH = BN / 8, RL = NT / CH;
        constexpr int ITER = (BM + RL - 1) / RL;
        const int c = threadIdx.x % CH, rl = threadIdx.x / CH;
        const int j = j0 + c * 8;
        const int jc = j < g.N ? j : 0;
        const bool bit_mask = EPI != 1 && g.relu_bits != nullptr;
        uint8_t hb[ITER];
        if constexpr (EPI != 1) {
            const uint8_t* bsrc = bit_mask ? g.relu_bits : reinterpret_cast<const uint8_t*>(g.A);
            const int64_t bld = bit_mask ? g.ld_bits : 0;
            if (bit_mask) {
#pragma unroll
                for (int it = 0; it < ITER; ++it) {
                    const int r = rl + it * RL;
                    const bool ok = rl < RL && j < g.N && r < BM && i0 + r < g.M;
                    hb[it] = bsrc[(int64_t)(ok ? i0 + r : 0) * bld + (ok ? (jc >> 3) : 0)];
                }
            }
        }
#pragma unroll
        for (int nh = 0; nh < 2; ++nh)
#pragma unroll
            for (int nt = 0; nt < TNH; ++nt) {
                const int jl = nh * BHR + wc * (SN / 2) + 16 * nt + g4;
                const float4 bj = load_bias4(g.bias, g.A, j0 + jl, g.N);
#pragma unroll
                for (int mh = 0; mh < 2; ++mh)
#pragma unroll
                    for (int mt = 0; mt < TMH; ++mt) {
                        const int il = mh * AHR + wr * (SM / 2) + 16 * mt + li;
                        const f32x4 a = acc[mh][mt][nh][nt];
                        const float v0 = clamp_below(a[0] + bj.x, floor_v), v1 = clamp_below(a[1] + bj.y, floor_v);
                        const float v2 = clamp_below(a[2] + bj.z, floor_v), v3 = clamp_below(a[3] + bj.w, floor_v);
                        u32x2 o;
                        o[0] = pack_bf16x2(v0, v1);
                        o[1] = pack_bf16x2(v2, v3);
                        *reinterpret_cast<__attribute__((address_space(3))) u32x2*>(smem + il * PITCH + jl * 2) = o;
                    }
            }
        __syncthreads();
        float cs[8] = {0.f, 0.f, 0.f, 0.f, 0.f, 0.f, 0.f, 0.f};
        {
            bf16_t* Cb = reinterpret_cast<bf16_t*>(g.C);
            const bool relu_mask = EPI != 1 && !bit_mask && g.relu_src != nullptr;
            const bf16_t* hsrc = relu_mask ? g.relu_src : g.A;
            const int64_t hld = relu_mask ? g.ld_relu : 0;
            uint4 hv[ITER];
            if constexpr (EPI != 1) {
                if (!bit_mask) {
#pragma unroll
                    for (int it = 0; it < ITER; ++it) {
                        const int r = rl + it * RL;
                        const bool ok = rl < RL && j < g.N && r < BM && i0 + r < g.M;
                        hv[it] = *reinterpret_cast<const uint4*>(hsrc + (int64_t)(ok ? i0 + r : 0) * hld + (relu_mask ? jc : 0));
                    }
                }
            }
#pragma unroll
            for (int it = 0; it < ITER; ++it) {
                const int r = rl + it * RL;
                const bool ok = rl < RL && j < g.N && r < BM && i0 + r < g.M;
                const u32x4 lv = *reinterpret_cast<const __attribute__((address_space(3))) u32x4*>(smem + (ok ? r : 0) * PITCH + c * 16);
                uint4 v = make_uint4(lv[0], lv[1], lv[2], lv[3]);
                if constexpr (EPI != 1) {
                    if (bit_mask) {
                        const uint32_t hbv = hb[it];
                        auto keepb = [](uint32_t val, uint32_t b2) -> uint32_t {
                            return val & (((b2 & 1u) ? 0x0000ffffu : 0u) | ((b2 & 2u) ? 0xffff0000u : 0u));
                        };
                        v.x = keepb(v.x, hbv); v.y = keepb(v.y, hbv >> 2); v.z = keepb(v.z, hbv >> 4); v.w = keepb(v.w, hbv >> 6);
                    } else if (relu_mask) {
                        const uint4 h = hv[it];
                        auto keep = [](uint32_t val, uint32_t hh) -> uint32_t {
                            const uint32_t lo = ((hh & 0x8000u) == 0 && (hh & 0x7fffu) != 0) ? 0x0000ffffu : 0u;
                            const uint32_t hi = ((hh & 0x80000000u) == 0 && (hh & 0x7fff0000u) != 0) ? 0xffff0000u : 0u;
                            return val & (lo | hi);
                        };
                        v.x = keep(v.x, h.x); v.y = keep(v.y, h.y); v.z = keep(v.z, h.z); v.w = keep(v.w, h.w);
                    }
                }
                if constexpr (EPI == 1) {
                    if (g.relu_bits_out != nullptr) {
                        auto pos = [](uint32_t w2) -> uint32_t {
                            const uint32_t t = (w2 & 0x7fff7fffu) + 0x7fff7fffu;
                            return ((t >> 15) & 1u) | ((t >> 30) & 2u);
                        };
                        const uint32_t b0 = ok ? (pos(v.x) | (pos(v.y) << 2) | (pos(v.z) << 4) | (pos(v.w) << 6)) : 0u;
                        const uint32_t b1 = (uint32_t)__builtin_amdgcn_update_dpp(0, (int)b0, 0x39, 0xf, 0xf, true);
                        const uint32_t b2 = (uint32_t)__builtin_amdgcn_update_dpp(0, (int)b0, 0x4e, 0xf, 0xf, true);
                        const uint32_t b3 = (uint32_t)__builtin_amdgcn_update_dpp(0, (int)b0, 0x93, 0xf, 0xf, true);
                        if (ok && (c & 3) == 0)
                            *reinterpret_cast<uint32_t*>(g.relu_bits_out + (int64_t)(i0 + r) * g.ld_bits + (j >> 3)) = b0 | (b1 << 8) | (b2 << 16) | (b3 << 24);
                    }
                }
                if (ok) {
                    *reinterpret_cast<uint4*>(Cb + (int64_t)(i0 + r) * g.ldc + j) = v;
                    if (EPI != 1 && g.colsum_part != nullptr) {
                        cs[0] += bf16_to_f32((bf16_t)(v.x & 0xffff)); cs[1] += bf16_to_f32((bf16_t)(v.x >> 16));
                        cs[2] += bf16_to_f32((bf16_t)(v.y & 0xffff)); cs[3] += bf16_to_f32((bf16_t)(v.y >> 16));
                        cs[4] += bf16_to_f32((bf16_t)(v.z & 0xffff)); cs[5] += bf16_to_f32((bf16_t)(v.z >> 16));
                        cs[6] += bf16_to_f32((bf16_t)(v.w & 0xffff)); cs[7] += bf16_to_f32((bf16_t)(v.w >> 16));
                    }
                }
            }
        }
        stamp(3);
        if constexpr (dbg_time) { wait_vmcnt<0>(); stamp(4); }
        if (EPI != 1 && g.colsum_part != nullptr) {
            __syncthreads();
            float* red = reinterpret_cast<float*>(smem_raw);
            static_assert(RL * BN * 4 <= 2 * BUF, "reduction scratch must fit");
            if (rl < RL) {
#pragma unroll
                for (int k = 0; k < 8; ++k) red[rl * BN + c * 8 + k] = cs[k];
            }
            __syncthreads();
            for (int col = threadIdx.x; col < BN; col += NT) {
                float sum = 0.f;
                for (int r = 0; r < RL; ++r) sum += red[r * BN + col];
                if (j0 + col < g.N) g.colsum_part[(int64_t)tm * g.N + j0 + col] = sum;
            }
        }
        consume_prefetch();
        return;
    }
    if constexpr (C_F32) {
        constexpr int NT = 64 * NW;
        constexpr int HR = AHR;
        constexpr int PITCH = BN * 4 + 16;
        static_assert(HR * PITCH <= 2 * BUF, "fp32 half tile must fit in the staging buffers");
        constexpr int CH = BN / 4, RL = NT / CH;
        float* Cf = reinterpret_cast<float*>(g.C);
        if (g.split_k > 1) Cf += (int64_t)z * g.M * g.ldc;
        const float floor_v = g.relu ? 0.f : -__builtin_inff();
        const int c = threadIdx.x % CH, rl = threadIdx.x / CH;
        const int j = j0 + c * 4;
        float sq = 0.f;
#pragma unroll
        for (int hh = 0; hh < 2; ++hh) {
#pragma unroll
            for (int nh = 0; nh < 2; ++nh)
#pragma unroll
                for (int nt = 0; nt < TNH; ++nt) {
                    const int jl = nh * BHR + wc * (SN / 2) + 16 * nt + g4;
                    const float4 bj = load_bias4(g.bias, g.A, j0 + jl, g.N);
#pragma unroll
                    for (int mt = 0; mt < TMH; ++mt) {
                        const int il = wr * (SM / 2) + 16 * mt + li;
                        const f32x4 a = acc[hh][mt][nh][nt];
                        f32x4 v;
                        v[0] = clamp_below(a[0] + bj.x, floor_v); v[1] = clamp_below(a[1] + bj.y, floor_v);
                        v[2] = clamp_below(a[2] + bj.z, floor_v); v[3] = clamp_below(a[3] + bj.w, floor_v);
                        *reinterpret_cast<__attribute__((address_space(3))) f32x4*>(smem + il * PITCH + jl * 4) = v;
                    }
                }
            __syncthreads();
            constexpr int ITER = (HR + RL - 1) / RL;
#pragma unroll
            for (int it = 0; it < ITER; ++it) {
                const int r = rl + it * RL;
                const bool ok = rl < RL && j < g.N && r < HR && i0 + hh * HR + r < g.M;
                const f32x4 v = *reinterpret_cast<const __attribute__((address_space(3))) f32x4*>(smem + (ok ? r : 0) * PITCH + c * 16);
                if (ok) {
                    *reinterpret_cast<float4*>(Cf + (int64_t)(i0 + hh * HR + r) * g.ldc + j) = make_float4(v[0], v[1], v[2], v[3]);
                    sq += v[0] * v[0] + v[1] * v[1] + v[2] * v[2] + v[3] * v[3];
                }
            }
            __syncthreads();
        }
        if (g.sumsq_slots != nullptr) {
#pragma unroll
            for (int o = 32; o > 0; o >>= 1) sq += __shfl_xor(sq, o);
            float* red = reinterpret_cast<float*>(smem_raw);
            if (lane == 0) red[w] = sq;
            __syncthreads();
            if (threadIdx.x == 0) {
                float t = 0.f;
                for (int ww = 0; ww < NW; ++ww) t += red[ww];
                atomicAdd(g.sumsq_slots + (wg & (CODAE_S_N_SLOTS - 1)), (double)t);
            }
        }
    }
}

template <int BM, int BN, int WM, int WN, int NLB, int A_MODE, int B_MODE, bool C_F32, int DBG = 0, int EPI = 0>
__global__ __launch_bounds__(64 * WM * WN, (WM * WN + 3) / 4)
void gemm_bf16_pipe_kernel(GemmBf16 g, int tiles_n, int tiles_mn, int kt_total) {
    __shared__ __attribute__((aligned(16))) char smem_raw[2 * (BM + BN) * 128 + (EPI == 3 ? BM * 8 : 0)];
    gemm_bf16_pipe_tile<BM, BN, WM, WN, NLB, A_MODE, B_MODE, C_F32, DBG, EPI>(g, tiles_n, tiles_mn, kt_total, blockIdx.x, gridDim.x, smem_raw);
}

__global__ __launch_bounds__(512, 2) void gemm_bf16_pipe_grouped_kernel(GemmBf16Group grp) {
    constexpr int BM = 256, BN = 192;
    __shared__ __attribute__((aligned(16))) char smem_raw[2 * (BM + BN) * 128];
    const int total = grp.wg_begin[grp.n];
    int t = (int)blockIdx.x;
    {
        const int q = total >> 3, r = total & 7, xcd = t & 7;
        t = (xcd < r ? xcd * (q + 1) : r * (q + 1) + (xcd - r) * q) + (t >> 3);
    }
    int j = 0;
    while (j + 1 < grp.n && t >= grp.wg_begin[j + 1]) ++j;
    const GemmBf16& g = grp.g[j];
    const int tiles_m = (g.M + BM - 1) / BM, tiles_n = (g.N + BN - 1) / BN;
    gemm_bf16_pipe_tile<BM, BN, 4, 2, 4, OP_KS, OP_KS, true, 0, 0>(g, tiles_n, tiles_m * tiles_n, g.K / BK, t - grp.wg_begin[j], 0, smem_raw);
}

template <int BM, int BN, int WM, int WN, int NLB>
int launch_pipe(const GemmBf16& g, hipStream_t s) {
    const int tiles_m = (g.M + BM - 1) / BM, tiles_n = (g.N + BN - 1) / BN;
    const int kt_total = g.K / BK;
    const int64_t nwg = (int64_t)tiles_m * tiles_n * g.split_k;
    CODAE_REQUIRE(nwg < (1 << 30), "gemm_bf16: grid too large");
    CODAE_REQUIRE((int64_t)(g.a_mode == OP_KC ? g.M : g.K) * g.lda * 2 < (int64_t)1 << 32 &&
                      (int64_t)(g.b_mode == OP_KC ? g.N : g.K) * g.ldb * 2 < (int64_t)1 << 32,
                  "gemm_bf16: operand larger than 4 GiB");
    dim3 grid((unsigned)nwg), block(64 * WM * WN);
#define LAUNCH(AM, BMODE, CF, EP) \
    hipLaunchKernelGGL((gemm_bf16_pipe_kernel<BM, BN, WM, WN, NLB, AM, BMODE, CF, 0, EP>), grid, block, 0, s, g, tiles_n, tiles_m * tiles_n, kt_total)
#define LAUNCH_BF16(AM, BMODE) do { if (bwd_epi) LAUNCH(AM, BMODE, false, 2); else LAUNCH(AM, BMODE, false, 1); } while (0)
    const bool bwd_epi = g.relu_src != nullptr || g.colsum_part != nullptr;
    if (g.coscheduled && bwd_epi && !g.loss.enabled && g.a_mode == OP_KC && g.b_mode == OP_KC && !g.c_f32) {
        hipLaunchKernelGGL((gemm_bf16_pipe_kernel<BM, BN, WM, WN, NLB, OP_KC, OP_KC, false, 64, 2>), grid, block, 0, s, g, tiles_n, tiles_m * tiles_n, kt_total);
        CODAE_LAUNCH_CHECK();
        return CODAE_OK;
    }
    if (g.loss.enabled) {
        if constexpr (WM * WN == 8) LAUNCH(OP_KC, OP_KC, false, 3);
        else { set_error("gemm_bf16: fused loss is built for the 8-wave pipelined tile only"); return CODAE_E_UNSUPPORTED; }
    } else if (g.a_mode == OP_KC && g.b_mode == OP_KC) { if (g.c_f32) LAUNCH(OP_KC, OP_KC, true, 0); else LAUNCH_BF16(OP_KC, OP_KC); }
    else if (g.a_mode == OP_KC && g.b_mode == OP_KS) { if (g.c_f32) LAUNCH(OP_KC, OP_KS, true, 0); else LAUNCH_BF16(OP_KC, OP_KS); }
    else if (g.a_mode == OP_KS && g.b_mode == OP_KS) { if (g.c_f32) LAUNCH(OP_KS, OP_KS, true, 0); else LAUNCH_BF16(OP_KS, OP_KS); }
    else { set_error("gemm_bf16: operand mode combination not built"); return CODAE_E_UNSUPPORTED; }
#undef LAUNCH_BF16
#undef LAUNCH
    CODAE_LAUNCH_CHECK();
    return CODAE_OK;
}

}

template <int DBG>
int launch_dbg(const GemmBf16& g, hipStream_t s) {
    constexpr int BM = 256, BN = 192;
    const int tiles_m = (g.M + BM - 1) / BM, tiles_n = (g.N + BN - 1) / BN;
    hipLaunchKernelGGL((gemm_bf16_pipe_kernel<BM, BN, 4, 2, 4, OP_KC, OP_KC, false, DBG>), dim3(tiles_m * tiles_n), dim3(512), 0, s, g,
                       tiles_n, tiles_m * tiles_n, g.K / BK);
    CODAE_LAUNCH_CHECK();
    return CODAE_OK;
}

int launch_pipe_mid(const GemmBf16& g, hipStream_t s) {
    constexpr int BM = 128, BN = 192;
    const int tiles_m = (g.M + BM - 1) / BM, tiles_n = (g.N + BN - 1) / BN;
    CODAE_REQUIRE(g.a_mode == OP_KC && g.b_mode == OP_KC && !g.c_f32 && !g.loss.enabled && g.split_k == 1, "gemm_bf16: 128 x 192 tile is forward-form only");
    CODAE_REQUIRE((int64_t)g.M * g.lda * 2 < (int64_t)1 << 32 && (int64_t)g.N * g.ldb * 2 < (int64_t)1 << 32, "gemm_bf16: operand larger than 4 GiB");
    dim3 grid((unsigned)(tiles_m * tiles_n)), block(512);
    if (g.relu_src != nullptr || g.colsum_part != nullptr)
        hipLaunchKernelGGL((gemm_bf16_pipe_kernel<BM, BN, 4, 2, 4, OP_KC, OP_KC, false, 0, 2>), grid, block, 0, s, g, tiles_n, tiles_m * tiles_n, g.K / BK);
    else
        hipLaunchKernelGGL((gemm_bf16_pipe_kernel<BM, BN, 4, 2, 4, OP_KC, OP_KC, false, 0, 1>), grid, block, 0, s, g, tiles_n, tiles_m * tiles_n, g.K / BK);
    CODAE_LAUNCH_CHECK();
    return CODAE_OK;
}

int gemm_bf16_pipe_grouped(GemmBf16Group& grp, hipStream_t s) {
    CODAE_REQUIRE(grp.n >= 1 && grp.n <= CODAE_GROUP_MAX, "gemm_bf16_pipe_grouped: %d GEMMs", grp.n);
    int total = 0;
    for (int j = 0; j < grp.n; ++j) {
        const GemmBf16& g = grp.g[j];
        CODAE_REQUIRE(g.a_mode == OP_KS && g.b_mode == OP_KS && g.c_f32 && g.split_k == 1 && g.K % BK == 0 && g.K >= BK && g.M % 8 == 0 &&
                          g.N % 8 == 0 && g.M >= 8 && g.N >= 8 && !g.loss.enabled && g.relu_src == nullptr && g.colsum_part == nullptr &&
                          g.bias == nullptr && !g.relu && (g.lda % 8) == 0 && (g.ldb % 8) == 0 && (g.ldc % 4) == 0,
                      "gemm_bf16_pipe_grouped: GEMM %d is not a plain unsplit weight-gradient form", j);
        CODAE_REQUIRE((int64_t)g.K * g.lda * 2 < (int64_t)1 << 32 && (int64_t)g.K * g.ldb * 2 < (int64_t)1 << 32,
                      "gemm_bf16_pipe_grouped: operand larger than 4 GiB");
        CODAE_REQUIRE((reinterpret_cast<uintptr_t>(g.A) & 15) == 0 && (reinterpret_cast<uintptr_t>(g.B) & 15) == 0 &&
                          (reinterpret_cast<uintptr_t>(g.C) & 15) == 0, "gemm_bf16_pipe_grouped: operands must be 16-byte aligned");
        grp.wg_begin[j] = total;
        total += ((g.M + 255) / 256) * ((g.N + 191) / 192);
    }
    grp.wg_begin[grp.n] = total;
    hipLaunchKernelGGL(gemm_bf16_pipe_grouped_kernel, dim3(total), dim3(512), 0, s, grp);
    CODAE_LAUNCH_CHECK();
    return CODAE_OK;
}

int gemm_bf16_pipe(const GemmBf16& g, int cfg, hipStream_t s) {
    if (cfg == 7) return launch_pipe_mid(g, s);
    if (g.dbg == 8 && g.loss.enabled) {
        const int tiles_m = (g.M + 255) / 256, tiles_n = (g.N + 191) / 192;
        hipLaunchKernelGGL((gemm_bf16_pipe_kernel<256, 192, 4, 2, 6, OP_KC, OP_KC, false, 8, 3>), dim3(tiles_m * tiles_n), dim3(512), 0, s, g,
                           tiles_n, tiles_m * tiles_n, g.K / BK);
        CODAE_LAUNCH_CHECK();
        return CODAE_OK;
    }
    if (g.dbg && !g.loss.enabled && g.a_mode == OP_KC && g.b_mode == OP_KC && !g.c_f32 && g.split_k == 1) {
        switch (g.dbg) {
            case 1: return launch_dbg<1>(g, s);
            case 2: return launch_dbg<2>(g, s);
            case 3: return launch_dbg<3>(g, s);
            case 4: return launch_dbg<4>(g, s);
            case 5: return launch_dbg<5>(g, s);
            case 6: return launch_dbg<6>(g, s);
            case 7: return launch_dbg<7>(g, s);
            case 8: return launch_dbg<8>(g, s);
            case 9: return launch_dbg<9>(g, s);
            case 10: return launch_dbg<10>(g, s);
            case 16: return launch_dbg<16>(g, s);
            case 32: return launch_dbg<32>(g, s);
            default: break;
        }
    }
    if (cfg == 6) return launch_pipe<256, 192, 4, 2, 4>(g, s);
    return launch_pipe<256, 192, 4, 2, 6>(g, s);
}

int gemm_bf16_timeline(unsigned long long* host_out, int n_wg) {
    CODAE_REQUIRE(host_out && n_wg > 0 && n_wg <= TIMELINE_WGS, "timeline: bad args");
    CODAE_HIP_CHECK(hipMemcpyFromSymbol(host_out, HIP_SYMBOL(g_timeline), (size_t)n_wg * TIMELINE_SLOTS * sizeof(unsigned long long)));
    return CODAE_OK;
}

}
```

### mui-deepautoencoder_amd/csrc/layer_gemm.h

```cpp
#pragma once
#include "codae_common.h"

namespace codae {

inline GemmBf16 fwd_gemm_bf16(const void* x, int64_t ldx, const void* W, int64_t ldw, void* y, int64_t ldy, int y_f32,
                              int rows, int n_out, int k, const float* bias) {
    GemmBf16 g{};
    g.A = reinterpret_cast<const bf16_t*>(x); g.lda = ldx; g.a_mode = OP_KC;
    g.B = reinterpret_cast<const bf16_t*>(W); g.ldb = ldw; g.b_mode = OP_KC;
    g.C = y; g.ldc = ldy; g.c_f32 = y_f32;
    g.M = rows; g.N = n_out; g.K = k;
    g.bias = bias; g.split_k = 1;
    return g;
}

inline GemmBf16 dgrad_gemm_bf16(const void* dy, int64_t lddy, const void* W, int64_t ldw, bool w_transposed, void* dx, int64_t lddx,
                                int dx_f32, int rows, int n_in, int k) {
    GemmBf16 g{};
    g.A = reinterpret_cast<const bf16_t*>(dy); g.lda = lddy; g.a_mode = OP_KC;
    g.B = reinterpret_cast<const bf16_t*>(W); g.ldb = ldw; g.b_mode = w_transposed ? OP_KC : OP_KS;
    g.C = dx; g.ldc = lddx; g.c_f32 = dx_f32;
    g.M = rows; g.N = n_in; g.K = k;
    g.split_k = 1;
    return g;
}

inline GemmBf16 wgrad_gemm_bf16(const void* dy, int64_t lddy, const void* x, int64_t ldx, void* dW, int rows, int n_out, int n_in) {
    GemmBf16 g{};
    g.A = reinterpret_cast<const bf16_t*>(dy); g.lda = lddy; g.a_mode = OP_KS;
    g.B = reinterpret_cast<const bf16_t*>(x); g.ldb = ldx; g.b_mode = OP_KS;
    g.C = dW; g.ldc = n_in; g.c_f32 = 1;
    g.M = n_out; g.N = n_in; g.K = rows;
    g.split_k = 1;
    return g;
}

inline GemmF32 fwd_gemm_f32(const float* x, const float* W, float* y, int rows, int n_out, int n_in, const float* bias) {
    GemmF32 g{};
    g.A = x; g.a_rs = n_in; g.a_ks = 1;
    g.B = W; g.b_rs = n_in; g.b_ks = 1;
    g.C = y; g.ldc = n_out;
    g.M = rows; g.N = n_out; g.K = n_in;
    g.bias = bias; g.split_k = 1;
    return g;
}

inline GemmF32 dgrad_gemm_f32(const float* dy, const float* W, float* dx, int rows, int n_out, int n_in) {
    GemmF32 g{};
    g.A = dy; g.a_rs = n_out; g.a_ks = 1;
    g.B = W; g.b_rs = 1; g.b_ks = n_in;
    g.C = dx; g.ldc = n_in;
    g.M = rows; g.N = n_in; g.K = n_out;
    g.split_k = 1;
    return g;
}

inline GemmF32 wgrad_gemm_f32(const float* dy, const float* x, float* dW, int rows, int n_out, int n_in) {
    GemmF32 g{};
    g.A = dy; g.a_rs = 1; g.a_ks = n_out;
    g.B = x; g.b_rs = 1; g.b_ks = n_in;
    g.C = dW; g.ldc = n_in;
    g.M = n_out; g.N = n_in; g.K = rows;
    g.split_k = 1;
    return g;
}

template <typename G>
inline void set_activation(G& g, int relu, int act, const float* p) {
    g.relu = relu;
    g.act = act;
    for (int k = 0; k < 3; ++k) g.act_p[k] = p != nullptr ? p[k] : 0.f;
}

}
```

Measured before the change: 6.862 million samples/s.

## Add write-through buffer stores for GEMM outputs and fold loss finish into backward

Adds a store-policy template so GEMM epilogues can write tiles through raw buffer stores carrying a cache-policy flag, chosen by output size (at most 32 MiB uses the write-through path). Forward, dgrad, wgrad and grouped wgrad launches all pick this policy, with environment overrides. It also folds the loss-finish step into the backward bias finish and zeroes the norm scalars inside the gather kernel, removing a separate finish launch and scalar reset. The cache-policy effect on MI355X is uncertain and could slow down intermediates that are read again soon.

```diff
diff --git a/mui-deepautoencoder_amd/csrc/codae_common.h b/mui-deepautoencoder_amd/csrc/codae_common.h
--- a/mui-deepautoencoder_amd/csrc/codae_common.h
+++ b/mui-deepautoencoder_amd/csrc/codae_common.h
@@ -147,6 +147,21 @@
 }
 
 static inline int64_t round_up(int64_t x, int64_t m) { return (x + m - 1) / m * m; }
+
+enum { STORE_PLAIN = 0, STORE_WT = 1 };
+int store_policy_for(int64_t out_bytes);
+
+template <int POL>
+struct TileStore {
+    __amdgpu_buffer_rsrc_t rsrc;
+    __device__ __forceinline__ explicit TileStore(void* tile_base) {
+        if constexpr (POL != STORE_PLAIN) rsrc = __builtin_amdgcn_make_buffer_rsrc(tile_base, 0, 0x7fffffff, 0x00020000);
+    }
+    __device__ __forceinline__ void store16(void* p, uint32_t byte_off, u32x4 v) const {
+        if constexpr (POL == STORE_PLAIN) *reinterpret_cast<u32x4*>(p) = v;
+        else __builtin_amdgcn_raw_buffer_store_b128(v, rsrc, (int)byte_off, 0, 16);
+    }
+};
 
 struct EnvToggles {
     int gemm_tile = -1;
@@ -162,6 +177,8 @@
          no_relu_bits = false,
          no_prefetch = false,
          no_defer_wgrad = false;
+    bool no_folded_loss_finish = false;
+    int store_policy = -1;
 };
 const EnvToggles& env();
 void env_reload();
@@ -229,6 +246,7 @@
     double* sumsq_slots;
     int act;
     float act_p[3];
+    int store_policy;
 };
 bool gemm_bf16_supported(int M, int N, int K);
 bool gemm_bf16_takes_relu_bits(int M, int N);
@@ -270,10 +288,10 @@
 int chain_rows_per_workgroup();
 int launch_chain_step(const ChainArgs& a, hipStream_t s);
 
-int launch_gather_corrupt(const codae_batch* b, void* out, int out_bf16, hipStream_t s, int64_t out_ld = 0);
+int launch_gather_corrupt(const codae_batch* b, void* out, int out_bf16, hipStream_t s, int64_t out_ld = 0, double* zero_norm = nullptr);
 int check_noise(const codae_noise* noise);
 int launch_gather_noise(const codae_batch* b, const codae_noise* noise, int32_t step, const double* step_dev, void* out,
-                        int out_bf16, hipStream_t s, int64_t out_ld = 0, const int32_t* noise_rows = nullptr);
+                        int out_bf16, hipStream_t s, int64_t out_ld = 0, const int32_t* noise_rows = nullptr, double* zero_norm = nullptr);
 int launch_noise_box_muller(const uint32_t* ra, const uint32_t* rb, float* rho, float* c, float* sn, int64_t n, hipStream_t s);
 int launch_cast_bf16(const float* src, bf16_t* dst, int64_t n, hipStream_t s);
 int launch_corrupt(const float* x, const float* mask, float* out, int64_t n, hipStream_t s);
diff --git a/mui-deepautoencoder_amd/csrc/elementwise.hip b/mui-deepautoencoder_amd/csrc/elementwise.hip
--- a/mui-deepautoencoder_amd/csrc/elementwise.hip
+++ b/mui-deepautoencoder_amd/csrc/elementwise.hip
@@ -36,13 +36,21 @@
     return o;
 }
 
+__device__ __forceinline__ void zero_norm_scalars(double* zero_norm) {
+    if (zero_norm != nullptr && blockIdx.x == 0) {
+        if (threadIdx.x == 0) zero_norm[CODAE_S_GRAD_SQ] = 0.0;
+        if (threadIdx.x < CODAE_S_N_SLOTS) zero_norm[CODAE_S_GRAD_SQ_SLOTS + threadIdx.x] = 0.0;
+    }
+}
+
 __global__ __launch_bounds__(NT) void gather_corrupt_bf16x8_kernel(const float* __restrict__ data,
                                                                    const int32_t* __restrict__ row_idx,
                                                                    const int32_t* __restrict__ mask_id,
                                                                    const uint8_t* __restrict__ table, int B, int io,
                                                                    bf16_t* __restrict__ out,
                                                                    const int32_t* __restrict__ mask_to_use, int nb_run,
-                                                                   int run, int64_t out_ld) {
+                                                                   int run, int64_t out_ld, double* zero_norm) {
+    zero_norm_scalars(zero_norm);
     const bool masked = (mask_id != nullptr) || (mask_to_use != nullptr);
     const int cols = io / 8;
     const int64_t total = (int64_t)B * cols;
@@ -74,7 +82,8 @@
                                                             const uint8_t* __restrict__ table, int B, int io,
                                                             void* __restrict__ out,
                                                             const int32_t* __restrict__ mask_to_use, int nb_run,
-                                                            int run, int64_t out_ld) {
+                                                            int run, int64_t out_ld, double* zero_norm) {
+    zero_norm_scalars(zero_norm);
     constexpr int W = VEC ? 4 : 1;
     const bool masked = (mask_id != nullptr) || (mask_to_use != nullptr);
     const int cols = io / W;
@@ -121,6 +130,7 @@
     const int32_t* rows;
     uint64_t thresh;
     float p0, p1, p2;
+    double* zero_norm;
 };
 
 __device__ __forceinline__ uint4 philox4x32_10(uint32_t c0, uint32_t c1, uint32_t c2, uint32_t c3, uint32_t k0, uint32_t k1) {
@@ -180,6 +190,7 @@
                                                                  int B, int io, bf16_t* __restrict__ out,
                                                                  const int32_t* __restrict__ mask_to_use, int nb_run, int run,
                                                                  int64_t out_ld, NoiseArgs na) {
+    zero_norm_scalars(na.zero_norm);
     const bool masked = (mask_id != nullptr) || (mask_to_use != nullptr);
     const uint32_t step = na.step_dev ? (uint32_t)*na.step_dev : na.step;
     const int cols = io / 8;
@@ -213,6 +224,7 @@
                                                           const int32_t* __restrict__ mask_id, const uint8_t* __restrict__ table, int B,
                                                           int io, void* __restrict__ out, const int32_t* __restrict__ mask_to_use,
                                                           int nb_run, int run, int64_t out_ld, NoiseArgs na) {
+    zero_norm_scalars(na.zero_norm);
     constexpr int W = VEC ? 4 : 1;
     const bool masked = (mask_id != nullptr) || (mask_to_use != nullptr);
     const uint32_t step = na.step_dev ? (uint32_t)*na.step_dev : na.step;
@@ -737,7 +749,7 @@
 
 }
 
-int launch_gather_corrupt(const codae_batch* b, void* out, int out_bf16, hipStream_t s, int64_t out_ld) {
+int launch_gather_corrupt(const codae_batch* b, void* out, int out_bf16, hipStream_t s, int64_t out_ld, double* zero_norm) {
     if (out_ld <= 0) out_ld = b ? b->io : 0;
     CODAE_REQUIRE(b && b->data && out && b->B > 0 && b->io > 0, "gather_corrupt: bad batch");
     const bool masked = b->mask_id || b->mask_to_use;
@@ -749,12 +761,12 @@
     const int grid = grid_for(items);
     if (vec && out_bf16 && b->io % 8 == 0 && (!masked || (reinterpret_cast<uintptr_t>(b->mask_table) & 7) == 0)) {
         hipLaunchKernelGGL(gather_corrupt_bf16x8_kernel, dim3(grid_for(items / 2)), dim3(NT), 0, s, b->data, b->row_idx, b->mask_id,
-                           b->mask_table, b->B, b->io, reinterpret_cast<bf16_t*>(out), b->mask_to_use, b->nb_run, b->run, out_ld);
+                           b->mask_table, b->B, b->io, reinterpret_cast<bf16_t*>(out), b->mask_to_use, b->nb_run, b->run, out_ld, zero_norm);
         CODAE_LAUNCH_CHECK();
         return CODAE_OK;
     }
 #define GC(V, O) hipLaunchKernelGGL((gather_corrupt_kernel<V, O>), dim3(grid), dim3(NT), 0, s, b->data, b->row_idx, \
-                                    b->mask_id, b->mask_table, b->B, b->io, out, b->mask_to_use, b->nb_run, b->run, out_ld)
+                                    b->mask_id, b->mask_table, b->B, b->io, out, b->mask_to_use, b->nb_run, b->run, out_ld, zero_norm)
     if (vec && out_bf16) GC(true, true);
     else if (vec) GC(true, false);
     else if (out_bf16) GC(false, true);
@@ -783,8 +795,8 @@
 }
 
 int launch_gather_noise(const codae_batch* b, const codae_noise* noise, int32_t step, const double* step_dev, void* out, int out_bf16,
-                        hipStream_t s, int64_t out_ld, const int32_t* noise_rows) {
-    if (noise == nullptr || noise->kind == CODAE_NOISE_NONE) return launch_gather_corrupt(b, out, out_bf16, s, out_ld);
+                        hipStream_t s, int64_t out_ld, const int32_t* noise_rows, double* zero_norm) {
+    if (noise == nullptr || noise->kind == CODAE_NOISE_NONE) return launch_gather_corrupt(b, out, out_bf16, s, out_ld, zero_norm);
     int rc = check_noise(noise);
     if (rc) return rc;
     if (out_ld <= 0) out_ld = b ? b->io : 0;
@@ -795,7 +807,7 @@
                   "gather_corrupt: run %d outside [0, %d)", b->run, b->nb_run);
     NoiseArgs na{};
     na.key0 = (uint32_t)(noise->seed & 0xffffffffu); na.key1 = (uint32_t)(noise->seed >> 32);
-    na.step = (uint32_t)step; na.step_dev = step_dev; na.rows = noise_rows;
+    na.step = (uint32_t)step; na.step_dev = step_dev; na.rows = noise_rows; na.zero_norm = zero_norm;
     na.thresh = (uint64_t)floor((double)noise->p0 * 4294967296.0);
     na.p0 = noise->p0; na.p1 = noise->p1; na.p2 = noise->p2;
     const bool vec = (b->io % 4 == 0) && (out_ld % 4 == 0) && a16(b->data) && a16(out) && (!masked || (reinterpret_cast<uintptr_t>(b->mask_table) & 3) == 0);
diff --git a/mui-deepautoencoder_amd/csrc/engine.hip b/mui-deepautoencoder_amd/csrc/engine.hip
--- a/mui-deepautoencoder_amd/csrc/engine.hip
+++ b/mui-deepautoencoder_amd/csrc/engine.hip
@@ -43,6 +43,9 @@
     e.no_defer_wgrad = getenv("CODAE_NO_DEFER_WGRAD") != nullptr;
     e.no_prefetch = getenv("CODAE_NO_PREFETCH") != nullptr;
     e.no_relu_bits = getenv("CODAE_NO_RELU_BITS") != nullptr;
+    e.no_folded_loss_finish = getenv("CODAE_NO_FOLDED_LOSS_FINISH") != nullptr;
+    if (const char* k = getenv("CODAE_STORE_POLICY"))
+        e.store_policy = !strcmp(k, "plain") ? STORE_PLAIN : (!strcmp(k, "wt") ? STORE_WT : -1);
     if (const char* k = getenv("CODAE_F32_GEMM")) e.f32_gemm = k[0] == 'n' ? 1 : (k[0] == 'x' ? 2 : 0);
     if (const char* k = getenv("CODAE_SMALL_TILE_MAX")) e.small_tile_max = atoi(k);
     if (const char* k = getenv("CODAE_SMALL_STAGES")) e.small_stages = atoi(k) == 2 ? 2 : 4;
@@ -481,6 +484,7 @@
         GemmBf16 g = layer_wgrad_bf16(e, b, l, rows);
         g.split_k = S;
         if (S > 1) {
+            g.store_policy = store_policy_for((int64_t)S * N * K * 4);
             CODAE_REQUIRE(b->slabs != nullptr, "bf16 wgrad needs the slab workspace");
             char* slab = reinterpret_cast<char*>(b->slabs) + (int64_t)slot * e->slab_bytes;
             g.C = slab;
@@ -603,7 +607,7 @@
 }
 
 int backward_range(codae_handle h, const codae_buffers* b, int B, int lo, int hi, float* dx, bool step_mode, bool with_norm,
-                   hipStream_t s, bool join = true) {
+                   hipStream_t s, bool join = true, const LossFinish* loss = nullptr) {
     const int rows = h->rows_for(B);
     const bool dual = !h->cfg.single_stream;
     if (dual) {
@@ -621,7 +625,7 @@
         rc = defer == 3 ? run_wgrad_deferred_f32(h, b, rows, s)
                         : (defer == 1 ? run_wgrad_deferred(h, b, rows, with_norm, s) : run_wgrad_grouped(h, b, rows, with_norm, s));
         if (rc) return rc;
-        return finish_bias(h, b, s, with_norm);
+        return finish_bias(h, b, s, with_norm, loss);
     }
     bool* w_pending = h->w_pending;
     const bool coscheduled = dual;
@@ -655,7 +659,7 @@
         }
     }
     if (join || lo == 0) {
-        int rc = finish_bias(h, b, s, with_norm);
+        int rc = finish_bias(h, b, s, with_norm, loss);
         if (rc) return rc;
     }
     if (dual) {
@@ -956,8 +960,8 @@
     return backward_range(h, b, B, layer_lo, layer_hi, dx, false, false, s);
 }
 
-int codae_step_forward_loss(codae_handle h, const codae_buffers* b, const codae_batch* batch, const codae_hyper* hyper,
-                            float* out_y, void* stream) {
+static int forward_loss_impl(codae_handle h, const codae_buffers* b, const codae_batch* batch, const codae_hyper* hyper,
+                             float* out_y, void* stream, LossFinish* fold) {
     CODAE_REQUIRE(batch != nullptr, "codae_step_forward_loss: null batch");
     int rc = check_common(h, b, batch->B);
     if (rc) return rc;
@@ -970,19 +974,21 @@
     const int B = batch->B, L = h->L;
     const int rows = h->rows_for(B);
     const bool bf = h->prec == CODAE_PREC_BF16;
+    const bool fuse_loss = bf && hyper != nullptr && out_y == nullptr && !h->cfg.no_fused_loss;
+    const bool fold_finish = fuse_loss && fold != nullptr && !h->cfg.no_folded_loss_finish;
     {
         ProfScope prof(h, CODAE_K_GATHER, s);
+        double* zero_norm = fold_finish ? b->scalars : nullptr;
         if (hyper != nullptr && h->noise.kind != CODAE_NOISE_NONE)
             rc = launch_gather_noise(batch, &h->noise, hyper->step, h->capturing ? b->scalars + CODAE_S_ADAM_STEP : nullptr,
-                                     act_ptr(h, b, 0), bf, s, h->in_ld[0]);
+                                     act_ptr(h, b, 0), bf, s, h->in_ld[0], nullptr, zero_norm);
         else
-            rc = launch_gather_corrupt(batch, act_ptr(h, b, 0), bf, s, h->in_ld[0]);
+            rc = launch_gather_corrupt(batch, act_ptr(h, b, 0), bf, s, h->in_ld[0], zero_norm);
     }
     if (rc) return rc;
     rc = zero_pad_rows(h, act_ptr(h, b, 0), B, rows, h->in_ld[0], s);
     if (rc) return rc;
     float* y = out_y ? out_y : reinterpret_cast<float*>(act_ptr(h, b, L));
-    const bool fuse_loss = bf && hyper != nullptr && out_y == nullptr && !h->cfg.no_fused_loss;
     GroupScope fwd_group(h, CODAE_K_GEMM_FWD, s);
     for (int l = 0; l < L; ++l) {
         const bool last = (l == L - 1);
@@ -1007,6 +1013,11 @@
             if (rc) return rc;
             h->parts_pending[l] = gemm_bf16_colsum_rows(g);
             h->norm_scalars_zero = true;
+            if (fold_finish) {
+                fold->scalars = b->scalars; fold->inv_n = 1.0 / ((double)B * batch->io);
+                fold->parts = loss_parts_ptr(h, b); fold->n_parts = n_loss_parts;
+                return CODAE_OK;
+            }
             return finish_loss(h, b, batch, n_loss_parts, s);
         }
         rc = last ? run_linear(h, b, l, act_ptr(h, b, l), y, true, B, s)
@@ -1031,6 +1042,11 @@
     rc = launch_mse_loss(batch, y, nullptr, 0, 0.f, nullptr, loss_parts_ptr(h, b), 0, s);
     if (rc) return rc;
     return finish_loss(h, b, batch, mse_loss_colsum_rows(B), s);
+}
+
+int codae_step_forward_loss(codae_handle h, const codae_buffers* b, const codae_batch* batch, const codae_hyper* hyper,
+                            float* out_y, void* stream) {
+    return forward_loss_impl(h, b, batch, hyper, out_y, stream, nullptr);
 }
 
 int codae_set_input_noise(codae_handle h, const codae_noise* noise) {
@@ -1184,10 +1200,11 @@
         if (rcc) return rcc;
         return update_impl(h, b, hyper, s, with_norm);
     }
-    int rc = codae_step_forward_loss(h, b, batch, hyper, nullptr, stream);
+    LossFinish lf{};
+    int rc = forward_loss_impl(h, b, batch, hyper, nullptr, stream, &lf);
     if (rc) return rc;
     const bool all_slabbed = h->prec == CODAE_PREC_BF16 && hyper->max_grad_norm > 0.f && !h->cfg.no_fused_norm;
-    rc = backward_range(h, b, batch->B, 0, h->L, nullptr, true, all_slabbed, (hipStream_t)stream);
+    rc = backward_range(h, b, batch->B, 0, h->L, nullptr, true, all_slabbed, (hipStream_t)stream, true, lf.scalars != nullptr ? &lf : nullptr);
     if (rc) return rc;
     return update_impl(h, b, hyper, (hipStream_t)stream, all_slabbed);
 }
diff --git a/mui-deepautoencoder_amd/csrc/gemm_bf16.hip b/mui-deepautoencoder_amd/csrc/gemm_bf16.hip
--- a/mui-deepautoencoder_amd/csrc/gemm_bf16.hip
+++ b/mui-deepautoencoder_amd/csrc/gemm_bf16.hip
@@ -604,6 +604,11 @@
     return CODAE_OK;
 }
 
+int store_policy_for(int64_t out_bytes) {
+    if (env().store_policy >= 0) return env().store_policy;
+    return out_bytes <= ((int64_t)32 << 20) ? STORE_WT : STORE_PLAIN;
+}
+
 bool gemm_bf16_supported(int M, int N, int K) {
     return M > 0 && N >= 8 && K >= BK && (K % BK) == 0 && (N % 8) == 0;
 }
diff --git a/mui-deepautoencoder_amd/csrc/gemm_bf16_pipe.hip b/mui-deepautoencoder_amd/csrc/gemm_bf16_pipe.hip
--- a/mui-deepautoencoder_amd/csrc/gemm_bf16_pipe.hip
+++ b/mui-deepautoencoder_amd/csrc/gemm_bf16_pipe.hip
@@ -9,7 +9,7 @@
 constexpr int TIMELINE_WGS = 4096, TIMELINE_SLOTS = 6;
 __device__ unsigned long long g_timeline[TIMELINE_WGS * TIMELINE_SLOTS];
 
-template <int BM, int BN, int WM, int WN, int NLB, int A_MODE, int B_MODE, bool C_F32, int DBG = 0, int EPI = 0>
+template <int BM, int BN, int WM, int WN, int NLB, int A_MODE, int B_MODE, bool C_F32, int DBG = 0, int EPI = 0, int POL = STORE_PLAIN>
 __device__ __forceinline__ void gemm_bf16_pipe_tile(const GemmBf16& g, int tiles_n, int tiles_mn, int kt_total, int wg, int nwg,
                                                     char* smem_raw) {
     constexpr int NW = WM * WN;
@@ -357,13 +357,14 @@
             const int c = threadIdx.x % CH, rl = threadIdx.x / CH;
             const int j = j0 + c * 8;
             bf16_t* Cb = reinterpret_cast<bf16_t*>(g.C);
+            const TileStore<POL> out(Cb + (int64_t)i0 * g.ldc);
             constexpr int ITER = (BM + RL - 1) / RL;
 #pragma unroll
             for (int it = 0; it < ITER; ++it) {
                 const int r = rl + it * RL;
                 const bool ok = rl < RL && j < g.N && r < BM && i0 + r < g.M;
                 const u32x4 lv = *reinterpret_cast<const __attribute__((address_space(3))) u32x4*>(smem + (ok ? r : 0) * PITCH + c * 16);
-                if (ok) *reinterpret_cast<uint4*>(Cb + (int64_t)(i0 + r) * g.ldc + j) = make_uint4(lv[0], lv[1], lv[2], lv[3]);
+                if (ok) out.store16(Cb + (int64_t)(i0 + r) * g.ldc + j, (uint32_t)(r * (int)g.ldc + j) * 2u, lv);
             }
         }
         if constexpr (dbg_time) { wait_vmcnt<0>(); stamp(4); }
@@ -460,6 +461,7 @@
         float cs[8] = {0.f, 0.f, 0.f, 0.f, 0.f, 0.f, 0.f, 0.f};
         {
             bf16_t* Cb = reinterpret_cast<bf16_t*>(g.C);
+            const TileStore<POL> out(Cb + (int64_t)i0 * g.ldc);
             const bool relu_mask = EPI != 1 && !bit_mask && g.relu_src != nullptr;
             const bf16_t* hsrc = relu_mask ? g.relu_src : g.A;
             const int64_t hld = relu_mask ? g.ld_relu : 0;
@@ -512,7 +514,7 @@
                     }
                 }
                 if (ok) {
-                    *reinterpret_cast<uint4*>(Cb + (int64_t)(i0 + r) * g.ldc + j) = v;
+                    out.store16(Cb + (int64_t)(i0 + r) * g.ldc + j, (uint32_t)(r * (int)g.ldc + j) * 2u, (u32x4){v.x, v.y, v.z, v.w});
                     if (EPI != 1 && g.colsum_part != nullptr) {
                         cs[0] += bf16_to_f32((bf16_t)(v.x & 0xffff)); cs[1] += bf16_to_f32((bf16_t)(v.x >> 16));
                         cs[2] += bf16_to_f32((bf16_t)(v.y & 0xffff)); cs[3] += bf16_to_f32((bf16_t)(v.y >> 16));
@@ -574,13 +576,14 @@
                 }
             __syncthreads();
             constexpr int ITER = (HR + RL - 1) / RL;
+            const TileStore<POL> out(Cf + (int64_t)(i0 + hh * HR) * g.ldc);
 #pragma unroll
             for (int it = 0; it < ITER; ++it) {
                 const int r = rl + it * RL;
                 const bool ok = rl < RL && j < g.N && r < HR && i0 + hh * HR + r < g.M;
                 const f32x4 v = *reinterpret_cast<const __attribute__((address_space(3))) f32x4*>(smem + (ok ? r : 0) * PITCH + c * 16);
                 if (ok) {
-                    *reinterpret_cast<float4*>(Cf + (int64_t)(i0 + hh * HR + r) * g.ldc + j) = make_float4(v[0], v[1], v[2], v[3]);
+                    out.store16(Cf + (int64_t)(i0 + hh * HR + r) * g.ldc + j, (uint32_t)(r * (int)g.ldc + j) * 4u, __builtin_bit_cast(u32x4, v));
                     sq += v[0] * v[0] + v[1] * v[1] + v[2] * v[2] + v[3] * v[3];
                 }
             }
@@ -601,13 +604,14 @@
     }
 }
 
-template <int BM, int BN, int WM, int WN, int NLB, int A_MODE, int B_MODE, bool C_F32, int DBG = 0, int EPI = 0>
+template <int BM, int BN, int WM, int WN, int NLB, int A_MODE, int B_MODE, bool C_F32, int DBG = 0, int EPI = 0, int POL = STORE_PLAIN>
 __global__ __launch_bounds__(64 * WM * WN, (WM * WN + 3) / 4)
 void gemm_bf16_pipe_kernel(GemmBf16 g, int tiles_n, int tiles_mn, int kt_total) {
     __shared__ __attribute__((aligned(16))) char smem_raw[2 * (BM + BN) * 128 + (EPI == 3 ? BM * 8 : 0)];
-    gemm_bf16_pipe_tile<BM, BN, WM, WN, NLB, A_MODE, B_MODE, C_F32, DBG, EPI>(g, tiles_n, tiles_mn, kt_total, blockIdx.x, gridDim.x, smem_raw);
-}
-
+    gemm_bf16_pipe_tile<BM, BN, WM, WN, NLB, A_MODE, B_MODE, C_F32, DBG, EPI, POL>(g, tiles_n, tiles_mn, kt_total, blockIdx.x, gridDim.x, smem_raw);
+}
+
+template <int POL>
 __global__ __launch_bounds__(512, 2) void gemm_bf16_pipe_grouped_kernel(GemmBf16Group grp) {
     constexpr int BM = 256, BN = 192;
     __shared__ __attribute__((aligned(16))) char smem_raw[2 * (BM + BN) * 128];
@@ -621,7 +625,7 @@
     while (j + 1 < grp.n && t >= grp.wg_begin[j + 1]) ++j;
     const GemmBf16& g = grp.g[j];
     const int tiles_m = (g.M + BM - 1) / BM, tiles_n = (g.N + BN - 1) / BN;
-    gemm_bf16_pipe_tile<BM, BN, 4, 2, 4, OP_KS, OP_KS, true, 0, 0>(g, tiles_n, tiles_m * tiles_n, g.K / BK, t - grp.wg_begin[j], 0, smem_raw);
+    gemm_bf16_pipe_tile<BM, BN, 4, 2, 4, OP_KS, OP_KS, true, 0, 0, POL>(g, tiles_n, tiles_m * tiles_n, g.K / BK, t - grp.wg_begin[j], 0, smem_raw);
 }
 
 template <int BM, int BN, int WM, int WN, int NLB>
@@ -634,8 +638,10 @@
                       (int64_t)(g.b_mode == OP_KC ? g.N : g.K) * g.ldb * 2 < (int64_t)1 << 32,
                   "gemm_bf16: operand larger than 4 GiB");
     dim3 grid((unsigned)nwg), block(64 * WM * WN);
+#define LAUNCH_POL(AM, BMODE, CF, EP, POL) \
+    hipLaunchKernelGGL((gemm_bf16_pipe_kernel<BM, BN, WM, WN, NLB, AM, BMODE, CF, 0, EP, POL>), grid, block, 0, s, g, tiles_n, tiles_m * tiles_n, kt_total)
 #define LAUNCH(AM, BMODE, CF, EP) \
-    hipLaunchKernelGGL((gemm_bf16_pipe_kernel<BM, BN, WM, WN, NLB, AM, BMODE, CF, 0, EP>), grid, block, 0, s, g, tiles_n, tiles_m * tiles_n, kt_total)
+    do { if (g.store_policy == STORE_WT) LAUNCH_POL(AM, BMODE, CF, EP, STORE_WT); else LAUNCH_POL(AM, BMODE, CF, EP, STORE_PLAIN); } while (0)
 #define LAUNCH_BF16(AM, BMODE) do { if (bwd_epi) LAUNCH(AM, BMODE, false, 2); else LAUNCH(AM, BMODE, false, 1); } while (0)
     const bool bwd_epi = g.relu_src != nullptr || g.colsum_part != nullptr;
     if (g.coscheduled && bwd_epi && !g.loss.enabled && g.a_mode == OP_KC && g.b_mode == OP_KC && !g.c_f32) {
@@ -652,6 +658,7 @@
     else { set_error("gemm_bf16: operand mode combination not built"); return CODAE_E_UNSUPPORTED; }
 #undef LAUNCH_BF16
 #undef LAUNCH
+#undef LAUNCH_POL
     CODAE_LAUNCH_CHECK();
     return CODAE_OK;
 }
@@ -662,6 +669,14 @@
 int launch_dbg(const GemmBf16& g, hipStream_t s) {
     constexpr int BM = 256, BN = 192;
     const int tiles_m = (g.M + BM - 1) / BM, tiles_n = (g.N + BN - 1) / BN;
+    if constexpr (DBG == 8) {
+        if (g.store_policy == STORE_WT) {
+            hipLaunchKernelGGL((gemm_bf16_pipe_kernel<BM, BN, 4, 2, 4, OP_KC, OP_KC, false, 8, 0, STORE_WT>), dim3(tiles_m * tiles_n), dim3(512), 0, s, g,
+                               tiles_n, tiles_m * tiles_n, g.K / BK);
+            CODAE_LAUNCH_CHECK();
+            return CODAE_OK;
+        }
+    }
     hipLaunchKernelGGL((gemm_bf16_pipe_kernel<BM, BN, 4, 2, 4, OP_KC, OP_KC, false, DBG>), dim3(tiles_m * tiles_n), dim3(512), 0, s, g,
                        tiles_n, tiles_m * tiles_n, g.K / BK);
     CODAE_LAUNCH_CHECK();
@@ -674,10 +689,11 @@
     CODAE_REQUIRE(g.a_mode == OP_KC && g.b_mode == OP_KC && !g.c_f32 && !g.loss.enabled && g.split_k == 1, "gemm_bf16: 128 x 192 tile is forward-form only");
     CODAE_REQUIRE((int64_t)g.M * g.lda * 2 < (int64_t)1 << 32 && (int64_t)g.N * g.ldb * 2 < (int64_t)1 << 32, "gemm_bf16: operand larger than 4 GiB");
     dim3 grid((unsigned)(tiles_m * tiles_n)), block(512);
-    if (g.relu_src != nullptr || g.colsum_part != nullptr)
-        hipLaunchKernelGGL((gemm_bf16_pipe_kernel<BM, BN, 4, 2, 4, OP_KC, OP_KC, false, 0, 2>), grid, block, 0, s, g, tiles_n, tiles_m * tiles_n, g.K / BK);
-    else
-        hipLaunchKernelGGL((gemm_bf16_pipe_kernel<BM, BN, 4, 2, 4, OP_KC, OP_KC, false, 0, 1>), grid, block, 0, s, g, tiles_n, tiles_m * tiles_n, g.K / BK);
+#define MID(EP, POL) hipLaunchKernelGGL((gemm_bf16_pipe_kernel<BM, BN, 4, 2, 4, OP_KC, OP_KC, false, 0, EP, POL>), grid, block, 0, s, g, tiles_n, tiles_m * tiles_n, g.K / BK)
+    const bool wt = g.store_policy == STORE_WT;
+    if (g.relu_src != nullptr || g.colsum_part != nullptr) { if (wt) MID(2, STORE_WT); else MID(2, STORE_PLAIN); }
+    else { if (wt) MID(1, STORE_WT); else MID(1, STORE_PLAIN); }
+#undef MID
     CODAE_LAUNCH_CHECK();
     return CODAE_OK;
 }
@@ -685,6 +701,9 @@
 int gemm_bf16_pipe_grouped(GemmBf16Group& grp, hipStream_t s) {
     CODAE_REQUIRE(grp.n >= 1 && grp.n <= CODAE_GROUP_MAX, "gemm_bf16_pipe_grouped: %d GEMMs", grp.n);
     int total = 0;
+    int64_t out_bytes = 0;
+    for (int j = 0; j < grp.n; ++j) out_bytes += (int64_t)grp.g[j].M * grp.g[j].N * 4;
+    bool all_wt = store_policy_for(out_bytes) == STORE_WT;
     for (int j = 0; j < grp.n; ++j) {
         const GemmBf16& g = grp.g[j];
         CODAE_REQUIRE(g.a_mode == OP_KS && g.b_mode == OP_KS && g.c_f32 && g.split_k == 1 && g.K % BK == 0 && g.K >= BK && g.M % 8 == 0 &&
@@ -695,16 +714,20 @@
                       "gemm_bf16_pipe_grouped: operand larger than 4 GiB");
         CODAE_REQUIRE((reinterpret_cast<uintptr_t>(g.A) & 15) == 0 && (reinterpret_cast<uintptr_t>(g.B) & 15) == 0 &&
                           (reinterpret_cast<uintptr_t>(g.C) & 15) == 0, "gemm_bf16_pipe_grouped: operands must be 16-byte aligned");
+        if (g.store_policy != STORE_WT || g.ldc >= ((int64_t)1 << 20)) all_wt = false;
         grp.wg_begin[j] = total;
         total += ((g.M + 255) / 256) * ((g.N + 191) / 192);
     }
     grp.wg_begin[grp.n] = total;
-    hipLaunchKernelGGL(gemm_bf16_pipe_grouped_kernel, dim3(total), dim3(512), 0, s, grp);
+    if (all_wt) hipLaunchKernelGGL(gemm_bf16_pipe_grouped_kernel<STORE_WT>, dim3(total), dim3(512), 0, s, grp);
+    else hipLaunchKernelGGL(gemm_bf16_pipe_grouped_kernel<STORE_PLAIN>, dim3(total), dim3(512), 0, s, grp);
     CODAE_LAUNCH_CHECK();
     return CODAE_OK;
 }
 
-int gemm_bf16_pipe(const GemmBf16& g, int cfg, hipStream_t s) {
+int gemm_bf16_pipe(const GemmBf16& g_in, int cfg, hipStream_t s) {
+    GemmBf16 g = g_in;
+    if (g.store_policy != STORE_WT || g.ldc >= ((int64_t)1 << 20)) g.store_policy = STORE_PLAIN;
     if (cfg == 7) return launch_pipe_mid(g, s);
     if (g.dbg == 8 && g.loss.enabled) {
         const int tiles_m = (g.M + 255) / 256, tiles_n = (g.N + 191) / 192;
diff --git a/mui-deepautoencoder_amd/csrc/layer_gemm.h b/mui-deepautoencoder_amd/csrc/layer_gemm.h
--- a/mui-deepautoencoder_amd/csrc/layer_gemm.h
+++ b/mui-deepautoencoder_amd/csrc/layer_gemm.h
@@ -11,6 +11,7 @@
     g.C = y; g.ldc = ldy; g.c_f32 = y_f32;
     g.M = rows; g.N = n_out; g.K = k;
     g.bias = bias; g.split_k = 1;
+    g.store_policy = store_policy_for((int64_t)rows * n_out * (y_f32 ? 4 : 2));
     return g;
 }
 
@@ -22,6 +23,7 @@
     g.C = dx; g.ldc = lddx; g.c_f32 = dx_f32;
     g.M = rows; g.N = n_in; g.K = k;
     g.split_k = 1;
+    g.store_policy = store_policy_for((int64_t)rows * n_in * (dx_f32 ? 4 : 2));
     return g;
 }
 
@@ -32,6 +34,7 @@
     g.C = dW; g.ldc = n_in; g.c_f32 = 1;
     g.M = n_out; g.N = n_in; g.K = rows;
     g.split_k = 1;
+    g.store_policy = store_policy_for((int64_t)n_out * n_in * 4);
     return g;
 }
 
```

After: 6.997 million samples/s (median of 6 runs). +2.0%, better.
